# ZhengyiLuo/PULSE

Measured on NVIDIA H100. Metric: env-steps/sec at 16384 humanoid envs, 1/2/4/8 H100; obs-kernel HBM GB/s, higher is better.
Workload: dtype bf16 GEMM operands, fp32 accumulate / master weights / observations

## Files before the change

include/pulse_b200.h:

```cpp
#ifndef PULSE_B200_H_
#define PULSE_B200_H_

#include <stdint.h>

#ifdef __cplusplus
extern "C" {
#endif

#define PULSE_ABI_VERSION 3

enum pulse_status {
  PULSE_OK = 0,
  PULSE_ERR_ARG = -1,
  PULSE_ERR_CUDA = -2,
  PULSE_ERR_UNSUPPORTED = -3
};

#define PULSE_NUM_BODIES 24
#define PULSE_NUM_DOF 69
#define PULSE_BODY_STATE_W 13
#define PULSE_SELF_OBS 358
#define PULSE_TASK_OBS_V6 576
#define PULSE_IM_OBS (PULSE_SELF_OBS + PULSE_TASK_OBS_V6)
#define PULSE_AMP_OBS 196
#define PULSE_FRAME_REC 312
#define PULSE_AUX_REC 240

int pulse_abi_version(void);
const char* pulse_last_error(void);
int64_t pulse_launch_count(void);

typedef struct pulse_motionlib pulse_motionlib_t;

typedef struct {
  const float* gts;
  const float* grs;
  const float* lrs;
  const float* gvs;
  const float* gavs;
  const float* dvs;
  const float* motion_aa;
  const float* lengths;
  const float* dt;
  const int64_t* num_frames;
  const int64_t* length_starts;
  int64_t total_frames;
  int64_t num_motions;
  float* frame_rec;
  float* aux_rec;
} pulse_motionlib_desc_t;

int pulse_motionlib_create(const pulse_motionlib_desc_t* desc, void* stream, pulse_motionlib_t** out);
int pulse_motionlib_destroy(pulse_motionlib_t* lib);

typedef struct {
  const int64_t* motion_ids;
  const float* motion_times;
  const float* offset;
  float* root_pos;
  float* root_rot;
  float* dof_pos;
  float* root_vel;
  float* root_ang_vel;
  float* dof_vel;
  float* motion_aa;
  float* rg_pos;
  float* rb_rot;
  float* body_vel;
  float* body_ang_vel;
  int64_t* frame_idx0;
  int64_t* frame_idx1;
  float* blend;
} pulse_motion_query_t;
int pulse_motion_state(const pulse_motionlib_t* lib, const pulse_motion_query_t* q, int64_t n, void* stream);

#define PULSE_STEP_REWARD 1u
#define PULSE_STEP_RESET 2u
#define PULSE_STEP_OBS 4u
#define PULSE_STEP_ALL 7u
#define PULSE_STEP_ADVANCE 8u

typedef struct {
  const float* body_state;
  int64_t body_env_stride;
  const float* dof_vel;
  int64_t dof_env_stride;
  int64_t dof_elem_stride;
  const float* dof_force;
  int64_t dof_force_stride;
  const int64_t* env_ids;
  const int64_t* progress_buf;
  const int64_t* motion_ids;
  const float* motion_start_times;
  const float* motion_start_offset;
  const float* global_offset;
  const int32_t* cycle_counter;
  const int64_t* reset_buf_in;
  const float* termination_distances;
  uint32_t reset_body_mask;
  uint32_t flags;
  float dt;
  float k_pos, k_rot, k_vel, k_ang_vel, w_pos, w_rot, w_vel, w_ang_vel;
  float power_coefficient;
  int32_t cycle_motion;
  int64_t max_episode_length;
  int32_t enable_early_termination;
  int32_t use_mean_reset;
  float* obs_buf;
  int64_t obs_stride;
  float* self_obs_buf;
  float* rew_buf;
  float* reward_raw;
  int64_t raw_stride;
  int64_t* reset_buf;
  int64_t* terminate_buf;
  uint8_t* pass_time;
  float* ref_body_pos;
  float* ref_body_vel;
  float* ref_body_rot;
  float* ref_dof_pos;
  const int32_t* env_count;
  const int32_t* recovery_counter;
  int64_t* progress_rw;
  float* fdones_out;
} pulse_im_step_args_t;
int pulse_im_step(const pulse_motionlib_t* lib, const pulse_im_step_args_t* args, int64_t num_envs, void* stream);

typedef struct {
  const float* body_state; int64_t body_env_stride;
  const float* dof_pos; const float* dof_vel; int64_t dof_env_stride; int64_t dof_elem_stride;
  float* amp_obs_buf;
  int32_t num_steps;
  int32_t shift_history;
} pulse_amp_obs_args_t;
int pulse_amp_obs(const pulse_amp_obs_args_t* args, int64_t num_envs, void* stream);

typedef struct {
  const float* mu; int64_t ld_mu;
  const float* logstd;
  const float* eps; int64_t ld_eps;
  uint64_t seed; const uint64_t* rng_offset; uint64_t rng_step;
  int32_t num_actions; int32_t reserved;
  float* actions; int64_t ld_actions;
  float* neglogp; int64_t ld_neglogp;
  float* mus_out; int64_t ld_mus;
  const float* value; int64_t ld_value;
  const double* value_mean; const double* value_var; float value_eps; int32_t reserved2;
  float* values_out; int64_t ld_values;
  const float* pd_offset; const float* pd_scale; float* pd_targets; int64_t ld_pd;
} pulse_policy_post_args_t;
int pulse_policy_post(const pulse_policy_post_args_t* args, int64_t rows, void* stream);
int pulse_value_post(const float* value, int64_t ld_value, const double* mean, const double* var, float eps, const int64_t* terminate,
                     float* out, int64_t ld_out, int64_t rows, void* stream);
typedef struct {
  const float* body_state; int64_t body_env_stride;
  const float* dof_pos; const float* dof_vel; int64_t dof_env_stride; int64_t dof_elem_stride;
  const float* prev; int64_t ld_prev;
  float* out; int64_t ld_out;
  int32_t num_steps; int32_t reserved;
  int32_t* fresh;
  const float* fresh_rows;
} pulse_amp_row_args_t;
int pulse_amp_obs_row(const pulse_amp_row_args_t* args, int64_t num_envs, void* stream);
int pulse_bump_counter(uint64_t* counter, uint64_t by, void* stream);
int pulse_event_create(void** event);
int pulse_event_destroy(void* event);
int pulse_event_record(void* event, void* stream);
int pulse_event_elapsed_ms(void* start, void* stop, float* ms);

typedef struct {
  int64_t* reset_buf;
  const int64_t* env_ids_in;
  int64_t num_ids;
  const float* phase;
  uint64_t seed, offset;
  const int64_t* motion_ids;
  float* motion_start_times;
  float* motion_start_offset;
  float* global_offset;
  int32_t* cycle_counter;
  int64_t* progress_buf;
  int64_t* terminate_buf;
  float* root_states; int64_t root_env_stride;
  float* dof_pos; float* dof_vel; int64_t dof_env_stride; int64_t dof_elem_stride;
  float* rigid_body_state; int64_t body_env_stride;
  float* contact_forces; int64_t contact_env_stride; int32_t contact_bodies;
  int32_t num_amp_steps;
  float* amp_obs_buf;
  float dt;
  int32_t reserved;
  const int32_t* actor_ids;
  int64_t* env_list;
  int32_t* actor_list;
  int32_t* count;
  int32_t* amp_fresh;
  const uint64_t* offset_dev;
} pulse_reset_args_t;
int pulse_reset_ref_state(const pulse_motionlib_t* lib, const pulse_reset_args_t* args, int64_t num_envs, void* stream);

typedef struct {
  const float* rewards;
  const float* values;
  const float* next_values;
  const float* fdones;
  float gamma, tau;
  float* advantages;
  float* returns;
  double* adv_sum;
} pulse_gae_args_t;
int pulse_gae(const pulse_gae_args_t* args, int32_t horizon, int64_t num_envs, void* stream);
int pulse_normalize_advantages(float* advantages, const double* adv_sum, int64_t count, void* stream);

typedef uint16_t pulse_bf16_t;
#define PULSE_ACT_NONE 0
#define PULSE_ACT_RELU 1
#define PULSE_ACT_SILU 2

typedef struct {
  const float* bias;
  int32_t act;
  int32_t gate_mode;
  const pulse_bf16_t* gate;
  int64_t ldg;
  float alpha;
  pulse_bf16_t* out;
  int64_t ldo;
  pulse_bf16_t* out_t;
  int64_t ldot;
  float* out_f32;
  int64_t ldf;
  int64_t split_stride;
  pulse_bf16_t* preact;
  int64_t ldp;
  float* colsum;
  int32_t accumulate;
  int32_t reserved;
  double* sumsq;
  uint32_t* relu_mask; int64_t ld_rmask;
  const uint32_t* gate_mask; int64_t ld_gmask;
} pulse_gemm_epilogue_t;

#define PULSE_GEMM_A_MN 1u
#define PULSE_GEMM_B_MN 2u

int pulse_gemm_bf16_nt(const void* a, int64_t lda, const void* b, int64_t ldb, int64_t m, int64_t n, int64_t k,
                       const pulse_gemm_epilogue_t* ep, int32_t split_k, void* stream);
int pulse_gemm_bf16(const void* a, int64_t lda, const void* b, int64_t ldb, int64_t m, int64_t n, int64_t k,
                    const pulse_gemm_epilogue_t* ep, int32_t split_k, uint32_t flags, void* stream);
int pulse_gemm_num_splits(int64_t k, int32_t split_k);

typedef struct {
  const void* a; int64_t lda;
  const void* b; int64_t ldb;
  int64_t m, n, k;
  pulse_gemm_epilogue_t ep;
  int32_t split_k, reserved;
} pulse_gemm_problem_t;
int pulse_gemm_bf16_grouped(const pulse_gemm_problem_t* problems, int32_t count, uint32_t flags, void* stream);

int pulse_normalize_to_bf16(const float* x, int64_t ldx, int64_t rows, int64_t cols, const float* mean, const float* rstd,
                            pulse_bf16_t* out, int64_t ld_out, pulse_bf16_t* out_t, int64_t ld_t, float pad_one, void* stream);

int pulse_column_moments(const float* x, int64_t ldx, int64_t rows, int64_t cols, double* sums, void* stream);

int pulse_normalize_moments(const float* x, int64_t ldx, int64_t rows, int64_t cols, const float* mean, const float* rstd,
                            pulse_bf16_t* out, int64_t ld_out, double* sums, float pad_one, void* stream);

int pulse_rms_merge(double* sums, int64_t n, int32_t size, double* mean, double* var, double* count, float eps,
                    float* mean_f32, float* rstd_f32, void* stream);

int pulse_head1_forward(const pulse_bf16_t* h, int64_t ldh, int64_t rows, int32_t k, const pulse_bf16_t* w, const float* bias, float* out,
                        int64_t ldo, void* stream);

#define PULSE_HEAD1_MAX_CTAS 264
int pulse_head1_backward(const pulse_bf16_t* h, int64_t ldh, int64_t rows, int32_t k, const pulse_bf16_t* dv, int64_t ld_dv,
                         const pulse_bf16_t* w, pulse_bf16_t* dh, int64_t ld_dh, float* dw, float* db, float* dbias_prev, float* partials,
                         void* stream);

int pulse_ordered_sum_add(const float* x, int64_t n, int64_t stride_n, int64_t rows, int64_t cols, int64_t ld, float* out, int64_t ldo,
                          void* stream);

int pulse_gaussian_sample(const float* mu, int64_t ld_mu, const float* eps, const float* logstd, int64_t rows, int32_t num_actions,
                          float* actions, float* neglogp, void* stream);

typedef struct {
  const float* mu; int64_t ld_mu;
  const float* value; int64_t ld_value;
  const float* actions;
  const float* old_neglogp;
  const float* advantages;
  const float* returns;
  const float* old_mu;
  const float* logstd;
  int32_t num_actions;
  float e_clip, critic_coef, bounds_coef;
  pulse_bf16_t* dmu; int64_t ld_dmu; pulse_bf16_t* dmu_t; int64_t ld_dmu_t;
  pulse_bf16_t* dvalue; int64_t ld_dv; pulse_bf16_t* dvalue_t; int64_t ld_dv_t;
  double* stats;
} pulse_ppo_loss_args_t;
int pulse_ppo_loss(const pulse_ppo_loss_args_t* args, int64_t rows, void* stream);

int pulse_disc_loss(const float* logits, int64_t ld, int64_t n_agent, int64_t n_demo, float scale, pulse_bf16_t* dlogit, int64_t ld_d,
                    double* stats, void* stream);
int pulse_relu_mask_scale(const pulse_bf16_t* h, int64_t ldh, int64_t rows, int64_t cols, const float* w, pulse_bf16_t* out, int64_t ldo,
                          void* stream);
int pulse_axpy(float a, const float* x, float* y, int64_t count, void* stream);
typedef struct {
  const float* w; float* g; int64_t rows, cols, ld; float coef; int32_t reserved; double* sumsq; double* sumsq2;
} pulse_weight_block_t;
typedef struct { pulse_weight_block_t block[4]; int32_t count; int32_t reserved; } pulse_weight_reg_t;
int pulse_weight_reg(const pulse_weight_reg_t* desc, void* stream);

int pulse_column_sum_bf16(const pulse_bf16_t* x, int64_t ldx, int64_t rows, int64_t cols, float* out, void* stream);
int pulse_reduce_slabs(const float* slabs, int64_t slab_stride, int32_t num_slabs, int64_t count, float* dst, void* stream);
int pulse_sum_squares(const float* x, int64_t count, double* sumsq, void* stream);
#define PULSE_ADAM_ZERO_GRADS 1u
#define PULSE_ADAM_SELF_CONTAINED 2u
int pulse_adam_step(float* params, float* grads, float* exp_avg, float* exp_avg_sq, int64_t count, double* grad_sumsq,
                    float max_norm, float lr, float beta1, float beta2, float eps, int32_t* step, pulse_bf16_t* params_bf16, uint32_t flags,
                    uint32_t* block_counter, void* stream);
#define PULSE_PEER_MAX 8
#define PULSE_PEER_MAX_GRID 256
#define PULSE_PEER_SIGNAL_BYTES (3 * PULSE_PEER_MAX * 4 + PULSE_PEER_MAX * 8)
typedef struct {
  int32_t rank, world;
  float* grads[PULSE_PEER_MAX];
  float* params[PULSE_PEER_MAX];
  pulse_bf16_t* params_bf16[PULSE_PEER_MAX];
  uint32_t* signals[PULSE_PEER_MAX];
  const float* mc_grads; float* mc_params; pulse_bf16_t* mc_params_bf16;
  float* exp_avg; float* exp_avg_sq;
  int64_t count;
  float max_norm, lr, beta1, beta2, eps;
  int32_t grid;
  uint32_t timeout_ms;
  uint32_t reserved;
  int32_t* step;
  uint32_t* epoch;
  double* cta_partials;
  unsigned long long* grid_bar;
} pulse_peer_adam_args_t;
int pulse_peer_reduce_adam(const pulse_peer_adam_args_t* args, void* stream);

int pulse_refresh_weight_bf16(const float* w, int64_t n, int64_t k, pulse_bf16_t* w_bf16, int64_t ld_k, pulse_bf16_t* wt_bf16,
                              int64_t ld_n, void* stream);

int pulse_normalize_cols(const float* x, int64_t ldx, int64_t rows, int64_t cols, const float* mean, const float* rstd, float clamp,
                         pulse_bf16_t* out, int64_t ld_out, int64_t zero_to, void* stream);
int pulse_copy_cols_bf16(const pulse_bf16_t* src, int64_t ld_src, int64_t rows, int64_t cols, pulse_bf16_t* dst1, int64_t ld1,
                         pulse_bf16_t* dst2, int64_t ld2, void* stream);

#define PULSE_Z_SAMPLE 0
#define PULSE_Z_MEAN 1
#define PULSE_Z_RESIDUAL 2
int pulse_vae_reparam(const float* head, int64_t ld_head, const float* noise, int64_t ld_noise, int64_t rows, int32_t latent,
                      int32_t mode, int32_t clamp, float clamp_lo, float clamp_hi, pulse_bf16_t* z_bf16, int64_t ld_z, float* z_f32,
                      int64_t ld_zf, void* stream);

int pulse_vae_action_loss(const float* pred, int64_t ld_pred, const float* gt, int64_t ld_gt, int64_t rows, int32_t num_actions,
                          pulse_bf16_t* dpred, int64_t ld_d, int64_t zero_to, double* stats, void* stream);

typedef struct {
  const float* enc_head; int64_t ld_enc;
  const float* prior_head; int64_t ld_prior;
  const float* noise; int64_t ld_noise;
  const float* dz; int64_t ld_dz;
  const int64_t* progress;
  int32_t latent, horizon, clamp, reserved;
  float clamp_lo, clamp_hi, kld_coef, ar1_coef, regu_coef, phi;
  pulse_bf16_t* d_enc_head; int64_t ld_de;
  pulse_bf16_t* d_prior_head; int64_t ld_dp;
  double* stats;
} pulse_vae_latent_args_t;
int pulse_vae_latent_loss(const pulse_vae_latent_args_t* args, int64_t rows, void* stream);

int pulse_pnn_compose(const float* acts, int64_t prim_stride, int64_t ld_a, const float* w, int64_t ld_w, int32_t act, int64_t rows,
                      int32_t num_actions, int32_t num_prim, float* out, int64_t ld_out, void* stream);

int pulse_pd_targets(const float* action, int64_t ld_a, const float* offset, const float* scale, const uint8_t* freeze, int64_t rows,
                     int32_t dofs, float* out, int64_t ld_out, void* stream);

int pulse_reach_update_task(const int64_t* progress, int64_t* tar_change_steps, float* tar_pos, const float* rand01, const int64_t* steps,
                            float dist_max, float h_min, float h_max, int64_t num_envs, void* stream);

typedef struct {
  const float* body_state; int64_t body_env_stride;
  const float* contact_forces; int64_t contact_env_stride;
  const float* termination_heights;
  const float* tar_pos;
  const int64_t* progress_buf;
  uint32_t contact_body_mask;
  int32_t reach_body_id;
  int32_t enable_early_termination, reserved;
  int64_t max_episode_length;
  float* obs_buf; int64_t obs_stride;
  float* rew_buf;
  int64_t* reset_buf; int64_t* terminate_buf;
} pulse_reach_step_args_t;
#define PULSE_REACH_OBS 361
int pulse_reach_step(const pulse_reach_step_args_t* args, int64_t num_envs, void* stream);

#define PULSE_ZTASK_SPEED 1
#define PULSE_ZTASK_STRIKE 2
#define PULSE_SPEED_OBS 361
#define PULSE_STRIKE_OBS 373
typedef struct {
  int32_t kind, enable_early_termination;
  const float* body_state; int64_t body_env_stride;
  const float* contact_forces; int64_t contact_env_stride;
  const float* termination_heights;
  uint32_t contact_body_mask;
  uint32_t strike_body_mask;
  const int64_t* progress_buf; int64_t max_episode_length;
  const float* prev_root_pos; float dt; float power_coefficient;
  const float* tar_speed;
  const float* target_states; int64_t target_env_stride;
  const float* tar_contact_forces; int64_t tar_contact_env_stride;
  const float* dof_force; int64_t dof_force_stride;
  const float* dof_vel; int64_t dof_env_stride, dof_elem_stride;
  float* obs_buf; int64_t obs_stride; float* rew_buf; float* reward_raw; int64_t raw_stride;
  int64_t* reset_buf; int64_t* terminate_buf;
} pulse_ztask_step_args_t;
int pulse_ztask_step(const pulse_ztask_step_args_t* args, int64_t num_envs, void* stream);

#define PULSE_TRAJ_VERTS 101
#define PULSE_TRAJ_DRAWS (4 * (PULSE_TRAJ_VERTS - 1) + 2)
#define PULSE_TERRAIN_OBS 1402
typedef struct {
  uint32_t flags;
  int32_t upright;
  const float* body_state; int64_t body_env_stride;
  const float* root_states; int64_t root_env_stride;
  const int64_t* progress_buf; int64_t max_episode_length;
  const float* contact_forces; int64_t contact_env_stride;
  uint32_t contact_body_mask;
  int32_t enable_early_termination, no_collision_check, fuzzy_target, power_reward;
  int32_t num_traj_samples, num_height_points, num_center_points, head_body_id, use_center_height;
  float dt, traj_dur, traj_sample_timestep, fail_dist, power_coefficient;
  const float* traj_verts;
  const int16_t* heightfield; int64_t hf_rows, hf_cols;
  float horizontal_scale, vertical_scale;
  const float* height_points;
  const float* center_points;
  const float* dof_force; int64_t dof_force_stride;
  const float* dof_vel; int64_t dof_env_stride, dof_elem_stride;
  const int64_t* env_ids; const int32_t* env_count;
  float* obs_buf; int64_t obs_stride;
  float* rew_buf; float* reward_raw; int64_t raw_stride;
  int64_t* reset_buf; int64_t* terminate_buf;
} pulse_terrain_step_args_t;
int pulse_terrain_step(const pulse_terrain_step_args_t* args, int64_t num_envs, void* stream);

typedef struct {
  const int64_t* env_ids; int64_t num_ids;
  const float* init_pos; int64_t init_stride;
  const float* rand;
  uint64_t seed, offset; const uint64_t* offset_dev;
  float dtheta_scale, dspeed_scale, seg_dt, speed_min, speed_max, sharp_turn_prob;
  float* verts;
} pulse_traj_reset_args_t;
int pulse_traj_reset(const pulse_traj_reset_args_t* args, void* stream);

#define PULSE_HEIGHTS_CENTER 1
#define PULSE_HEIGHTS_GRID 2
typedef struct {
  int32_t mode, upright;
  const float* root_states; int64_t root_stride; int64_t num_rows;
  const float* points; int64_t num_points;
  const int16_t* heightfield; int64_t hf_rows, hf_cols;
  float horizontal_scale, vertical_scale;
  float* heights; int64_t heights_stride;
} pulse_terrain_heights_args_t;
int pulse_terrain_heights(const pulse_terrain_heights_args_t* args, void* stream);

typedef struct {
  const float* body_state; int64_t body_env_stride;
  const int32_t* track_ids;
  int32_t num_track, time_steps, version, upright;
  const float* ref_pos; const float* ref_rot; const float* ref_vel; const float* ref_ang_vel;
  const float* dof_pos; int64_t dof_env_stride, dof_elem_stride;
  const float* ref_dof_pos;
  float* obs; int64_t obs_stride;
  int64_t num_envs;
} pulse_task_obs_args_t;
int pulse_task_obs_size(int32_t version, int32_t num_track, int32_t time_steps);
int pulse_im_task_obs(const pulse_task_obs_args_t* args, void* stream);

typedef struct {
  const float* body_pos; int64_t pos_env_stride, pos_body_stride;
  const float* body_pos_gt; int64_t gt_env_stride, gt_body_stride;
  const int64_t* terminate;
  const int32_t* num_steps;
  int32_t num_envs, bound, max_steps_all, reserved;
  int32_t* ctrl; int32_t* terminate_state; float* hist; double* sums; int32_t* counts; float* mpjpe_out;
} pulse_eval_args_t;
int pulse_eval_step(const pulse_eval_args_t* args, void* stream);

typedef struct {
  const double* pose_quat_global;
  const double* root_trans;
  const int32_t* frame_clip;
  const int64_t* clip_start;
  const float* fps;
  const double* headings;
  const int32_t* parents;
  const float* local_translation;
  int64_t total_frames, num_clips;
  float* gts; float* grs; float* lrs; float* gvs; float* gavs; float* dvs;
  float* tmp_vel; float* tmp_ang;
} pulse_loader_args_t;
int pulse_motionlib_load_clips(const pulse_loader_args_t* args, void* stream);

#ifdef __cplusplus
}
#endif
#endif
```

pulse_b200/_lib.py:

```python
import ctypes as C
import os

_PKG = os.path.dirname(os.path.abspath(__file__))
LIB_PATH = os.path.join(_PKG, "libpulse_b200.so")


class PulseError(RuntimeError):
    pass


c_float_p = C.POINTER(C.c_float)
c_i64_p = C.POINTER(C.c_int64)
c_i32_p = C.POINTER(C.c_int32)
c_u8_p = C.POINTER(C.c_uint8)
c_f64_p = C.POINTER(C.c_double)


class MotionLibDesc(C.Structure):
    _fields_ = [
        ("gts", C.c_void_p), ("grs", C.c_void_p), ("lrs", C.c_void_p), ("gvs", C.c_void_p), ("gavs", C.c_void_p),
        ("dvs", C.c_void_p), ("motion_aa", C.c_void_p), ("lengths", C.c_void_p), ("dt", C.c_void_p),
        ("num_frames", C.c_void_p), ("length_starts", C.c_void_p), ("total_frames", C.c_int64),
        ("num_motions", C.c_int64), ("frame_rec", C.c_void_p), ("aux_rec", C.c_void_p),
    ]


class MotionQuery(C.Structure):
    _fields_ = [(n, C.c_void_p) for n in (
        "motion_ids", "motion_times", "offset", "root_pos", "root_rot", "dof_pos", "root_vel", "root_ang_vel", "dof_vel",
        "motion_aa", "rg_pos", "rb_rot", "body_vel", "body_ang_vel", "frame_idx0", "frame_idx1", "blend")]


class ImStepArgs(C.Structure):
    _fields_ = [
        ("body_state", C.c_void_p), ("body_env_stride", C.c_int64),
        ("dof_vel", C.c_void_p), ("dof_env_stride", C.c_int64), ("dof_elem_stride", C.c_int64),
        ("dof_force", C.c_void_p), ("dof_force_stride", C.c_int64), ("env_ids", C.c_void_p),
        ("progress_buf", C.c_void_p), ("motion_ids", C.c_void_p), ("motion_start_times", C.c_void_p),
        ("motion_start_offset", C.c_void_p), ("global_offset", C.c_void_p), ("cycle_counter", C.c_void_p),
        ("reset_buf_in", C.c_void_p), ("termination_distances", C.c_void_p),
        ("reset_body_mask", C.c_uint32), ("flags", C.c_uint32), ("dt", C.c_float),
        ("k_pos", C.c_float), ("k_rot", C.c_float), ("k_vel", C.c_float), ("k_ang_vel", C.c_float),
        ("w_pos", C.c_float), ("w_rot", C.c_float), ("w_vel", C.c_float), ("w_ang_vel", C.c_float),
        ("power_coefficient", C.c_float), ("cycle_motion", C.c_int32), ("max_episode_length", C.c_int64),
        ("enable_early_termination", C.c_int32), ("use_mean_reset", C.c_int32),
        ("obs_buf", C.c_void_p), ("obs_stride", C.c_int64), ("self_obs_buf", C.c_void_p), ("rew_buf", C.c_void_p),
        ("reward_raw", C.c_void_p), ("raw_stride", C.c_int64), ("reset_buf", C.c_void_p), ("terminate_buf", C.c_void_p),
        ("pass_time", C.c_void_p), ("ref_body_pos", C.c_void_p), ("ref_body_vel", C.c_void_p),
        ("ref_body_rot", C.c_void_p), ("ref_dof_pos", C.c_void_p),
        ("env_count", C.c_void_p), ("recovery_counter", C.c_void_p), ("progress_rw", C.c_void_p), ("fdones_out", C.c_void_p),
    ]


class ResetArgs(C.Structure):
    _fields_ = [
        ("reset_buf", C.c_void_p), ("env_ids_in", C.c_void_p), ("num_ids", C.c_int64), ("phase", C.c_void_p),
        ("seed", C.c_uint64), ("offset", C.c_uint64), ("motion_ids", C.c_void_p), ("motion_start_times", C.c_void_p),
        ("motion_start_offset", C.c_void_p), ("global_offset", C.c_void_p), ("cycle_counter", C.c_void_p), ("progress_buf", C.c_void_p),
        ("terminate_buf", C.c_void_p), ("root_states", C.c_void_p), ("root_env_stride", C.c_int64),
        ("dof_pos", C.c_void_p), ("dof_vel", C.c_void_p), ("dof_env_stride", C.c_int64), ("dof_elem_stride", C.c_int64),
        ("rigid_body_state", C.c_void_p), ("body_env_stride", C.c_int64),
        ("contact_forces", C.c_void_p), ("contact_env_stride", C.c_int64), ("contact_bodies", C.c_int32),
        ("num_amp_steps", C.c_int32), ("amp_obs_buf", C.c_void_p), ("dt", C.c_float), ("reserved", C.c_int32),
        ("actor_ids", C.c_void_p), ("env_list", C.c_void_p), ("actor_list", C.c_void_p), ("count", C.c_void_p), ("amp_fresh", C.c_void_p),
        ("offset_dev", C.c_void_p),
    ]


class WeightBlock(C.Structure):
    _fields_ = [("w", C.c_void_p), ("g", C.c_void_p), ("rows", C.c_int64), ("cols", C.c_int64), ("ld", C.c_int64), ("coef", C.c_float),
                ("reserved", C.c_int32), ("sumsq", C.c_void_p), ("sumsq2", C.c_void_p)]


class WeightReg(C.Structure):
    _fields_ = [("block", WeightBlock * 4), ("count", C.c_int32), ("reserved", C.c_int32)]


class PolicyPostArgs(C.Structure):
    _fields_ = [
        ("mu", C.c_void_p), ("ld_mu", C.c_int64), ("logstd", C.c_void_p), ("eps", C.c_void_p), ("ld_eps", C.c_int64),
        ("seed", C.c_uint64), ("rng_offset", C.c_void_p), ("rng_step", C.c_uint64), ("num_actions", C.c_int32), ("reserved", C.c_int32),
        ("actions", C.c_void_p), ("ld_actions", C.c_int64), ("neglogp", C.c_void_p), ("ld_neglogp", C.c_int64),
        ("mus_out", C.c_void_p), ("ld_mus", C.c_int64), ("value", C.c_void_p), ("ld_value", C.c_int64),
        ("value_mean", C.c_void_p), ("value_var", C.c_void_p), ("value_eps", C.c_float), ("reserved2", C.c_int32),
        ("values_out", C.c_void_p), ("ld_values", C.c_int64),
        ("pd_offset", C.c_void_p), ("pd_scale", C.c_void_p), ("pd_targets", C.c_void_p), ("ld_pd", C.c_int64),
    ]


class AmpRowArgs(C.Structure):
    _fields_ = [
        ("body_state", C.c_void_p), ("body_env_stride", C.c_int64), ("dof_pos", C.c_void_p), ("dof_vel", C.c_void_p),
        ("dof_env_stride", C.c_int64), ("dof_elem_stride", C.c_int64), ("prev", C.c_void_p), ("ld_prev", C.c_int64),
        ("out", C.c_void_p), ("ld_out", C.c_int64), ("num_steps", C.c_int32), ("reserved", C.c_int32),
        ("fresh", C.c_void_p), ("fresh_rows", C.c_void_p),
    ]


class AmpObsArgs(C.Structure):
    _fields_ = [
        ("body_state", C.c_void_p), ("body_env_stride", C.c_int64), ("dof_pos", C.c_void_p), ("dof_vel", C.c_void_p),
        ("dof_env_stride", C.c_int64), ("dof_elem_stride", C.c_int64), ("amp_obs_buf", C.c_void_p),
        ("num_steps", C.c_int32), ("shift_history", C.c_int32),
    ]


class GaeArgs(C.Structure):
    _fields_ = [
        ("rewards", C.c_void_p), ("values", C.c_void_p), ("next_values", C.c_void_p), ("fdones", C.c_void_p),
        ("gamma", C.c_float), ("tau", C.c_float), ("advantages", C.c_void_p), ("returns", C.c_void_p), ("adv_sum", C.c_void_p),
    ]


class GemmEpilogue(C.Structure):
    _fields_ = [
        ("bias", C.c_void_p), ("act", C.c_int32), ("gate_mode", C.c_int32), ("gate", C.c_void_p), ("ldg", C.c_int64),
        ("alpha", C.c_float), ("out", C.c_void_p), ("ldo", C.c_int64), ("out_t", C.c_void_p), ("ldot", C.c_int64),
        ("out_f32", C.c_void_p), ("ldf", C.c_int64), ("split_stride", C.c_int64), ("preact", C.c_void_p), ("ldp", C.c_int64),
        ("colsum", C.c_void_p), ("accumulate", C.c_int32), ("reserved", C.c_int32), ("sumsq", C.c_void_p),
        ("relu_mask", C.c_void_p), ("ld_rmask", C.c_int64), ("gate_mask", C.c_void_p), ("ld_gmask", C.c_int64),
    ]


GEMM_A_MN, GEMM_B_MN = 1, 2


class GemmProblem(C.Structure):
    _fields_ = [("a", C.c_void_p), ("lda", C.c_int64), ("b", C.c_void_p), ("ldb", C.c_int64), ("m", C.c_int64), ("n", C.c_int64),
                ("k", C.c_int64), ("ep", GemmEpilogue), ("split_k", C.c_int32), ("reserved", C.c_int32)]


class PpoLossArgs(C.Structure):
    _fields_ = [
        ("mu", C.c_void_p), ("ld_mu", C.c_int64), ("value", C.c_void_p), ("ld_value", C.c_int64), ("actions", C.c_void_p),
        ("old_neglogp", C.c_void_p), ("advantages", C.c_void_p), ("returns", C.c_void_p), ("old_mu", C.c_void_p),
        ("logstd", C.c_void_p), ("num_actions", C.c_int32), ("e_clip", C.c_float), ("critic_coef", C.c_float),
        ("bounds_coef", C.c_float), ("dmu", C.c_void_p), ("ld_dmu", C.c_int64), ("dmu_t", C.c_void_p), ("ld_dmu_t", C.c_int64),
        ("dvalue", C.c_void_p), ("ld_dv", C.c_int64), ("dvalue_t", C.c_void_p), ("ld_dv_t", C.c_int64), ("stats", C.c_void_p),
    ]


class VaeLatentArgs(C.Structure):
    _fields_ = [
        ("enc_head", C.c_void_p), ("ld_enc", C.c_int64), ("prior_head", C.c_void_p), ("ld_prior", C.c_int64),
        ("noise", C.c_void_p), ("ld_noise", C.c_int64), ("dz", C.c_void_p), ("ld_dz", C.c_int64), ("progress", C.c_void_p),
        ("latent", C.c_int32), ("horizon", C.c_int32), ("clamp", C.c_int32), ("reserved", C.c_int32),
        ("clamp_lo", C.c_float), ("clamp_hi", C.c_float), ("kld_coef", C.c_float), ("ar1_coef", C.c_float),
        ("regu_coef", C.c_float), ("phi", C.c_float),
        ("d_enc_head", C.c_void_p), ("ld_de", C.c_int64), ("d_prior_head", C.c_void_p), ("ld_dp", C.c_int64), ("stats", C.c_void_p),
    ]


class ReachStepArgs(C.Structure):
    _fields_ = [
        ("body_state", C.c_void_p), ("body_env_stride", C.c_int64), ("contact_forces", C.c_void_p), ("contact_env_stride", C.c_int64),
        ("termination_heights", C.c_void_p), ("tar_pos", C.c_void_p), ("progress_buf", C.c_void_p),
        ("contact_body_mask", C.c_uint32), ("reach_body_id", C.c_int32), ("enable_early_termination", C.c_int32), ("reserved", C.c_int32),
        ("max_episode_length", C.c_int64), ("obs_buf", C.c_void_p), ("obs_stride", C.c_int64), ("rew_buf", C.c_void_p),
        ("reset_buf", C.c_void_p), ("terminate_buf", C.c_void_p),
    ]


class LoaderArgs(C.Structure):
    _fields_ = [
        ("pose_quat_global", C.c_void_p), ("root_trans", C.c_void_p), ("frame_clip", C.c_void_p), ("clip_start", C.c_void_p),
        ("fps", C.c_void_p), ("headings", C.c_void_p), ("parents", C.c_void_p), ("local_translation", C.c_void_p),
        ("total_frames", C.c_int64), ("num_clips", C.c_int64),
        ("gts", C.c_void_p), ("grs", C.c_void_p), ("lrs", C.c_void_p), ("gvs", C.c_void_p), ("gavs", C.c_void_p), ("dvs", C.c_void_p),
        ("tmp_vel", C.c_void_p), ("tmp_ang", C.c_void_p),
    ]


class ZTaskStepArgs(C.Structure):
    _fields_ = [
        ("kind", C.c_int32), ("enable_early_termination", C.c_int32), ("body_state", C.c_void_p), ("body_env_stride", C.c_int64),
        ("contact_forces", C.c_void_p), ("contact_env_stride", C.c_int64), ("termination_heights", C.c_void_p),
        ("contact_body_mask", C.c_uint32), ("strike_body_mask", C.c_uint32), ("progress_buf", C.c_void_p), ("max_episode_length", C.c_int64),
        ("prev_root_pos", C.c_void_p), ("dt", C.c_float), ("power_coefficient", C.c_float), ("tar_speed", C.c_void_p),
        ("target_states", C.c_void_p), ("target_env_stride", C.c_int64), ("tar_contact_forces", C.c_void_p), ("tar_contact_env_stride", C.c_int64),
        ("dof_force", C.c_void_p), ("dof_force_stride", C.c_int64), ("dof_vel", C.c_void_p), ("dof_env_stride", C.c_int64), ("dof_elem_stride", C.c_int64),
        ("obs_buf", C.c_void_p), ("obs_stride", C.c_int64), ("rew_buf", C.c_void_p), ("reward_raw", C.c_void_p), ("raw_stride", C.c_int64),
        ("reset_buf", C.c_void_p), ("terminate_buf", C.c_void_p),
    ]


ZTASK_SPEED, ZTASK_STRIKE = 1, 2


class TerrainStepArgs(C.Structure):
    _fields_ = [
        ("flags", C.c_uint32), ("upright", C.c_int32), ("body_state", C.c_void_p), ("body_env_stride", C.c_int64),
        ("root_states", C.c_void_p), ("root_env_stride", C.c_int64), ("progress_buf", C.c_void_p), ("max_episode_length", C.c_int64),
        ("contact_forces", C.c_void_p), ("contact_env_stride", C.c_int64), ("contact_body_mask", C.c_uint32),
        ("enable_early_termination", C.c_int32), ("no_collision_check", C.c_int32), ("fuzzy_target", C.c_int32), ("power_reward", C.c_int32),
        ("num_traj_samples", C.c_int32), ("num_height_points", C.c_int32), ("num_center_points", C.c_int32), ("head_body_id", C.c_int32),
        ("use_center_height", C.c_int32), ("dt", C.c_float), ("traj_dur", C.c_float), ("traj_sample_timestep", C.c_float),
        ("fail_dist", C.c_float), ("power_coefficient", C.c_float), ("traj_verts", C.c_void_p),
        ("heightfield", C.c_void_p), ("hf_rows", C.c_int64), ("hf_cols", C.c_int64), ("horizontal_scale", C.c_float), ("vertical_scale", C.c_float),
        ("height_points", C.c_void_p), ("center_points", C.c_void_p), ("dof_force", C.c_void_p), ("dof_force_stride", C.c_int64),
        ("dof_vel", C.c_void_p), ("dof_env_stride", C.c_int64), ("dof_elem_stride", C.c_int64), ("env_ids", C.c_void_p), ("env_count", C.c_void_p),
        ("obs_buf", C.c_void_p), ("obs_stride", C.c_int64), ("rew_buf", C.c_void_p), ("reward_raw", C.c_void_p), ("raw_stride", C.c_int64),
        ("reset_buf", C.c_void_p), ("terminate_buf", C.c_void_p),
    ]


class TrajResetArgs(C.Structure):
    _fields_ = [
        ("env_ids", C.c_void_p), ("num_ids", C.c_int64), ("init_pos", C.c_void_p), ("init_stride", C.c_int64), ("rand", C.c_void_p),
        ("seed", C.c_uint64), ("offset", C.c_uint64), ("offset_dev", C.c_void_p), ("dtheta_scale", C.c_float), ("dspeed_scale", C.c_float),
        ("seg_dt", C.c_float), ("speed_min", C.c_float), ("speed_max", C.c_float), ("sharp_turn_prob", C.c_float), ("verts", C.c_void_p),
    ]


class TerrainHeightsArgs(C.Structure):
    _fields_ = [
        ("mode", C.c_int32), ("upright", C.c_int32), ("root_states", C.c_void_p), ("root_stride", C.c_int64), ("num_rows", C.c_int64),
        ("points", C.c_void_p), ("num_points", C.c_int64), ("heightfield", C.c_void_p), ("hf_rows", C.c_int64), ("hf_cols", C.c_int64),
        ("horizontal_scale", C.c_float), ("vertical_scale", C.c_float), ("heights", C.c_void_p), ("heights_stride", C.c_int64),
    ]


TRAJ_VERTS = 101
TRAJ_DRAWS = 4 * (TRAJ_VERTS - 1) + 2
HEIGHTS_CENTER, HEIGHTS_GRID = 1, 2


class TaskObsArgs(C.Structure):
    _fields_ = [
        ("body_state", C.c_void_p), ("body_env_stride", C.c_int64), ("track_ids", C.c_void_p),
        ("num_track", C.c_int32), ("time_steps", C.c_int32), ("version", C.c_int32), ("upright", C.c_int32),
        ("ref_pos", C.c_void_p), ("ref_rot", C.c_void_p), ("ref_vel", C.c_void_p), ("ref_ang_vel", C.c_void_p),
        ("dof_pos", C.c_void_p), ("dof_env_stride", C.c_int64), ("dof_elem_stride", C.c_int64), ("ref_dof_pos", C.c_void_p),
        ("obs", C.c_void_p), ("obs_stride", C.c_int64), ("num_envs", C.c_int64),
    ]


class EvalArgs(C.Structure):
    _fields_ = [
        ("body_pos", C.c_void_p), ("pos_env_stride", C.c_int64), ("pos_body_stride", C.c_int64),
        ("body_pos_gt", C.c_void_p), ("gt_env_stride", C.c_int64), ("gt_body_stride", C.c_int64),
        ("terminate", C.c_void_p), ("num_steps", C.c_void_p),
        ("num_envs", C.c_int32), ("bound", C.c_int32), ("max_steps_all", C.c_int32), ("reserved", C.c_int32),
        ("ctrl", C.c_void_p), ("terminate_state", C.c_void_p), ("hist", C.c_void_p), ("sums", C.c_void_p), ("counts", C.c_void_p),
        ("mpjpe_out", C.c_void_p),
    ]


PEER_MAX, PEER_MAX_GRID, PEER_SIGNAL_BYTES = 8, 256, 3 * 8 * 4 + 8 * 8


class PeerAdamArgs(C.Structure):
    _fields_ = [
        ("rank", C.c_int32), ("world", C.c_int32),
        ("grads", C.c_void_p * PEER_MAX), ("params", C.c_void_p * PEER_MAX), ("params_bf16", C.c_void_p * PEER_MAX),
        ("signals", C.c_void_p * PEER_MAX),
        ("mc_grads", C.c_void_p), ("mc_params", C.c_void_p), ("mc_params_bf16", C.c_void_p),
        ("exp_avg", C.c_void_p), ("exp_avg_sq", C.c_void_p), ("count", C.c_int64),
        ("max_norm", C.c_float), ("lr", C.c_float), ("beta1", C.c_float), ("beta2", C.c_float), ("eps", C.c_float), ("grid", C.c_int32),
        ("timeout_ms", C.c_uint32), ("reserved", C.c_uint32), ("step", C.c_void_p), ("epoch", C.c_void_p), ("cta_partials", C.c_void_p), ("grid_bar", C.c_void_p),
    ]


ABI_VERSION = 3
HEAD1_MAX_CTAS = 264
ACT_NONE, ACT_RELU, ACT_SILU = 0, 1, 2
Z_SAMPLE, Z_MEAN, Z_RESIDUAL = 0, 1, 2
STEP_REWARD, STEP_RESET, STEP_OBS, STEP_ALL, STEP_ADVANCE = 1, 2, 4, 7, 8

SIGNATURES = {
    "pulse_abi_version": (C.c_int, []),
    "pulse_last_error": (C.c_char_p, []),
    "pulse_launch_count": (C.c_int64, []),
    "pulse_motionlib_create": (C.c_int, [C.POINTER(MotionLibDesc), C.c_void_p, C.POINTER(C.c_void_p)]),
    "pulse_motionlib_destroy": (C.c_int, [C.c_void_p]),
    "pulse_motion_state": (C.c_int, [C.c_void_p, C.POINTER(MotionQuery), C.c_int64, C.c_void_p]),
    "pulse_im_step": (C.c_int, [C.c_void_p, C.POINTER(ImStepArgs), C.c_int64, C.c_void_p]),
    "pulse_reset_ref_state": (C.c_int, [C.c_void_p, C.POINTER(ResetArgs), C.c_int64, C.c_void_p]),
    "pulse_policy_post": (C.c_int, [C.POINTER(PolicyPostArgs), C.c_int64, C.c_void_p]),
    "pulse_value_post": (C.c_int, [C.c_void_p, C.c_int64, C.c_void_p, C.c_void_p, C.c_float, C.c_void_p, C.c_void_p, C.c_int64, C.c_int64, C.c_void_p]),
    "pulse_amp_obs_row": (C.c_int, [C.POINTER(AmpRowArgs), C.c_int64, C.c_void_p]),
    "pulse_bump_counter": (C.c_int, [C.c_void_p, C.c_uint64, C.c_void_p]),
    "pulse_event_create": (C.c_int, [C.POINTER(C.c_void_p)]),
    "pulse_event_destroy": (C.c_int, [C.c_void_p]),
    "pulse_event_record": (C.c_int, [C.c_void_p, C.c_void_p]),
    "pulse_event_elapsed_ms": (C.c_int, [C.c_void_p, C.c_void_p, C.POINTER(C.c_float)]),
    "pulse_amp_obs": (C.c_int, [C.POINTER(AmpObsArgs), C.c_int64, C.c_void_p]),
    "pulse_gae": (C.c_int, [C.POINTER(GaeArgs), C.c_int32, C.c_int64, C.c_void_p]),
    "pulse_normalize_advantages": (C.c_int, [C.c_void_p, C.c_void_p, C.c_int64, C.c_void_p]),
    "pulse_gemm_bf16_nt": (C.c_int, [C.c_void_p, C.c_int64, C.c_void_p, C.c_int64, C.c_int64, C.c_int64, C.c_int64,
                                     C.POINTER(GemmEpilogue), C.c_int32, C.c_void_p]),
    "pulse_gemm_bf16": (C.c_int, [C.c_void_p, C.c_int64, C.c_void_p, C.c_int64, C.c_int64, C.c_int64, C.c_int64,
                                  C.POINTER(GemmEpilogue), C.c_int32, C.c_uint32, C.c_void_p]),
    "pulse_gemm_num_splits": (C.c_int, [C.c_int64, C.c_int32]),
    "pulse_gemm_bf16_grouped": (C.c_int, [C.POINTER(GemmProblem), C.c_int32, C.c_uint32, C.c_void_p]),
    "pulse_normalize_to_bf16": (C.c_int, [C.c_void_p, C.c_int64, C.c_int64, C.c_int64, C.c_void_p, C.c_void_p, C.c_void_p, C.c_int64,
                                          C.c_void_p, C.c_int64, C.c_float, C.c_void_p]),
    "pulse_normalize_moments": (C.c_int, [C.c_void_p, C.c_int64, C.c_int64, C.c_int64, C.c_void_p, C.c_void_p, C.c_void_p, C.c_int64,
                                          C.c_void_p, C.c_float, C.c_void_p]),
    "pulse_head1_forward": (C.c_int, [C.c_void_p, C.c_int64, C.c_int64, C.c_int32, C.c_void_p, C.c_void_p, C.c_void_p, C.c_int64, C.c_void_p]),
    "pulse_head1_backward": (C.c_int, [C.c_void_p, C.c_int64, C.c_int64, C.c_int32, C.c_void_p, C.c_int64, C.c_void_p, C.c_void_p, C.c_int64,
                                       C.c_void_p, C.c_void_p, C.c_void_p, C.c_void_p, C.c_void_p]),
    "pulse_ordered_sum_add": (C.c_int, [C.c_void_p, C.c_int64, C.c_int64, C.c_int64, C.c_int64, C.c_int64, C.c_void_p, C.c_int64, C.c_void_p]),
    "pulse_column_moments": (C.c_int, [C.c_void_p, C.c_int64, C.c_int64, C.c_int64, C.c_void_p, C.c_void_p]),
    "pulse_rms_merge": (C.c_int, [C.c_void_p, C.c_int64, C.c_int32, C.c_void_p, C.c_void_p, C.c_void_p, C.c_float, C.c_void_p, C.c_void_p,
                                  C.c_void_p]),
    "pulse_gaussian_sample": (C.c_int, [C.c_void_p, C.c_int64, C.c_void_p, C.c_void_p, C.c_int64, C.c_int32, C.c_void_p, C.c_void_p,
                                        C.c_void_p]),
    "pulse_ppo_loss": (C.c_int, [C.POINTER(PpoLossArgs), C.c_int64, C.c_void_p]),
    "pulse_disc_loss": (C.c_int, [C.c_void_p, C.c_int64, C.c_int64, C.c_int64, C.c_float, C.c_void_p, C.c_int64, C.c_void_p, C.c_void_p]),
    "pulse_relu_mask_scale": (C.c_int, [C.c_void_p, C.c_int64, C.c_int64, C.c_int64, C.c_void_p, C.c_void_p, C.c_int64, C.c_void_p]),
    "pulse_weight_reg": (C.c_int, [C.POINTER(WeightReg), C.c_void_p]),
    "pulse_axpy": (C.c_int, [C.c_float, C.c_void_p, C.c_void_p, C.c_int64, C.c_void_p]),
    "pulse_column_sum_bf16": (C.c_int, [C.c_void_p, C.c_int64, C.c_int64, C.c_int64, C.c_void_p, C.c_void_p]),
    "pulse_reduce_slabs": (C.c_int, [C.c_void_p, C.c_int64, C.c_int32, C.c_int64, C.c_void_p, C.c_void_p]),
    "pulse_sum_squares": (C.c_int, [C.c_void_p, C.c_int64, C.c_void_p, C.c_void_p]),
    "pulse_adam_step": (C.c_int, [C.c_void_p, C.c_void_p, C.c_void_p, C.c_void_p, C.c_int64, C.c_void_p, C.c_float, C.c_float,
                                  C.c_float, C.c_float, C.c_float, C.c_void_p, C.c_void_p, C.c_uint32, C.c_void_p, C.c_void_p]),
    "pulse_peer_reduce_adam": (C.c_int, [C.POINTER(PeerAdamArgs), C.c_void_p]),
    "pulse_refresh_weight_bf16": (C.c_int, [C.c_void_p, C.c_int64, C.c_int64, C.c_void_p, C.c_int64, C.c_void_p, C.c_int64, C.c_void_p]),
    "pulse_normalize_cols": (C.c_int, [C.c_void_p, C.c_int64, C.c_int64, C.c_int64, C.c_void_p, C.c_void_p, C.c_float, C.c_void_p, C.c_int64,
                                       C.c_int64, C.c_void_p]),
    "pulse_copy_cols_bf16": (C.c_int, [C.c_void_p, C.c_int64, C.c_int64, C.c_int64, C.c_void_p, C.c_int64, C.c_void_p, C.c_int64, C.c_void_p]),
    "pulse_vae_reparam": (C.c_int, [C.c_void_p, C.c_int64, C.c_void_p, C.c_int64, C.c_int64, C.c_int32, C.c_int32, C.c_int32, C.c_float,
                                    C.c_float, C.c_void_p, C.c_int64, C.c_void_p, C.c_int64, C.c_void_p]),
    "pulse_vae_action_loss": (C.c_int, [C.c_void_p, C.c_int64, C.c_void_p, C.c_int64, C.c_int64, C.c_int32, C.c_void_p, C.c_int64, C.c_int64,
                                        C.c_void_p, C.c_void_p]),
    "pulse_vae_latent_loss": (C.c_int, [C.POINTER(VaeLatentArgs), C.c_int64, C.c_void_p]),
    "pulse_pnn_compose": (C.c_int, [C.c_void_p, C.c_int64, C.c_int64, C.c_void_p, C.c_int64, C.c_int32, C.c_int64, C.c_int32, C.c_int32,
                                    C.c_void_p, C.c_int64, C.c_void_p]),
    "pulse_pd_targets": (C.c_int, [C.c_void_p, C.c_int64, C.c_void_p, C.c_void_p, C.c_void_p, C.c_int64, C.c_int32, C.c_void_p, C.c_int64,
                                   C.c_void_p]),
    "pulse_reach_update_task": (C.c_int, [C.c_void_p, C.c_void_p, C.c_void_p, C.c_void_p, C.c_void_p, C.c_float, C.c_float, C.c_float,
                                          C.c_int64, C.c_void_p]),
    "pulse_reach_step": (C.c_int, [C.POINTER(ReachStepArgs), C.c_int64, C.c_void_p]),
    "pulse_ztask_step": (C.c_int, [C.POINTER(ZTaskStepArgs), C.c_int64, C.c_void_p]),
    "pulse_terrain_step": (C.c_int, [C.POINTER(TerrainStepArgs), C.c_int64, C.c_void_p]),
    "pulse_traj_reset": (C.c_int, [C.POINTER(TrajResetArgs), C.c_void_p]),
    "pulse_terrain_heights": (C.c_int, [C.POINTER(TerrainHeightsArgs), C.c_void_p]),
    "pulse_task_obs_size": (C.c_int, [C.c_int32, C.c_int32, C.c_int32]),
    "pulse_im_task_obs": (C.c_int, [C.POINTER(TaskObsArgs), C.c_void_p]),
    "pulse_eval_step": (C.c_int, [C.POINTER(EvalArgs), C.c_void_p]),
    "pulse_motionlib_load_clips": (C.c_int, [C.POINTER(LoaderArgs), C.c_void_p]),
}

_lib = None


def load():
    global _lib
    if _lib is not None:
        return _lib
    if not os.path.exists(LIB_PATH):
        raise PulseError(f"{LIB_PATH} is missing: build it with `python -m pulse_b200.build` "
                         "(nvcc, sm_90a). pulse_b200 has no CPU fallback.")
    lib = C.CDLL(LIB_PATH)
    for name, (res, args) in SIGNATURES.items():
        fn = getattr(lib, name)
        fn.restype = res
        fn.argtypes = args
    if lib.pulse_abi_version() != ABI_VERSION:
        raise PulseError(f"ABI version mismatch: library {lib.pulse_abi_version()} != binding {ABI_VERSION}")
    _lib = lib
    return lib


def check(status, what):
    if status != 0:
        msg = load().pulse_last_error().decode("utf-8", "replace")
        raise PulseError(f"{what} failed with status {status}: {msg}")


def ptr(t):
    return None if t is None else C.c_void_p(t.data_ptr())


def current_stream(device=None):
    import torch
    return C.c_void_p(torch.cuda.current_stream(device).cuda_stream)


class GraphEvent:

    def __init__(self):
        self._h = C.c_void_p()
        check(load().pulse_event_create(C.byref(self._h)), "pulse_event_create")

    def record(self, device=None):
        check(load().pulse_event_record(self._h, current_stream(device)), "pulse_event_record")

    def elapsed_ms(self, stop: "GraphEvent") -> float:
        ms = C.c_float()
        check(load().pulse_event_elapsed_ms(self._h, stop._h, C.byref(ms)), "pulse_event_elapsed_ms")
        return float(ms.value)

    def __del__(self):
        try:
            if self._h:
                load().pulse_event_destroy(self._h)
        except Exception:
            pass
```

pulse_b200/amp.py:

```python
import ctypes as C
from typing import Dict, Optional, Sequence

import torch

from . import _lib
from .dense import column_sum_add, gemm
from .nets import MLP, FlatParams, pad_k, pick_split
from .ppo import RunningMeanStdB200


class AmpDiscriminator:
    def __init__(self, flat: FlatParams, amp_obs_size: int = 1960, units: Sequence[int] = (1024, 512), disc_coef: float = 5.0,
                 logit_reg: float = 0.01, grad_penalty: float = 5.0, weight_decay: float = 0.0001, reward_scale: float = 2.0):
        self.flat, self.device = flat, flat.device
        self.size = amp_obs_size
        self.mlp = MLP(flat, amp_obs_size, units, 1, "relu", aug=True)
        self.Kp = self.mlp.Kp0
        if len(units) != 2:
            raise _lib.PulseError("the analytic gradient penalty is written for the 2-hidden-layer discriminator of im.yaml")
        self.disc_coef, self.logit_reg, self.grad_penalty, self.weight_decay = disc_coef, logit_reg, grad_penalty, weight_decay
        self.reward_scale = reward_scale
        self.rms = RunningMeanStdB200(amp_obs_size, self.device)
        self.rms.pad_one = 1.0
        self.stats = torch.zeros(8, dtype=torch.float64, device=self.device)
        self._bufs: Dict[int, dict] = {}
        self.lib = _lib.load()

    def rewards(self, amp_obs: torch.Tensor, x_buf: Optional[torch.Tensor] = None) -> torch.Tensor:
        R = amp_obs.shape[0]
        x = x_buf if x_buf is not None else torch.empty(R, self.Kp, device=self.device, dtype=torch.bfloat16)
        self.rms.normalize_into(amp_obs, x)
        logits = self.mlp.forward(x)
        prob = 1.0 / (1.0 + torch.exp(-logits))
        return -torch.log(torch.clamp(1.0 - prob, min=1e-4)) * self.reward_scale

    def _buf(self, B: int):
        if B not in self._bufs:
            dev, bf = self.device, torch.bfloat16
            L1, L2, _ = self.mlp.layers
            self._bufs[B] = {
                "x": torch.zeros(2, 3 * B, self.Kp, device=dev, dtype=bf),
                "dlogit": torch.zeros(3 * B, 8, device=dev, dtype=bf),
                "g2": torch.zeros(B, L2.Np, device=dev, dtype=bf), "g1": torch.zeros(B, L1.Np, device=dev, dtype=bf),
                "Gb": torch.zeros(B, self.Kp, device=dev, dtype=bf),
                "du": torch.zeros(B, L1.Np, device=dev, dtype=bf), "scratch": torch.zeros(B, L2.Np, device=dev),
                "split1": pick_split(((L1.N + 127) // 128) * ((L1.Kp + 127) // 128), (B + 63) // 64),
                "split2": pick_split(((L2.N + 127) // 128) * ((L2.Kp + 127) // 128), (B + 63) // 64),
            }
        return self._bufs[B]

    def prepare_inputs(self, amp_agent: torch.Tensor, amp_replay: torch.Tensor, amp_demo: torch.Tensor, update_rms: bool = True, slot: int = 0) -> None:
        B = amp_agent.shape[0]
        if amp_replay.shape[0] != B or amp_demo.shape[0] != B:
            raise _lib.PulseError("agent / replay / demo AMP batches must have the same number of rows")
        x = self._buf(B)["x"][slot]
        for k, src in enumerate((amp_agent, amp_replay, amp_demo)):
            if update_rms:
                self.rms.normalize_update(src, x[k * B:(k + 1) * B])
            else:
                self.rms.normalize_into(src, x[k * B:(k + 1) * B])

    def loss_backward(self, amp_agent: torch.Tensor, amp_replay: torch.Tensor, amp_demo: torch.Tensor, update_rms: bool = True,
                      slot: int = 0, prepared: bool = False) -> torch.Tensor:
        B = amp_agent.shape[0]
        if not prepared:
            self.prepare_inputs(amp_agent, amp_replay, amp_demo, update_rms, slot)
        b = self._buf(B)
        lib, dev = self.lib, self.device
        L1, L2, L3 = self.mlp.layers
        x = b["x"][slot]
        logits = self.mlp.forward(x, train=True)
        self.stats.zero_()
        with torch.cuda.device(dev):
            st = _lib.current_stream(dev)
            _lib.check(lib.pulse_disc_loss(logits.data_ptr(), logits.stride(0), 2 * B, B, self.disc_coef, b["dlogit"].data_ptr(),
                                           b["dlogit"].stride(0), self.stats.data_ptr(), st), "pulse_disc_loss")
        self.mlp.backward(b["dlogit"], 3 * B)
        ws = self.mlp._ws[(3 * B, True)]
        h2 = ws["act"][1][2 * B:]
        m1, m2 = ws["mask"][0][:, 2 * B:], ws["mask"][1][:, 2 * B:]
        w3 = L3.weight.view(-1)
        with torch.cuda.device(dev):
            _lib.check(lib.pulse_relu_mask_scale(h2.data_ptr(), h2.stride(0), B, L2.N, w3.data_ptr(), b["g2"].data_ptr(), b["g2"].stride(0),
                                                 _lib.current_stream(dev)), "pulse_relu_mask_scale")
        W1, W2 = L1.w_bf16[:, :L1.K], L2.w_bf16[:, :L1.N]
        gemm(b["g2"][:, :L2.N], W2, b_mn=True, gate_mask=m1, out=b["g1"])
        c = 2.0 * self.disc_coef * self.grad_penalty / B
        gemm(b["g1"][:, :L1.N], W1, b_mn=True, alpha=c, out=b["Gb"], sumsq=self.stats[4:])
        gemm(b["g1"][:, :L1.N], b["Gb"], a_mn=True, b_mn=True, out_f32=L1.weight_grad, accumulate=True, split_k=b["split1"])
        gemm(b["Gb"], L1.w_bf16, gate_mask=m1, out=b["du"])
        gemm(b["g2"][:, :L2.N], b["du"][:, :L1.N], a_mn=True, b_mn=True, out_f32=L2.weight_grad, accumulate=True, split_k=b["split2"])
        gemm(b["du"][:, :L1.N], W2, gate_mask=m2, out_f32=b["scratch"])
        column_sum_add(b["scratch"][:, :L2.N], L3.weight_grad.view(-1))
        reg = _lib.WeightReg()
        reg.count = 3
        for k, l in enumerate((L1, L2, L3)):
            coef = 2.0 * self.disc_coef * (self.weight_decay + (self.logit_reg if l is L3 else 0.0))
            blk = reg.block[k]
            blk.w, blk.g, blk.rows, blk.cols, blk.ld, blk.coef = l.weight.data_ptr(), l.weight_grad.data_ptr(), l.N, l.K, l.Kp, coef
            blk.sumsq = self.stats[6:].data_ptr()
            if l is L3:
                blk.sumsq2 = self.stats[5:].data_ptr()
        with torch.cuda.device(dev):
            _lib.check(lib.pulse_weight_reg(C.byref(reg), _lib.current_stream(dev)), "pulse_weight_reg")
        return self.stats

    def loss_from_stats(self, stats: torch.Tensor, B: int) -> Dict[str, float]:
        s = stats.cpu()
        c = 2.0 * self.disc_coef * self.grad_penalty / B
        gp = float(s[4]) / (c * c) / B
        bce = 0.5 * (float(s[0]) / (2 * B) + float(s[1]) / B)
        loss = bce + self.logit_reg * float(s[5]) + self.grad_penalty * gp + self.weight_decay * float(s[6])
        return {"disc_loss": loss, "disc_grad_penalty": gp, "disc_logit_loss": float(s[5]), "disc_agent_acc": float(s[2]) / (2 * B),
                "disc_demo_acc": float(s[3]) / B}

    def loss_tensors(self, B: int) -> Dict[str, torch.Tensor]:
        s = self.stats
        c = 2.0 * self.disc_coef * self.grad_penalty / B
        gp = s[4] / (c * c) / B
        bce = 0.5 * (s[0] / (2 * B) + s[1] / B)
        logits = self.mlp._ws[(3 * B, True)]["out"]
        return {"disc_loss": bce + self.logit_reg * s[5] + self.grad_penalty * gp + self.weight_decay * s[6], "disc_grad_penalty": gp,
                "disc_logit_loss": s[5].clone(), "disc_agent_acc": s[2] / (2 * B), "disc_demo_acc": s[3] / B,
                "disc_agent_logit": logits[:2 * B].mean(), "disc_demo_logit": logits[2 * B:].mean()}

    def state_dict(self) -> Dict[str, torch.Tensor]:
        sd = {f"a2c_network.{k}": v for k, v in self.mlp.state_dict("_disc_mlp", "_disc_logits").items()}
        sd["amp_input_mean_std.running_mean"] = self.rms.running_mean.clone()
        sd["amp_input_mean_std.running_var"] = self.rms.running_var.clone()
        sd["amp_input_mean_std.count"] = self.rms.count.clone()
        return sd
```

pulse_b200/csrc/gemm_kernel.inc:

```
#if PULSE_GEMM_GROUPED
#define PULSE_GEMM_FIRST(member) grp.p[0].member
#define PULSE_GEMM_W wl
#define PULSE_GEMM_SELECT(w)                                                                                         \
  int pi = 0;                                                                                                        \
  while (pi + 1 < grp.count && (w) >= grp.p[pi].item_end) ++pi;                                                      \
  const GemmProblem& P = grp.p[pi];                                                                                  \
  const int wl = (w) - (pi == 0 ? 0 : grp.p[pi - 1].item_end);                                                       \
  const CUtensorMap& map_a = P.map_a;                                                                                \
  const CUtensorMap& map_b = P.map_b;                                                                                \
  const CUtensorMap& map_c = P.map_c;                                                                                \
  const int use_tma_red = P.use_tma_red;                                                                             \
  const pulse_gemm_epilogue_t& ep = P.ep;                                                                            \
  const int M = P.M, N = P.N, K = P.K, kb_per_split = P.kb_per_split;                                                \
  const int tiles_n = (N + BN - 1) / BN, tiles_m = (M + BM - 1) / BM;                                                \
  const int tiles = tiles_m * tiles_n;                                                                               \
  const int num_kb_total = (K + BK - 1) / BK;                                                                        \
  (void)map_a; (void)map_b; (void)map_c; (void)use_tma_red; (void)ep; (void)M; (void)N; (void)tiles_n; (void)kb_per_split; (void)num_kb_total;
#else
#define PULSE_GEMM_FIRST(member) member
#define PULSE_GEMM_W w
#define PULSE_GEMM_SELECT(w)
#endif

#if PULSE_GEMM_GROUPED
template <bool A_MN, bool B_MN, int MODE>
__global__ void __launch_bounds__(kThreads, 1) gemm_bf16_grouped_kernel(const __grid_constant__ GemmGroup grp) {
#else
template <bool A_MN, bool B_MN, int MODE>
__global__ void __launch_bounds__(kThreads, 1) gemm_bf16_kernel(const __grid_constant__ CUtensorMap map_a,
                                                                const __grid_constant__ CUtensorMap map_b,
                                                                const __grid_constant__ CUtensorMap map_c,
                                                                const pulse_gemm_epilogue_t ep, int M, int N, int K,
                                                                int kb_per_split, int splits, int use_tma_red) {
#endif
  constexpr bool kFwd = MODE == kModeGeneric || MODE == kModeFwd;
  constexpr bool kDgrad = MODE == kModeGeneric || MODE == kModeDgrad || MODE == kModeDgradVec;
  constexpr bool kGateVec = MODE == kModeGeneric || MODE == kModeDgradVec;
  constexpr bool kAccum = MODE == kModeGeneric || MODE == kModeWgrad;
  constexpr bool kBf16Out = MODE != kModeWgrad;
  extern __shared__ unsigned char gsm_raw[];
  GemmSmem& sm = *reinterpret_cast<GemmSmem*>((reinterpret_cast<uintptr_t>(gsm_raw) + 1023) & ~static_cast<uintptr_t>(1023));
  const int warp = threadIdx.x >> 5, lane = threadIdx.x & 31;
  const int work0 = static_cast<int>(blockIdx.x);
  const int work_stride = static_cast<int>(gridDim.x);
#if PULSE_GEMM_GROUPED
  const int total = grp.total_items;
#else
  const int tiles_n = (N + BN - 1) / BN, tiles_m = (M + BM - 1) / BM;
  const int tiles = tiles_m * tiles_n;
  const int total = tiles * splits;
  const int num_kb_total = (K + BK - 1) / BK;
#endif
  if (threadIdx.x == 0) PULSE_TRACE(0);

  if (threadIdx.x == 0) {
#pragma unroll
    for (int s = 0; s < kStages; ++s) {
      g_mbar_init(&sm.full[s], 1);
      g_mbar_init(&sm.empty[s], kConsumerWarps);
    }
    asm volatile("fence.mbarrier_init.release.cluster;\n" ::: "memory");
    asm volatile("prefetch.tensormap [%0];\n" ::"l"(&PULSE_GEMM_FIRST(map_a)) : "memory");
    asm volatile("prefetch.tensormap [%0];\n" ::"l"(&PULSE_GEMM_FIRST(map_b)) : "memory");
  }
  __syncthreads();
  if (threadIdx.x == 0) PULSE_TRACE(1);
  asm volatile("griddepcontrol.launch_dependents;\n" ::: "memory");

  if (warp < 4) {
    if (warp == 0 && lane == 0) {
      asm volatile("griddepcontrol.wait;\n" ::: "memory");
      PULSE_TRACE(2);
      int it = 0;
      for (int w = work0; w < total; w += work_stride) {
        PULSE_GEMM_SELECT(w)
        const int split = PULSE_GEMM_W / tiles, t = PULSE_GEMM_W - split * tiles;
        const int m0 = (t / tiles_n) * BM, n0 = (t % tiles_n) * BN;
        const int kb0 = split * kb_per_split;
        const int num_kb = min(kb_per_split, num_kb_total - kb0);
        for (int kb = 0; kb < num_kb; ++kb, ++it) {
          const int s = it % kStages;
          g_mbar_wait(&sm.empty[s], ((it / kStages) & 1) ^ 1);
          g_mbar_expect_tx(&sm.full[s], kStageBytesA + kStageBytesB);
          const int kk = (kb0 + kb) * BK;
          if (A_MN) {
            tma_load_2d(sm.a[s], &map_a, m0, kk, &sm.full[s]);
            tma_load_2d(sm.a[s] + 8192, &map_a, m0 + 64, kk, &sm.full[s]);
          } else {
            tma_load_2d(sm.a[s], &map_a, kk, m0, &sm.full[s]);
          }
          if (B_MN) {
            tma_load_2d(sm.b[s], &map_b, n0, kk, &sm.full[s]);
            tma_load_2d(sm.b[s] + 8192, &map_b, n0 + 64, kk, &sm.full[s]);
          } else {
            tma_load_2d(sm.b[s], &map_b, kk, n0, &sm.full[s]);
          }
        }
      }
    }
  } else {
    const int wg = (warp >> 2) - 1;
    const int ew = warp - 4;
    const int quarter = wg * 2 + (warp & 1);
    const int chalf = (warp >> 1) & 1;
    float* red_stage = sm.red[ew];
    float* acc_s = sm.acc[wg];
    asm volatile("griddepcontrol.wait;\n" ::: "memory");
    int it = 0, lw = 0;
    for (int w = work0; w < total; w += work_stride, ++lw) {
      PULSE_GEMM_SELECT(w)
      const int split = PULSE_GEMM_W / tiles, t = PULSE_GEMM_W - split * tiles;
      const int m0 = (t / tiles_n) * BM, n0 = (t % tiles_n) * BN;
      const int kb0 = split * kb_per_split;
      const int num_kb = min(kb_per_split, num_kb_total - kb0);
      const int row = m0 + quarter * 32 + lane;
      const bool row_ok = row < M;
      const bool gate_fast = (MODE == kModeGeneric || MODE == kModeDgrad) && ep.gate != nullptr && ep.gate_mask == nullptr && ep.gate_mode == PULSE_ACT_RELU && (ep.ldg & 7) == 0 && n0 + chalf * kCols + kCols <= N;
      unsigned gmask[kChunks] = {};
      const bool gate_bits = kDgrad && ep.gate_mask != nullptr;
      if (gate_bits && row_ok) {
#pragma unroll
        for (int cc = 0; cc < kChunks; ++cc) {
          const int col = n0 + (chalf * kChunks + cc) * 32;
          if (col < N) gmask[cc] = __ldg(ep.gate_mask + static_cast<long long>(col >> 5) * ep.ld_gmask + row);
        }
      }
      if (gate_fast && row_ok) {
        const uint4* g = reinterpret_cast<const uint4*>(reinterpret_cast<const __nv_bfloat16*>(ep.gate) + static_cast<long long>(row) * ep.ldg +
                                                        n0 + chalf * kCols);
        uint4 u[kChunks * 4];
#pragma unroll
        for (int i = 0; i < kChunks * 4; ++i) u[i] = __ldg(g + i);
#pragma unroll
        for (int i = 0; i < kChunks * 4; ++i) {
          const unsigned wds[4] = {u[i].x, u[i].y, u[i].z, u[i].w};
#pragma unroll
          for (int q = 0; q < 4; ++q) {
            const unsigned pos = (((wds[q] & 0x7fff7fffu) + 0x7fff7fffu) & ~wds[q]) & 0x80008000u;
            gmask[i >> 2] |= (pos >> 15) << ((i & 3) * 4 + q);
          }
        }
      }
      const bool gate_vec = kGateVec && ep.gate != nullptr && !gate_fast && !gate_bits && (ep.ldg & 7) == 0;
      uint4 gq[4] = {};
      auto gate_fetch = [&](int cc) {
        const int c0 = n0 + cc * 32;
        if (gate_vec && row_ok && c0 + 32 <= N) {
          const uint4* g = reinterpret_cast<const uint4*>(reinterpret_cast<const __nv_bfloat16*>(ep.gate) + static_cast<long long>(row) * ep.ldg + c0);
#pragma unroll
          for (int q = 0; q < 4; ++q) gq[q] = __ldg(g + q);
        }
      };
      gate_fetch(chalf * kChunks);
      float bias_l[kChunks] = {};
      const bool fwd_fast = MODE == kModeFwd && ep.out != nullptr && (ep.ldo & 7) == 0 && ep.out_f32 == nullptr && ep.out_t == nullptr &&
                            (ep.preact == nullptr || (ep.ldp & 7) == 0) && n0 + chalf * kCols + kCols <= N;
      float* bias_s = sm.bias[ew];
      if (fwd_fast && ep.bias != nullptr) {
        __syncwarp();
#pragma unroll
        for (int cc = 0; cc < kChunks; ++cc) bias_s[cc * 32 + lane] = __ldg(ep.bias + n0 + (chalf * kChunks + cc) * 32 + lane);
        __syncwarp();
      } else if (kFwd && ep.bias != nullptr) {
#pragma unroll
        for (int cc = 0; cc < kChunks; ++cc) {
          const int col = n0 + (chalf * kChunks + cc) * 32 + lane;
          if (col < N) bias_l[cc] = __ldg(ep.bias + col);
        }
      }

      float d[64];
#pragma unroll
      for (int i = 0; i < 64; ++i) d[i] = 0.0f;
      acc_fence(d);
      int prev_s = -1;
      for (int kb = 0; kb < num_kb; ++kb, ++it) {
        const int s = it % kStages;
        g_mbar_wait(&sm.full[s], (it / kStages) & 1);
        if (it == 0 && ew == 0 && lane == 0) PULSE_TRACE(3);
        wgmma_fence();
        const unsigned a_addr = s_u32(sm.a[s]) + static_cast<unsigned>(wg) * 8192u, b_addr = s_u32(sm.b[s]);
#pragma unroll
        for (int k = 0; k < BK / MMA_K; ++k) {
          const unsigned long long da = A_MN ? gmma_desc(a_addr + k * 2048, 8192) : gmma_desc(a_addr + k * 32, 16);
          const unsigned long long db = B_MN ? gmma_desc(b_addr + k * 2048, 8192) : gmma_desc(b_addr + k * 32, 16);
          wgmma_m64n128<A_MN ? 1 : 0, B_MN ? 1 : 0>(d, da, db, (kb | k) != 0 ? 1u : 0u);
        }
        wgmma_commit();
        wgmma_wait<1>();
        if (prev_s >= 0 && lane == 0) g_mbar_arrive(&sm.empty[prev_s]);
        prev_s = s;
      }
      wgmma_wait<0>();
      acc_fence(d);
      if (lane == 0) g_mbar_arrive(&sm.empty[prev_s]);
      if (ew == 0 && lane == 0 && lw < 3) PULSE_TRACE(4 + lw);

      wg_sync(wg);
      {
        const int r0 = (warp & 3) * 16 + (lane >> 2);
#pragma unroll
        for (int j = 0; j < BN / 8; ++j) {
          const int col = 8 * j + 2 * (lane & 3);
#pragma unroll
          for (int h = 0; h < 2; ++h) {
            const int r = r0 + 8 * h;
            const int rb = r & 31;
            float* blk = acc_s + ((r >> 5) * 4 + (col >> 5)) * 1024;
            const int unit = ((col & 31) >> 2) ^ (rb & 7);
            *reinterpret_cast<float2*>(blk + rb * 32 + unit * 4 + (col & 3)) = make_float2(d[4 * j + 2 * h], d[4 * j + 2 * h + 1]);
          }
        }
      }
      if (MODE == kModeWgrad && use_tma_red) asm volatile("fence.proxy.async.shared::cta;\n" ::: "memory");
      wg_sync(wg);
      if (ew == 0 && lane == 0 && lw < 3) PULSE_TRACE(16 + 2 * lw);

      float* outf = ep.out_f32 != nullptr ? ep.out_f32 + static_cast<long long>(ep.accumulate ? 0 : split) * ep.split_stride : nullptr;
      float sq = 0.0f;
#pragma unroll 1
      for (int c = chalf * kChunks; c < chalf * kChunks + kChunks; ++c) {
        const int col0 = n0 + c * 32;
        const bool full = col0 + 32 <= N;
        float* blk = acc_s + ((quarter & 1) * 4 + c) * 1024;
        if (MODE == kModeWgrad && use_tma_red) {
          if (lane == 0) {
            asm volatile("cp.reduce.async.bulk.tensor.2d.global.shared::cta.add.tile.bulk_group [%0, {%2, %3}], [%1];\n" ::"l"(&map_c),
                         "r"(s_u32(blk)), "r"(col0), "r"(m0 + quarter * 32)
                         : "memory");
            asm volatile("cp.async.bulk.commit_group;\n" ::: "memory");
          }
          continue;
        }
        float v[32];
        {
          const float4* b4 = reinterpret_cast<const float4*>(blk) + lane * 8;
#pragma unroll
          for (int u = 0; u < 8; ++u) {
            const float4 x = b4[u ^ (lane & 7)];
            v[4 * u] = x.x; v[4 * u + 1] = x.y; v[4 * u + 2] = x.z; v[4 * u + 3] = x.w;
          }
        }
        if (MODE != kModeWgrad && ep.alpha != 1.0f) {
#pragma unroll
          for (int i = 0; i < 32; ++i) v[i] *= ep.alpha;
        }
        if (fwd_fast) {
          if (ep.bias != nullptr) {
            const float4* b4 = reinterpret_cast<const float4*>(bias_s + (c % kChunks) * 32);
#pragma unroll
            for (int i = 0; i < 32; i += 4) {
              const float4 b = b4[i >> 2];
              v[i] += b.x; v[i + 1] += b.y; v[i + 2] += b.z; v[i + 3] += b.w;
            }
          }
          if (ep.relu_mask != nullptr) {
            unsigned word = 0u;
#pragma unroll
            for (int i = 0; i < 32; ++i) word |= (v[i] > 0.0f ? 1u : 0u) << i;
            if (row_ok) ep.relu_mask[static_cast<long long>(col0 >> 5) * ep.ld_rmask + row] = word;
          }
          uint4* st = reinterpret_cast<uint4*>(red_stage);
          const int sw = (lane >> 1) & 3;
#pragma unroll
          for (int q = 0; q < 4; ++q) {
            const int i = 8 * q;
            __nv_bfloat162 h0 = __floats2bfloat162_rn(v[i], v[i + 1]), h1 = __floats2bfloat162_rn(v[i + 2], v[i + 3]);
            __nv_bfloat162 h2 = __floats2bfloat162_rn(v[i + 4], v[i + 5]), h3 = __floats2bfloat162_rn(v[i + 6], v[i + 7]);
            uint4 u;
            u.x = *reinterpret_cast<unsigned*>(&h0);
            u.y = *reinterpret_cast<unsigned*>(&h1);
            u.z = *reinterpret_cast<unsigned*>(&h2);
            u.w = *reinterpret_cast<unsigned*>(&h3);
            st[lane * 4 + (q ^ sw)] = u;
          }
          __syncwarp();
          const long long coff = col0 + (lane & 3) * 8;
          const __nv_bfloat162 zero2 = __float2bfloat162_rn(0.0f);
#pragma unroll
          for (int it2 = 0; it2 < 4; ++it2) {
            const int rr = it2 * 8 + (lane >> 2);
            uint4 u = st[rr * 4 + ((lane & 3) ^ ((rr >> 1) & 3))];
            __nv_bfloat162* h = reinterpret_cast<__nv_bfloat162*>(&u);
            const long long grow = m0 + quarter * 32 + rr;
            if (grow < M) {
              if (ep.preact != nullptr) *reinterpret_cast<uint4*>(reinterpret_cast<__nv_bfloat16*>(ep.preact) + grow * ep.ldp + coff) = u;
              if (ep.act == PULSE_ACT_RELU) {
#pragma unroll
                for (int q = 0; q < 4; ++q) h[q] = __hmax2(h[q], zero2);
              } else if (ep.act == PULSE_ACT_SILU) {
#pragma unroll
                for (int q = 0; q < 4; ++q) h[q] = silu_bf16x2(h[q]);
              }
              *reinterpret_cast<uint4*>(reinterpret_cast<__nv_bfloat16*>(ep.out) + grow * ep.ldo + coff) = u;
            }
          }
          __syncwarp();
          continue;
        }
        if (kFwd && ep.bias != nullptr) {
          float bl = bias_l[0];
#pragma unroll
          for (int cc = 1; cc < kChunks; ++cc) bl = (c % kChunks) == cc ? bias_l[cc] : bl;
#pragma unroll
          for (int i = 0; i < 32; ++i) v[i] += __shfl_sync(0xffffffffu, bl, i);
        }
        if (kFwd && ep.preact != nullptr) {
          if (full && (ep.ldp & 7) == 0) {
            store_block_bf16(reinterpret_cast<uint4*>(red_stage), v,
                             reinterpret_cast<__nv_bfloat16*>(ep.preact) + static_cast<long long>(m0 + quarter * 32) * ep.ldp + col0, ep.ldp,
                             M - (m0 + quarter * 32), lane);
          } else if (row_ok) {
            __nv_bfloat16* p = reinterpret_cast<__nv_bfloat16*>(ep.preact) + static_cast<long long>(row) * ep.ldp + col0;
#pragma unroll
            for (int i = 0; i < 32; ++i)
              if (col0 + i < N) p[i] = __float2bfloat16(v[i]);
          }
        }
        if (kFwd && ep.relu_mask != nullptr && row_ok) {
          unsigned word = 0u;
#pragma unroll
          for (int i = 0; i < 32; ++i) word |= ((col0 + i < N && v[i] > 0.0f) ? 1u : 0u) << i;
          if (col0 < N) ep.relu_mask[static_cast<long long>(col0 >> 5) * ep.ld_rmask + row] = word;
        }
        if (kFwd && ep.act != PULSE_ACT_NONE) {
#pragma unroll
          for (int i = 0; i < 32; ++i) v[i] = act_apply(v[i], ep.act);
        }
        if (gate_bits) {
          unsigned mk = gmask[0];
#pragma unroll
          for (int cc = 1; cc < kChunks; ++cc) mk = (c % kChunks) == cc ? gmask[cc] : mk;
#pragma unroll
          for (int i = 0; i < 32; ++i) v[i] = ((mk >> i) & 1u) ? v[i] : 0.0f;
        } else if (gate_fast) {
          unsigned mk = gmask[0];
#pragma unroll
          for (int cc = 1; cc < kChunks; ++cc) mk = (c % kChunks) == cc ? gmask[cc] : mk;
#pragma unroll
          for (int i = 0; i < 32; ++i) v[i] = ((mk >> ((i >> 1) + 16 * (i & 1))) & 1u) ? v[i] : 0.0f;
        } else if (kDgrad && ep.gate != nullptr && row_ok) {
          const __nv_bfloat16* g = reinterpret_cast<const __nv_bfloat16*>(ep.gate) + static_cast<long long>(row) * ep.ldg + col0;
          if (full && (gate_vec || (ep.ldg & 7) == 0)) {
#pragma unroll
            for (int i = 0; i < 32; i += 8) {
              const uint4 u = gate_vec ? gq[i >> 3] : __ldg(reinterpret_cast<const uint4*>(g + i));
              const __nv_bfloat162* h = reinterpret_cast<const __nv_bfloat162*>(&u);
#pragma unroll
              for (int q = 0; q < 4; ++q) {
                const float2 f = __bfloat1622float2(h[q]);
                v[i + 2 * q] *= act_grad(f.x, ep.gate_mode);
                v[i + 2 * q + 1] *= act_grad(f.y, ep.gate_mode);
              }
            }
          } else {
#pragma unroll
            for (int i = 0; i < 32; ++i)
              if (col0 + i < N) v[i] *= act_grad(__bfloat162float(g[i]), ep.gate_mode);
          }
        }
        if (gate_vec && c != chalf * kChunks + kChunks - 1) gate_fetch(c + 1);
        if (kDgrad && ep.sumsq != nullptr && row_ok) {
#pragma unroll
          for (int i = 0; i < 32; ++i)
            if (full || col0 + i < N) sq = fmaf(v[i], v[i], sq);
        }
        if (kDgrad && ep.colsum != nullptr) {
          float wv[32];
#pragma unroll
          for (int i = 0; i < 32; ++i) wv[i] = row_ok ? v[i] : 0.0f;
#pragma unroll
          for (int half = 16; half >= 1; half >>= 1) {
            const bool upper = (lane & half) != 0;
#pragma unroll
            for (int i = 0; i < half; ++i) {
              const float mine = upper ? wv[i + half] : wv[i];
              const float send = upper ? wv[i] : wv[i + half];
              wv[i] = mine + __shfl_xor_sync(0xffffffffu, send, half);
            }
          }
          if (col0 + lane < N) atomicAdd(ep.colsum + col0 + lane, wv[0]);
        }
        if (kAccum && outf != nullptr && ep.accumulate) {
#pragma unroll
          for (int hr = 0; hr < 2; ++hr) {
            if ((lane >> 4) == hr) {
#pragma unroll
              for (int i = 0; i < 32; ++i) red_stage[(lane & 15) * 33 + i] = v[i];
            }
            __syncwarp();
            const int rbase = m0 + quarter * 32 + hr * 16;
            const int rows_here = min(16, M - rbase);
            if (col0 + lane < N) {
              float* p = outf + static_cast<long long>(rbase) * ep.ldf + col0 + lane;
              for (int rr = 0; rr < rows_here; ++rr) atomicAdd(p + static_cast<long long>(rr) * ep.ldf, red_stage[rr * 33 + lane]);
            }
            __syncwarp();
          }
        } else if (outf != nullptr && row_ok) {
          float* p = outf + static_cast<long long>(row) * ep.ldf + col0;
          if (full && (ep.ldf & 3) == 0 && (reinterpret_cast<uintptr_t>(outf) & 15u) == 0) {
#pragma unroll
            for (int i = 0; i < 32; i += 4) *reinterpret_cast<float4*>(p + i) = make_float4(v[i], v[i + 1], v[i + 2], v[i + 3]);
          } else {
#pragma unroll
            for (int i = 0; i < 32; ++i)
              if (col0 + i < N) p[i] = v[i];
          }
        }
        if (kBf16Out && ep.out != nullptr) {
          if (full && (ep.ldo & 7) == 0) {
            store_block_bf16(reinterpret_cast<uint4*>(red_stage), v,
                             reinterpret_cast<__nv_bfloat16*>(ep.out) + static_cast<long long>(m0 + quarter * 32) * ep.ldo + col0, ep.ldo,
                             M - (m0 + quarter * 32), lane);
          } else if (row_ok) {
            __nv_bfloat16* p = reinterpret_cast<__nv_bfloat16*>(ep.out) + static_cast<long long>(row) * ep.ldo + col0;
#pragma unroll
            for (int i = 0; i < 32; ++i)
              if (col0 + i < N) p[i] = __float2bfloat16(v[i]);
          }
        }
        if (kFwd && ep.out_t != nullptr && row_ok) {
#pragma unroll
          for (int i = 0; i < 32; ++i)
            if (col0 + i < N)
              reinterpret_cast<__nv_bfloat16*>(ep.out_t)[static_cast<long long>(col0 + i) * ep.ldot + row] = __float2bfloat16(v[i]);
        }
      }
      if (MODE == kModeWgrad && use_tma_red) {
        if (lane == 0) asm volatile("cp.async.bulk.wait_group.read 0;\n" ::: "memory");
        __syncwarp();
      }
      if (kDgrad && ep.sumsq != nullptr) {
#pragma unroll
        for (int o = 16; o > 0; o >>= 1) sq += __shfl_xor_sync(0xffffffffu, sq, o);
        if (lane == 0) atomicAdd(ep.sumsq, static_cast<double>(sq));
      }
      if (ew == 0 && lane == 0 && lw < 3) PULSE_TRACE(17 + 2 * lw);
    }
  }
  if (MODE == kModeWgrad && warp >= 4 && lane == 0) asm volatile("cp.async.bulk.wait_group 0;\n" ::: "memory");
  if (threadIdx.x == 0) PULSE_TRACE(10);
}


#undef PULSE_GEMM_FIRST
#undef PULSE_GEMM_W
#undef PULSE_GEMM_SELECT
```

pulse_b200/csrc/gemm_wgmma.cu:

```cuda
#include <cuda.h>
#include <stdlib.h>
#include <string.h>
#include <cuda_bf16.h>

#include "pulse_common.cuh"

namespace pulse {
namespace {

#ifndef PULSE_GEMM_VARIANT
#define PULSE_GEMM_VARIANT 0
#endif
constexpr int BM = 128, BN = 128, BK = 64, MMA_K = 16;
constexpr int kConsumerWarps = 8;
constexpr int kThreads = 128 + 32 * kConsumerWarps;
constexpr int kCols = 64;
constexpr int kChunks = kCols / 32;
constexpr int kStages = 4;
constexpr unsigned kStageBytesA = BM * BK * 2;
constexpr unsigned kStageBytesB = BN * BK * 2;

struct __align__(1024) GemmSmem {
  unsigned char a[kStages][kStageBytesA];
  unsigned char b[kStages][kStageBytesB];
  float acc[2][64 * BN];
  float red[kConsumerWarps][16 * 33];
  float bias[kConsumerWarps][kCols];
  unsigned long long full[kStages];
  unsigned long long empty[kStages];
};

__device__ __forceinline__ unsigned s_u32(const void* p) { return static_cast<unsigned>(__cvta_generic_to_shared(p)); }
__device__ __forceinline__ void g_mbar_init(unsigned long long* bar, unsigned count) {
  asm volatile("mbarrier.init.shared::cta.b64 [%0], %1;\n" ::"r"(s_u32(bar)), "r"(count));
}
__device__ __forceinline__ void g_mbar_expect_tx(unsigned long long* bar, unsigned bytes) {
  asm volatile("mbarrier.arrive.expect_tx.shared::cta.b64 _, [%0], %1;\n" ::"r"(s_u32(bar)), "r"(bytes) : "memory");
}
__device__ __forceinline__ void g_mbar_arrive(unsigned long long* bar) {
  asm volatile("mbarrier.arrive.shared::cta.b64 _, [%0];\n" ::"r"(s_u32(bar)) : "memory");
}
__device__ __forceinline__ bool g_mbar_try(unsigned long long* bar, unsigned parity) {
  unsigned ok;
  asm volatile(
      "{\n\t.reg .pred p;\n\t"
      "mbarrier.try_wait.parity.shared::cta.b64 p, [%1], %2;\n\t"
      "selp.u32 %0, 1, 0, p;\n\t}\n"
      : "=r"(ok)
      : "r"(s_u32(bar)), "r"(parity)
      : "memory");
  return ok != 0;
}
__device__ __forceinline__ void g_mbar_wait(unsigned long long* bar, unsigned parity) {
  for (int spin = 0; spin < (1 << 26); ++spin)
    if (g_mbar_try(bar, parity)) return;
  __trap();
}
__device__ __forceinline__ void tma_load_2d(void* smem_dst, const CUtensorMap* map, int c0, int c1, unsigned long long* bar) {
  asm volatile("cp.async.bulk.tensor.2d.shared::cluster.global.mbarrier::complete_tx::bytes [%0], [%1, {%3, %4}], [%2];\n" ::"r"(
                   s_u32(smem_dst)),
               "l"(map), "r"(s_u32(bar)), "r"(c0), "r"(c1)
               : "memory");
}
__device__ __forceinline__ void wg_sync(int wg) { asm volatile("bar.sync %0, 128;\n" ::"r"(1 + wg) : "memory"); }

__device__ __forceinline__ unsigned long long gmma_desc(unsigned smem_addr, unsigned lbo) {
  unsigned long long d = 0;
  d |= static_cast<unsigned long long>((smem_addr >> 4) & 0x3fffu);
  d |= static_cast<unsigned long long>((lbo >> 4) & 0x3fffu) << 16;
  d |= static_cast<unsigned long long>(1024u >> 4) << 32;
  d |= static_cast<unsigned long long>(1u) << 62;
  return d;
}
__device__ __forceinline__ void wgmma_fence() { asm volatile("wgmma.fence.sync.aligned;\n" ::: "memory"); }
__device__ __forceinline__ void wgmma_commit() { asm volatile("wgmma.commit_group.sync.aligned;\n" ::: "memory"); }
template <int N>
__device__ __forceinline__ void wgmma_wait() { asm volatile("wgmma.wait_group.sync.aligned %0;\n" ::"n"(N) : "memory"); }
__device__ __forceinline__ void acc_fence(float (&d)[64]) {
#pragma unroll
  for (int i = 0; i < 64; ++i) asm volatile("" : "+f"(d[i])::"memory");
}
template <int TA, int TB>
__device__ __forceinline__ void wgmma_m64n128(float (&d)[64], unsigned long long da, unsigned long long db, unsigned accumulate) {
  asm volatile(
      "{\n\t.reg .pred p;\n\t"
      "setp.ne.b32 p, %66, 0;\n\t"
      "wgmma.mma_async.sync.aligned.m64n128k16.f32.bf16.bf16 "
      "{%0, %1, %2, %3, %4, %5, %6, %7, %8, %9, %10, %11, %12, %13, %14, %15, %16, %17, %18, %19, %20, %21, %22, %23, %24, %25, %26, "
      "%27, %28, %29, %30, %31, %32, %33, %34, %35, %36, %37, %38, %39, %40, %41, %42, %43, %44, %45, %46, %47, %48, %49, %50, %51, "
      "%52, %53, %54, %55, %56, %57, %58, %59, %60, %61, %62, %63}, "
      "%64, %65, p, 1, 1, %67, %68;\n\t}\n"
      : "+f"(d[0]), "+f"(d[1]), "+f"(d[2]), "+f"(d[3]), "+f"(d[4]), "+f"(d[5]), "+f"(d[6]), "+f"(d[7]),
        "+f"(d[8]), "+f"(d[9]), "+f"(d[10]), "+f"(d[11]), "+f"(d[12]), "+f"(d[13]), "+f"(d[14]), "+f"(d[15]),
        "+f"(d[16]), "+f"(d[17]), "+f"(d[18]), "+f"(d[19]), "+f"(d[20]), "+f"(d[21]), "+f"(d[22]), "+f"(d[23]),
        "+f"(d[24]), "+f"(d[25]), "+f"(d[26]), "+f"(d[27]), "+f"(d[28]), "+f"(d[29]), "+f"(d[30]), "+f"(d[31]),
        "+f"(d[32]), "+f"(d[33]), "+f"(d[34]), "+f"(d[35]), "+f"(d[36]), "+f"(d[37]), "+f"(d[38]), "+f"(d[39]),
        "+f"(d[40]), "+f"(d[41]), "+f"(d[42]), "+f"(d[43]), "+f"(d[44]), "+f"(d[45]), "+f"(d[46]), "+f"(d[47]),
        "+f"(d[48]), "+f"(d[49]), "+f"(d[50]), "+f"(d[51]), "+f"(d[52]), "+f"(d[53]), "+f"(d[54]), "+f"(d[55]),
        "+f"(d[56]), "+f"(d[57]), "+f"(d[58]), "+f"(d[59]), "+f"(d[60]), "+f"(d[61]), "+f"(d[62]), "+f"(d[63])
      : "l"(da), "l"(db), "r"(accumulate), "n"(TA), "n"(TB)
      : "memory");
}

__device__ __forceinline__ float act_apply(float x, int act) {
  if (act == PULSE_ACT_RELU) return fmaxf(x, 0.0f);
  if (act == PULSE_ACT_SILU) return __fdividef(x, 1.0f + __expf(-x));
  return x;
}
__device__ __forceinline__ float act_grad(float g, int mode) {
  if (mode == PULSE_ACT_RELU) return g > 0.0f ? 1.0f : 0.0f;
  if (mode == PULSE_ACT_SILU) {
    const float s = __fdividef(1.0f, 1.0f + __expf(-g));
    return s * (1.0f + g * (1.0f - s));
  }
  return 1.0f;
}


__device__ __forceinline__ void store_block_bf16(uint4* st, const float (&v)[32], __nv_bfloat16* base, long long ld, int rows_valid, int lane) {
  const int sw = (lane >> 1) & 3;
#pragma unroll
  for (int q = 0; q < 4; ++q) {
    const int i = 8 * q;
    __nv_bfloat162 h0 = __floats2bfloat162_rn(v[i], v[i + 1]), h1 = __floats2bfloat162_rn(v[i + 2], v[i + 3]);
    __nv_bfloat162 h2 = __floats2bfloat162_rn(v[i + 4], v[i + 5]), h3 = __floats2bfloat162_rn(v[i + 6], v[i + 7]);
    uint4 u;
    u.x = *reinterpret_cast<unsigned*>(&h0);
    u.y = *reinterpret_cast<unsigned*>(&h1);
    u.z = *reinterpret_cast<unsigned*>(&h2);
    u.w = *reinterpret_cast<unsigned*>(&h3);
    st[lane * 4 + (q ^ sw)] = u;
  }
  __syncwarp();
  __nv_bfloat16* obase = base + (lane & 3) * 8;
#pragma unroll
  for (int it = 0; it < 4; ++it) {
    const int rr = it * 8 + (lane >> 2);
    const uint4 val = st[rr * 4 + ((lane & 3) ^ ((rr >> 1) & 3))];
    if (rr < rows_valid) *reinterpret_cast<uint4*>(obase + static_cast<long long>(rr) * ld) = val;
  }
  __syncwarp();
}

#if PULSE_GEMM_VARIANT == 3
__device__ long long g_gemm_trace[32];
#define PULSE_TRACE(slot)                                          \
  do {                                                             \
    if (blockIdx.x == 0) g_gemm_trace[slot] = clock64();           \
  } while (0)
#else
#define PULSE_TRACE(slot) \
  do {                    \
  } while (0)
#endif

__device__ __forceinline__ __nv_bfloat162 silu_bf16x2(__nv_bfloat162 z) {
  float2 f = __bfloat1622float2(z);
  f.x = __fdividef(f.x, 1.0f + __expf(-f.x));
  f.y = __fdividef(f.y, 1.0f + __expf(-f.y));
  return __floats2bfloat162_rn(f.x, f.y);
}

enum : int { kModeGeneric = 0, kModeFwd = 1, kModeDgrad = 2, kModeWgrad = 3, kModeDgradVec = 4 };

constexpr int kMaxGroup = 4;
struct GemmProblem {
  CUtensorMap map_a, map_b, map_c;
  pulse_gemm_epilogue_t ep;
  int M, N, K, kb_per_split;
  int item_end;
  int use_tma_red;
  int pad[2];
};
struct GemmGroup {
  GemmProblem p[kMaxGroup];
  int count, total_items;
};

#define PULSE_GEMM_GROUPED 0
#include "gemm_kernel.inc"
#undef PULSE_GEMM_GROUPED
#define PULSE_GEMM_GROUPED 1
#include "gemm_kernel.inc"
#undef PULSE_GEMM_GROUPED

typedef CUresult (*EncodeTiledFn)(CUtensorMap*, CUtensorMapDataType, cuuint32_t, void*, const cuuint64_t*, const cuuint64_t*,
                                  const cuuint32_t*, const cuuint32_t*, CUtensorMapInterleave, CUtensorMapSwizzle,
                                  CUtensorMapL2promotion, CUtensorMapFloatOOBfill);
EncodeTiledFn get_encode_fn() {
  static EncodeTiledFn fn = nullptr;
  if (fn == nullptr) {
    void* p = nullptr;
    cudaDriverEntryPointQueryResult q;
    if (cudaGetDriverEntryPoint("cuTensorMapEncodeTiled", &p, cudaEnableDefault, &q) == cudaSuccess && q == cudaDriverEntryPointSuccess)
      fn = reinterpret_cast<EncodeTiledFn>(p);
  }
  return fn;
}

bool make_map(CUtensorMap* map, const void* base, long long rows, long long cols, long long ld, unsigned box_rows) {
  EncodeTiledFn fn = get_encode_fn();
  if (fn == nullptr) return false;
  cuuint64_t dims[2] = {static_cast<cuuint64_t>(cols), static_cast<cuuint64_t>(rows)};
  cuuint64_t strides[1] = {static_cast<cuuint64_t>(ld) * 2};
  cuuint32_t box[2] = {BK, box_rows};
  cuuint32_t estr[2] = {1, 1};
  return fn(map, CU_TENSOR_MAP_DATA_TYPE_BFLOAT16, 2, const_cast<void*>(base), dims, strides, box, estr, CU_TENSOR_MAP_INTERLEAVE_NONE,
            CU_TENSOR_MAP_SWIZZLE_128B, CU_TENSOR_MAP_L2_PROMOTION_L2_256B, CU_TENSOR_MAP_FLOAT_OOB_FILL_NONE) == CUDA_SUCCESS;
}

bool make_map_c(CUtensorMap* map, const float* base, long long rows, long long cols, long long ld) {
  EncodeTiledFn fn = get_encode_fn();
  if (fn == nullptr) return false;
  cuuint64_t dims[2] = {static_cast<cuuint64_t>(cols), static_cast<cuuint64_t>(rows)};
  cuuint64_t strides[1] = {static_cast<cuuint64_t>(ld) * 4};
  cuuint32_t box[2] = {32, 32};
  cuuint32_t estr[2] = {1, 1};
  return fn(map, CU_TENSOR_MAP_DATA_TYPE_FLOAT32, 2, const_cast<float*>(base), dims, strides, box, estr, CU_TENSOR_MAP_INTERLEAVE_NONE,
            CU_TENSOR_MAP_SWIZZLE_128B, CU_TENSOR_MAP_L2_PROMOTION_NONE, CU_TENSOR_MAP_FLOAT_OOB_FILL_NONE) == CUDA_SUCCESS;
}
bool tma_reduce_ok(const pulse_gemm_epilogue_t& ep) {
  return ep.out_f32 != nullptr && ep.accumulate && (ep.ldf % 4) == 0 && (reinterpret_cast<uintptr_t>(ep.out_f32) % 16) == 0;
}

constexpr size_t kSmemBytes = sizeof(GemmSmem) + 1024;

int gemm_num_sms(bool honour_limit) {
  static int num_sms = 0, limited = 0;
  if (num_sms == 0) {
    int dev = 0;
    if (cudaGetDevice(&dev) != cudaSuccess || cudaDeviceGetAttribute(&num_sms, cudaDevAttrMultiProcessorCount, dev) != cudaSuccess) return 0;
    limited = num_sms;
    const char* e = getenv("PULSE_GEMM_SMS");
    if (e != nullptr && atoi(e) >= 1 && atoi(e) < num_sms) limited = atoi(e);
  }
  return honour_limit ? limited : num_sms;
}

template <bool A_MN, bool B_MN, int MODE>
int launch_gemm(const CUtensorMap& map_a, const CUtensorMap& map_b, const pulse_gemm_epilogue_t& ep, int m, int n, int k, int splits,
                int kb_per_split, cudaStream_t stream) {
  static bool attr_set = false;
  CUtensorMap map_c;
  memset(&map_c, 0, sizeof(map_c));
  int use_tma_red = 0;
  if (MODE == kModeWgrad && tma_reduce_ok(ep)) {
    if (!make_map_c(&map_c, ep.out_f32, m, n, ep.ldf)) {
      set_error("pulse_gemm_bf16: cuTensorMapEncodeTiled failed for the fp32 output");
      return PULSE_ERR_CUDA;
    }
    use_tma_red = 1;
  }
  if (!attr_set) {
    PULSE_CUDA_OK(cudaFuncSetAttribute(gemm_bf16_kernel<A_MN, B_MN, MODE>, cudaFuncAttributeMaxDynamicSharedMemorySize, (int)kSmemBytes));
    attr_set = true;
  }
  const int num_sms = gemm_num_sms(true);
  PULSE_REQUIRE(num_sms > 0, "pulse_gemm_bf16: cannot query the device's SM count");
  const long long total = static_cast<long long>((n + BN - 1) / BN) * ((m + BM - 1) / BM) * splits;
  const unsigned grid = static_cast<unsigned>(total < num_sms ? total : num_sms);
  static int use_pdl = -1;
  if (use_pdl < 0) {
    const char* e = getenv("PULSE_GEMM_PDL");
    use_pdl = (e != nullptr && e[0] == '0') ? 0 : 1;
  }
  cudaLaunchConfig_t cfg = {};
  cfg.gridDim = dim3(grid, 1, 1);
  cfg.blockDim = dim3(kThreads, 1, 1);
  cfg.dynamicSmemBytes = kSmemBytes;
  cfg.stream = stream;
  cudaLaunchAttribute attr[1];
  int na = 0;
  if (use_pdl) {
    attr[na].id = cudaLaunchAttributeProgrammaticStreamSerialization;
    attr[na].val.programmaticStreamSerializationAllowed = 1;
    ++na;
  }
  cfg.attrs = attr;
  cfg.numAttrs = na;
  PULSE_CUDA_OK(cudaLaunchKernelEx(&cfg, gemm_bf16_kernel<A_MN, B_MN, MODE>, map_a, map_b, map_c, ep, m, n, k, kb_per_split, splits, use_tma_red));
  PULSE_LAUNCH_OK("gemm_bf16_kernel");
  return PULSE_OK;
}

template <bool A_MN, bool B_MN, int MODE>
int launch_gemm_grouped(const GemmGroup& grp, cudaStream_t stream) {
  static bool attr_set = false;
  if (!attr_set) {
    PULSE_CUDA_OK(cudaFuncSetAttribute(gemm_bf16_grouped_kernel<A_MN, B_MN, MODE>, cudaFuncAttributeMaxDynamicSharedMemorySize, (int)kSmemBytes));
    attr_set = true;
  }
  const int num_sms = gemm_num_sms(false);
  PULSE_REQUIRE(num_sms > 0, "pulse_gemm_bf16_grouped: cannot query the device's SM count");
  const unsigned grid = static_cast<unsigned>(grp.total_items < num_sms ? grp.total_items : num_sms);
  cudaLaunchConfig_t cfg = {};
  cfg.gridDim = dim3(grid, 1, 1);
  cfg.blockDim = dim3(kThreads, 1, 1);
  cfg.dynamicSmemBytes = kSmemBytes;
  cfg.stream = stream;
  cudaLaunchAttribute attr[1];
  attr[0].id = cudaLaunchAttributeProgrammaticStreamSerialization;
  attr[0].val.programmaticStreamSerializationAllowed = 1;
  cfg.attrs = attr;
  cfg.numAttrs = 1;
  PULSE_CUDA_OK(cudaLaunchKernelEx(&cfg, gemm_bf16_grouped_kernel<A_MN, B_MN, MODE>, grp));
  PULSE_LAUNCH_OK("gemm_bf16_grouped_kernel");
  return PULSE_OK;
}

int epilogue_mode(const pulse_gemm_epilogue_t* ep) {
  const bool want_fwd = ep->bias || ep->act != PULSE_ACT_NONE || ep->preact || ep->out_t || ep->relu_mask;
  const bool want_dgrad = ep->gate || ep->colsum || ep->sumsq || ep->gate_mask;
  const bool want_accum = ep->accumulate != 0;
  if (!want_dgrad && !want_accum) return kModeFwd;
  if (!want_fwd && !want_accum) return (ep->gate && ep->gate_mode != PULSE_ACT_RELU) ? kModeDgradVec : kModeDgrad;
  if (!want_fwd && !want_dgrad && !ep->out) return kModeWgrad;
  return kModeGeneric;
}

}
}

#if PULSE_GEMM_VARIANT == 3
extern "C" int pulse_debug_gemm_trace(long long* out) {
  return cudaMemcpyFromSymbol(out, pulse::g_gemm_trace, sizeof(long long) * 32) == cudaSuccess ? 0 : -2;
}
#endif

extern "C" int pulse_gemm_num_splits(int64_t k, int32_t split_k) {
  const int num_kb = static_cast<int>((k + 63) / 64);
  int splits = split_k < 1 ? 1 : (split_k > num_kb ? num_kb : split_k);
  const int kb_per_split = (num_kb + splits - 1) / splits;
  return (num_kb + kb_per_split - 1) / kb_per_split;
}

extern "C" int pulse_gemm_bf16(const void* a, int64_t lda, const void* b, int64_t ldb, int64_t m, int64_t n, int64_t k,
                               const pulse_gemm_epilogue_t* ep, int32_t split_k, uint32_t flags, void* stream) {
  using namespace pulse;
  PULSE_REQUIRE(a && b && ep, "pulse_gemm_bf16: null argument");
  PULSE_REQUIRE(m > 0 && n > 0 && k > 0, "pulse_gemm_bf16: empty problem %lld x %lld x %lld", (long long)m, (long long)n, (long long)k);
  PULSE_REQUIRE(m < (1ll << 31) && n < (1ll << 31) && k < (1ll << 31), "pulse_gemm_bf16: dimension too large");
  PULSE_REQUIRE((flags & ~3u) == 0, "pulse_gemm_bf16: bad flags");
  const bool a_mn = flags & PULSE_GEMM_A_MN, b_mn = flags & PULSE_GEMM_B_MN;
  PULSE_REQUIRE(lda >= (a_mn ? m : k) && ldb >= (b_mn ? n : k) && (lda % 8) == 0 && (ldb % 8) == 0,
                "pulse_gemm_bf16: leading dimensions must cover the contiguous extent and be multiples of 8 (16-byte rows), got %lld %lld",
                (long long)lda, (long long)ldb);
  PULSE_REQUIRE(aligned16(a) && aligned16(b), "pulse_gemm_bf16: operands must be 16-byte aligned");
  PULSE_REQUIRE(ep->out || ep->out_t || ep->out_f32, "pulse_gemm_bf16: no output requested");
  PULSE_REQUIRE(split_k >= 1, "pulse_gemm_bf16: split_k must be >= 1");
  PULSE_REQUIRE(split_k == 1 || (ep->out_f32 && !ep->out && !ep->out_t && !ep->bias && ep->act == PULSE_ACT_NONE && !ep->gate && !ep->preact && !ep->colsum),
                "pulse_gemm_bf16: split-K only supports plain fp32 outputs (slabs or atomic accumulation)");
  PULSE_REQUIRE(ep->gate == nullptr || ep->gate_mode == PULSE_ACT_RELU || ep->gate_mode == PULSE_ACT_SILU, "pulse_gemm_bf16: bad gate_mode");
  PULSE_REQUIRE((ep->relu_mask == nullptr || ep->ld_rmask >= m) && (ep->gate_mask == nullptr || ep->ld_gmask >= m),
                "pulse_gemm_bf16: mask word rows must hold at least M entries");
  PULSE_REQUIRE(!(ep->gate_mask && ep->gate), "pulse_gemm_bf16: give the ReLU gate either as bf16 activations or as bit words, not both");
  CUtensorMap map_a, map_b;
  const bool ok_a = a_mn ? make_map(&map_a, a, k, m, lda, 64) : make_map(&map_a, a, m, k, lda, BM);
  const bool ok_b = b_mn ? make_map(&map_b, b, k, n, ldb, 64) : make_map(&map_b, b, n, k, ldb, BN);
  if (!ok_a || !ok_b) {
    set_error("pulse_gemm_bf16: cuTensorMapEncodeTiled failed (driver entry point missing or bad strides)");
    return PULSE_ERR_CUDA;
  }
  const int num_kb = static_cast<int>((k + BK - 1) / BK);
  const int splits = pulse_gemm_num_splits(k, split_k);
  const int kb_per_split = (num_kb + splits - 1) / splits;
  cudaStream_t st = static_cast<cudaStream_t>(stream);
  const int mode = epilogue_mode(ep);
  const int mi = (int)m, ni = (int)n, ki = (int)k;
#define PULSE_GEMM_DISPATCH(AM, BM_)                                                                                        \
  switch (mode) {                                                                                                           \
    case kModeFwd: return launch_gemm<AM, BM_, kModeFwd>(map_a, map_b, *ep, mi, ni, ki, splits, kb_per_split, st);             \
    case kModeDgrad: return launch_gemm<AM, BM_, kModeDgrad>(map_a, map_b, *ep, mi, ni, ki, splits, kb_per_split, st);         \
    case kModeWgrad: return launch_gemm<AM, BM_, kModeWgrad>(map_a, map_b, *ep, mi, ni, ki, splits, kb_per_split, st);         \
    case kModeDgradVec: return launch_gemm<AM, BM_, kModeDgradVec>(map_a, map_b, *ep, mi, ni, ki, splits, kb_per_split, st);   \
    default: return launch_gemm<AM, BM_, kModeGeneric>(map_a, map_b, *ep, mi, ni, ki, splits, kb_per_split, st);               \
  }
  if (a_mn && b_mn) { PULSE_GEMM_DISPATCH(true, true) }
  if (a_mn) { PULSE_GEMM_DISPATCH(true, false) }
  if (b_mn) { PULSE_GEMM_DISPATCH(false, true) }
  PULSE_GEMM_DISPATCH(false, false)
#undef PULSE_GEMM_DISPATCH
}

extern "C" int pulse_gemm_bf16_nt(const void* a, int64_t lda, const void* b, int64_t ldb, int64_t m, int64_t n, int64_t k,
                                  const pulse_gemm_epilogue_t* ep, int32_t split_k, void* stream) {
  return pulse_gemm_bf16(a, lda, b, ldb, m, n, k, ep, split_k, 0u, stream);
}

extern "C" int pulse_gemm_bf16_grouped(const pulse_gemm_problem_t* problems, int32_t count, uint32_t flags, void* stream) {
  using namespace pulse;
  PULSE_REQUIRE(problems != nullptr && count >= 1 && count <= kMaxGroup, "pulse_gemm_bf16_grouped: 1..%d problems", kMaxGroup);
  PULSE_REQUIRE((flags & ~3u) == 0, "pulse_gemm_bf16_grouped: bad flags");
  const bool a_mn = flags & PULSE_GEMM_A_MN, b_mn = flags & PULSE_GEMM_B_MN;
  int mode = -1;
  for (int i = 0; i < count; ++i) {
    const pulse_gemm_problem_t& q = problems[i];
    PULSE_REQUIRE(q.a && q.b, "pulse_gemm_bf16_grouped: null operand in problem %d", i);
    PULSE_REQUIRE(q.m > 0 && q.n > 0 && q.k > 0 && q.m < (1ll << 31) && q.n < (1ll << 31) && q.k < (1ll << 31), "pulse_gemm_bf16_grouped: bad shape in problem %d", i);
    PULSE_REQUIRE(q.lda >= (a_mn ? q.m : q.k) && q.ldb >= (b_mn ? q.n : q.k) && (q.lda % 8) == 0 && (q.ldb % 8) == 0,
                  "pulse_gemm_bf16_grouped: leading dimensions of problem %d must cover the contiguous extent and be multiples of 8", i);
    PULSE_REQUIRE(aligned16(q.a) && aligned16(q.b), "pulse_gemm_bf16_grouped: operands of problem %d must be 16-byte aligned", i);
    PULSE_REQUIRE(q.ep.out || q.ep.out_t || q.ep.out_f32, "pulse_gemm_bf16_grouped: problem %d has no output", i);
    PULSE_REQUIRE(q.split_k >= 1, "pulse_gemm_bf16_grouped: split_k must be >= 1");
    PULSE_REQUIRE(q.split_k == 1 || (q.ep.out_f32 && q.ep.accumulate && !q.ep.out && !q.ep.out_t && !q.ep.bias && q.ep.act == PULSE_ACT_NONE && !q.ep.gate &&
                                     !q.ep.preact && !q.ep.colsum),
                  "pulse_gemm_bf16_grouped: split-K only with fp32 atomic accumulation");
    const int mq = epilogue_mode(&q.ep);
    PULSE_REQUIRE(mode < 0 || mq == mode, "pulse_gemm_bf16_grouped: problem %d needs a different epilogue specialisation than problem 0", i);
    mode = mq;
  }
  PULSE_REQUIRE(mode == kModeFwd || mode == kModeDgrad || mode == kModeWgrad, "pulse_gemm_bf16_grouped: forward, ReLU-dgrad and wgrad groups only");
  PULSE_REQUIRE((mode == kModeFwd && !a_mn && !b_mn) || (mode == kModeDgrad && !a_mn && b_mn) || (mode == kModeWgrad && a_mn && b_mn),
                "pulse_gemm_bf16_grouped: operand majors do not match the group kind (fwd K/K, dgrad K/MN, wgrad MN/MN)");
  GemmGroup grp;
  memset(&grp, 0, sizeof(grp));
  grp.count = count;
  long long items = 0;
  for (int i = 0; i < count; ++i) {
    const pulse_gemm_problem_t& q = problems[i];
    GemmProblem& g = grp.p[i];
    const bool ok_a = a_mn ? make_map(&g.map_a, q.a, q.k, q.m, q.lda, 64) : make_map(&g.map_a, q.a, q.m, q.k, q.lda, BM);
    const bool ok_b = b_mn ? make_map(&g.map_b, q.b, q.k, q.n, q.ldb, 64) : make_map(&g.map_b, q.b, q.n, q.k, q.ldb, BN);
    if (!ok_a || !ok_b) {
      set_error("pulse_gemm_bf16_grouped: cuTensorMapEncodeTiled failed for problem %d", i);
      return PULSE_ERR_CUDA;
    }
    g.ep = q.ep;
    g.use_tma_red = 0;
    if (mode == kModeWgrad && tma_reduce_ok(q.ep)) {
      if (!make_map_c(&g.map_c, q.ep.out_f32, q.m, q.n, q.ep.ldf)) {
        set_error("pulse_gemm_bf16_grouped: cuTensorMapEncodeTiled failed for the fp32 output of problem %d", i);
        return PULSE_ERR_CUDA;
      }
      g.use_tma_red = 1;
    }
    g.M = static_cast<int>(q.m);
    g.N = static_cast<int>(q.n);
    g.K = static_cast<int>(q.k);
    const int num_kb = static_cast<int>((q.k + BK - 1) / BK);
    const int splits = pulse_gemm_num_splits(q.k, q.split_k);
    g.kb_per_split = (num_kb + splits - 1) / splits;
    items += static_cast<long long>((q.n + BN - 1) / BN) * ((q.m + BM - 1) / BM) * splits;
    PULSE_REQUIRE(items < (1ll << 30), "pulse_gemm_bf16_grouped: too many work items");
    g.item_end = static_cast<int>(items);
  }
  grp.total_items = static_cast<int>(items);
  cudaStream_t st = static_cast<cudaStream_t>(stream);
  if (mode == kModeFwd) return launch_gemm_grouped<false, false, kModeFwd>(grp, st);
  if (mode == kModeDgrad) return launch_gemm_grouped<false, true, kModeDgrad>(grp, st);
  return launch_gemm_grouped<true, true, kModeWgrad>(grp, st);
}
```

pulse_b200/dense.py:

```python
import ctypes as C
from typing import Optional

import torch

from . import _lib

ACT = {"none": _lib.ACT_NONE, None: _lib.ACT_NONE, "relu": _lib.ACT_RELU, "silu": _lib.ACT_SILU}


def _check_bf16(t, name):
    if t.dtype != torch.bfloat16 or t.dim() != 2 or t.stride(1) != 1:
        raise _lib.PulseError(f"{name} must be a 2-D bf16 tensor with contiguous rows, got {t.dtype} {tuple(t.shape)} {t.stride()}")


def num_splits(k: int, split_k: int) -> int:
    return int(_lib.load().pulse_gemm_num_splits(k, split_k))


def ordered_sum_add(x: torch.Tensor, out: torch.Tensor) -> None:
    if x.dtype != torch.float32 or out.dtype != torch.float32 or x.stride(-1) != 1 or out.stride(-1) != 1 or x.shape[1:] != out.shape:
        raise _lib.PulseError("ordered_sum_add: fp32 x [n, rows, cols] and out [rows, cols] with contiguous columns")
    with torch.cuda.device(x.device):
        _lib.check(_lib.load().pulse_ordered_sum_add(x.data_ptr(), x.shape[0], x.stride(0), x.shape[1], x.shape[2], x.stride(1), out.data_ptr(),
                                                     out.stride(0), _lib.current_stream(x.device)), "pulse_ordered_sum_add")


def column_sum_add(y: torch.Tensor, out: torch.Tensor, chunk: int = 64) -> None:
    rows, cols = y.shape
    n = -(-rows // chunk)
    part = torch.zeros(n, cols, device=y.device)
    full = rows // chunk
    if full:
        ordered_sum_add(y[:full * chunk].as_strided((chunk, full, cols), (y.stride(0), chunk * y.stride(0), 1)), part[:full])
    if rows > full * chunk:
        ordered_sum_add(y[full * chunk:].unsqueeze(1), part[full:])
    ordered_sum_add(part.unsqueeze(1), out.view(1, -1)[:, :cols])


def gemm_nt(a, b, **kw) -> None:
    gemm(a, b, **kw)


def gemm(a: torch.Tensor, b: torch.Tensor, *, a_mn: bool = False, b_mn: bool = False, bias: Optional[torch.Tensor] = None, act=None,
         gate: Optional[torch.Tensor] = None, gate_mode=None, alpha: float = 1.0, out: Optional[torch.Tensor] = None,
         out_t: Optional[torch.Tensor] = None, out_f32: Optional[torch.Tensor] = None, preact: Optional[torch.Tensor] = None,
         colsum: Optional[torch.Tensor] = None, accumulate: bool = False, split_k: int = 1, sumsq: Optional[torch.Tensor] = None,
         relu_mask: Optional[torch.Tensor] = None, gate_mask: Optional[torch.Tensor] = None) -> None:
    lib = _lib.load()
    _check_bf16(a, "a")
    _check_bf16(b, "b")
    (K, M) = a.shape if a_mn else (a.shape[1], a.shape[0])
    if accumulate and out_f32 is not None and out_f32.dim() == 2 and split_k > 1 and num_splits(K, split_k) > 1:
        if (bias, gate, gate_mode, out, out_t, preact, colsum, sumsq, relu_mask, gate_mask) != (None,) * 10 or act not in (None, "none") \
                or alpha != 1.0:
            raise _lib.PulseError("split-K accumulation takes a plain fp32 output only (no alpha, activation, gate or extra outputs)")
        N = b.shape[1] if b_mn else b.shape[0]
        slabs = torch.empty(num_splits(K, split_k), M, (N + 3) // 4 * 4, device=a.device)[:, :, :N]
        gemm(a, b, a_mn=a_mn, b_mn=b_mn, out_f32=slabs, split_k=split_k)
        if out_f32.stride(-1) != 1:
            raise _lib.PulseError("out_f32 must be fp32 with contiguous rows")
        ordered_sum_add(slabs, out_f32[:M, :N])
        return
    (Kb, N) = b.shape if b_mn else (b.shape[1], b.shape[0])
    if K != Kb:
        raise _lib.PulseError(f"K mismatch: a {tuple(a.shape)} (mn={a_mn}) vs b {tuple(b.shape)} (mn={b_mn})")
    ep = _lib.GemmEpilogue()
    ep.alpha = alpha
    ep.act = ACT[act] if not isinstance(act, int) else act
    if bias is not None:
        if bias.dtype != torch.float32 or bias.numel() != N or not bias.is_contiguous():
            raise _lib.PulseError("bias must be contiguous fp32 [N]")
        ep.bias = bias.data_ptr()
    if gate is not None:
        _check_bf16(gate, "gate")
        ep.gate, ep.ldg = gate.data_ptr(), gate.stride(0)
        ep.gate_mode = ACT[gate_mode] if not isinstance(gate_mode, int) else gate_mode
    if out is not None:
        _check_bf16(out, "out")
        if out.shape[0] < M or out.shape[1] < N:
            raise _lib.PulseError("out too small")
        ep.out, ep.ldo = out.data_ptr(), out.stride(0)
    if out_t is not None:
        _check_bf16(out_t, "out_t")
        if out_t.shape[0] < N or out_t.shape[1] < M:
            raise _lib.PulseError("out_t too small")
        ep.out_t, ep.ldot = out_t.data_ptr(), out_t.stride(0)
    if preact is not None:
        _check_bf16(preact, "preact")
        ep.preact, ep.ldp = preact.data_ptr(), preact.stride(0)
    if out_f32 is not None:
        if out_f32.dtype != torch.float32 or out_f32.stride(-1) != 1:
            raise _lib.PulseError("out_f32 must be fp32 with contiguous rows")
        if out_f32.dim() == 3:
            if out_f32.shape[0] < num_splits(K, split_k):
                raise _lib.PulseError("out_f32 has fewer slabs than split-K needs")
            ep.split_stride, ep.ldf = out_f32.stride(0), out_f32.stride(1)
        else:
            if split_k != 1 and not accumulate:
                raise _lib.PulseError("split_k > 1 needs a [splits, M, N] out_f32 or accumulate=True")
            ep.ldf = out_f32.stride(0)
        ep.out_f32 = out_f32.data_ptr()
        ep.accumulate = int(accumulate)
    if colsum is not None:
        if colsum.dtype != torch.float32 or colsum.numel() < N:
            raise _lib.PulseError("colsum must be fp32 [N]")
        ep.colsum = colsum.data_ptr()
    if sumsq is not None:
        if sumsq.dtype != torch.float64 or sumsq.numel() < 1:
            raise _lib.PulseError("sumsq must be an fp64 accumulator")
        ep.sumsq = sumsq.data_ptr()
    for name, t in (("relu_mask", relu_mask), ("gate_mask", gate_mask)):
        if t is not None:
            if t.dtype != torch.int32 or t.dim() != 2 or t.stride(1) != 1 or t.shape[0] * 32 < N or t.shape[1] < M:
                raise _lib.PulseError(f"{name} must be int32 [ceil(N/32), >= M] with contiguous rows, got {t.dtype} {tuple(t.shape)}")
            if name == "relu_mask":
                ep.relu_mask, ep.ld_rmask = t.data_ptr(), t.stride(0)
            else:
                ep.gate_mask, ep.ld_gmask = t.data_ptr(), t.stride(0)
    flags = (_lib.GEMM_A_MN if a_mn else 0) | (_lib.GEMM_B_MN if b_mn else 0)
    with torch.cuda.device(a.device):
        _lib.check(lib.pulse_gemm_bf16(a.data_ptr(), a.stride(0), b.data_ptr(), b.stride(0), M, N, K, C.byref(ep), split_k, flags,
                                       _lib.current_stream(a.device)), "pulse_gemm_bf16")


def _prepare(a: torch.Tensor, b: torch.Tensor, *, a_mn: bool = False, b_mn: bool = False, bias: Optional[torch.Tensor] = None, act=None,
         gate: Optional[torch.Tensor] = None, gate_mode=None, alpha: float = 1.0, out: Optional[torch.Tensor] = None,
         out_t: Optional[torch.Tensor] = None, out_f32: Optional[torch.Tensor] = None, preact: Optional[torch.Tensor] = None,
         colsum: Optional[torch.Tensor] = None, accumulate: bool = False, split_k: int = 1, sumsq: Optional[torch.Tensor] = None,
         relu_mask: Optional[torch.Tensor] = None, gate_mask: Optional[torch.Tensor] = None) -> tuple:
    _check_bf16(a, "a")
    _check_bf16(b, "b")
    (K, M) = a.shape if a_mn else (a.shape[1], a.shape[0])
    (Kb, N) = b.shape if b_mn else (b.shape[1], b.shape[0])
    if K != Kb:
        raise _lib.PulseError(f"K mismatch: a {tuple(a.shape)} (mn={a_mn}) vs b {tuple(b.shape)} (mn={b_mn})")
    ep = _lib.GemmEpilogue()
    ep.alpha = alpha
    ep.act = ACT[act] if not isinstance(act, int) else act
    if bias is not None:
        if bias.dtype != torch.float32 or bias.numel() != N or not bias.is_contiguous():
            raise _lib.PulseError("bias must be contiguous fp32 [N]")
        ep.bias = bias.data_ptr()
    if gate is not None:
        _check_bf16(gate, "gate")
        ep.gate, ep.ldg = gate.data_ptr(), gate.stride(0)
        ep.gate_mode = ACT[gate_mode] if not isinstance(gate_mode, int) else gate_mode
    if out is not None:
        _check_bf16(out, "out")
        if out.shape[0] < M or out.shape[1] < N:
            raise _lib.PulseError("out too small")
        ep.out, ep.ldo = out.data_ptr(), out.stride(0)
    if out_t is not None:
        _check_bf16(out_t, "out_t")
        if out_t.shape[0] < N or out_t.shape[1] < M:
            raise _lib.PulseError("out_t too small")
        ep.out_t, ep.ldot = out_t.data_ptr(), out_t.stride(0)
    if preact is not None:
        _check_bf16(preact, "preact")
        ep.preact, ep.ldp = preact.data_ptr(), preact.stride(0)
    if out_f32 is not None:
        if out_f32.dtype != torch.float32 or out_f32.stride(-1) != 1:
            raise _lib.PulseError("out_f32 must be fp32 with contiguous rows")
        if out_f32.dim() == 3:
            if out_f32.shape[0] < num_splits(K, split_k):
                raise _lib.PulseError("out_f32 has fewer slabs than split-K needs")
            ep.split_stride, ep.ldf = out_f32.stride(0), out_f32.stride(1)
        else:
            if split_k != 1 and not accumulate:
                raise _lib.PulseError("split_k > 1 needs a [splits, M, N] out_f32 or accumulate=True")
            ep.ldf = out_f32.stride(0)
        ep.out_f32 = out_f32.data_ptr()
        ep.accumulate = int(accumulate)
    if colsum is not None:
        if colsum.dtype != torch.float32 or colsum.numel() < N:
            raise _lib.PulseError("colsum must be fp32 [N]")
        ep.colsum = colsum.data_ptr()
    if sumsq is not None:
        if sumsq.dtype != torch.float64 or sumsq.numel() < 1:
            raise _lib.PulseError("sumsq must be an fp64 accumulator")
        ep.sumsq = sumsq.data_ptr()
    for name, t in (("relu_mask", relu_mask), ("gate_mask", gate_mask)):
        if t is not None:
            if t.dtype != torch.int32 or t.dim() != 2 or t.stride(1) != 1 or t.shape[0] * 32 < N or t.shape[1] < M:
                raise _lib.PulseError(f"{name} must be int32 [ceil(N/32), >= M] with contiguous rows, got {t.dtype} {tuple(t.shape)}")
            if name == "relu_mask":
                ep.relu_mask, ep.ld_rmask = t.data_ptr(), t.stride(0)
            else:
                ep.gate_mask, ep.ld_gmask = t.data_ptr(), t.stride(0)
    flags = (_lib.GEMM_A_MN if a_mn else 0) | (_lib.GEMM_B_MN if b_mn else 0)
    return ep, M, N, K, flags, split_k


def grouped_enabled() -> bool:
    import os
    return os.environ.get("PULSE_GROUPED", "0") == "1"


def gemm_grouped(problems) -> None:
    lib = _lib.load()
    if not 1 <= len(problems) <= 4:
        raise _lib.PulseError("gemm_grouped takes 1..4 problems")
    arr = (_lib.GemmProblem * len(problems))()
    flags0 = None
    for i, (a, b, kw) in enumerate(problems):
        ep, M, N, K, flags, split_k = _prepare(a, b, **kw)
        if flags0 is None:
            flags0 = flags
        elif flags != flags0:
            raise _lib.PulseError("gemm_grouped: all problems must share the operand majors")
        arr[i].a, arr[i].lda, arr[i].b, arr[i].ldb = a.data_ptr(), a.stride(0), b.data_ptr(), b.stride(0)
        arr[i].m, arr[i].n, arr[i].k, arr[i].ep, arr[i].split_k = M, N, K, ep, split_k
    dev = problems[0][0].device
    with torch.cuda.device(dev):
        _lib.check(lib.pulse_gemm_bf16_grouped(arr, len(problems), flags0, _lib.current_stream(dev)), "pulse_gemm_bf16_grouped")
```

pulse_b200/nets.py:

```python
import ctypes as C
import math
import os
import warnings
from typing import Dict, List, Optional, Sequence

import torch

from . import _lib
from .dense import gemm, gemm_nt


def pad8(n: int) -> int:
    return (n + 7) // 8 * 8


def pad_k(n: int) -> int:
    return pad8(n) if n <= 64 else (n + 63) // 64 * 64


def pick_split(tiles: int, num_kb: int, sms: int = 132, epilogue_kb: int = 24) -> int:
    best, best_cost = 1, None
    for s in range(1, min(64, num_kb) + 1):
        per = -(-num_kb // s)
        if -(-num_kb // per) != s:
            continue
        rounds = -(-(tiles * s) // sms)
        cost = rounds * (per + epilogue_kb)
        if best_cost is None or cost < best_cost:
            best, best_cost = s, cost
    return best


class FlatParams:

    def __init__(self, device):
        self.device = device
        self._shapes: List[tuple] = []
        self._numel = 0
        self.params = self.grads = self.exp_avg = self.exp_avg_sq = None
        self.step = None
        self.sumsq = None

    def reserve(self, *shape) -> int:
        off = self._numel
        n = 1
        for s in shape:
            n *= s
        self._numel += (n + 63) // 64 * 64
        self._shapes.append((off, tuple(shape)))
        return len(self._shapes) - 1

    def finalize(self, peer: Optional[bool] = None):
        z = lambda: torch.zeros(self._numel, device=self.device, dtype=torch.float32)
        self.peer = None
        if peer is None:
            peer = os.environ.get("PULSE_PEER_ADAM", "1") != "0"
        if peer and torch.device(self.device).type == "cuda":
            try:
                self._alloc_peer()
            except Exception as e:
                warnings.warn(f"pulse_b200: peer-memory optimizer unavailable ({type(e).__name__}: {e}); using the NCCL all-reduce path")
                self.peer = None
        if self.peer is None:
            self.params, self.grads = z(), z()
            self.params_bf16 = torch.zeros(self._numel, device=self.device, dtype=torch.bfloat16)
        self.exp_avg, self.exp_avg_sq = z(), z()
        self.sumsq = torch.zeros(1, device=self.device, dtype=torch.float64)
        self.step = torch.zeros(1, device=self.device, dtype=torch.int32)
        self._adam_sync = torch.zeros(1, device=self.device, dtype=torch.int32)
        self.clean = True

    def _alloc_peer(self):
        import torch.distributed as dist
        if not (dist.is_available() and dist.is_initialized()) or dist.get_world_size() <= 1 or dist.get_backend() != "nccl":
            return
        world, rank = dist.get_world_size(), dist.get_rank()
        if world > _lib.PEER_MAX:
            return
        import torch.distributed._symmetric_memory as symm
        group = dist.group.WORLD
        try:
            symm.enable_symm_mem_for_group(group.group_name)
        except Exception:
            pass

        def alloc(n, dtype):
            t = symm.empty(n, dtype=dtype, device=self.device)
            t.zero_()
            return t, symm.rendezvous(t, group)

        grads, hg = alloc(self._numel, torch.float32)
        params, hp = alloc(self._numel, torch.float32)
        pbf16, hb = alloc(self._numel, torch.bfloat16)
        sig, hs = alloc(256, torch.uint8)
        torch.cuda.synchronize(self.device)
        dist.barrier()
        a = _lib.PeerAdamArgs(rank=rank, world=world, count=self._numel)
        for p in range(world):
            a.grads[p], a.params[p], a.params_bf16[p], a.signals[p] = int(hg.buffer_ptrs[p]), int(hp.buffer_ptrs[p]), int(hb.buffer_ptrs[p]), int(hs.buffer_ptrs[p])
        if int(a.grads[rank]) != grads.data_ptr() or int(a.params[rank]) != params.data_ptr():
            raise RuntimeError("symmetric-memory handle does not describe the local tensors")
        mc_env = os.environ.get("PULSE_PEER_MC", "auto")
        use_mc = mc_env == "1" or (mc_env == "auto" and world >= 8)
        mc = [int(getattr(h, "multicast_ptr", 0) or 0) for h in (hg, hp, hb)]
        if use_mc and all(mc):
            a.mc_grads, a.mc_params, a.mc_params_bf16 = mc
        self.grads, self.params, self.params_bf16 = grads, params, pbf16
        dev = self.device
        scratch = dict(epoch=torch.zeros(1, dtype=torch.int32, device=dev), partials=torch.zeros(_lib.PEER_MAX_GRID, dtype=torch.float64, device=dev),
                       bar=torch.zeros(1, dtype=torch.int64, device=dev))
        a.epoch, a.cta_partials, a.grid_bar = scratch["epoch"].data_ptr(), scratch["partials"].data_ptr(), scratch["bar"].data_ptr()
        a.grid = int(os.environ.get("PULSE_PEER_GRID", "0"))
        a.timeout_ms = int(os.environ.get("PULSE_PEER_TIMEOUT_MS", "0"))
        self.peer = dict(args=a, handles=(hg, hp, hb, hs), signals=sig, scratch=scratch, world=world, rank=rank, multicast=bool(a.mc_grads))

    def shard_span(self):
        if self.peer is None:
            return 0, self._numel
        w, r, n4 = self.peer["world"], self.peer["rank"], self._numel // 4
        per = (n4 + w - 1) // w
        s0 = min(per * r, n4)
        return 4 * s0, 4 * min(s0 + per, n4)

    def peer_adam_step(self, lr: float, max_norm: float = 0.0, betas=(0.9, 0.999), eps: float = 1e-8):
        a = self.peer["args"]
        a.exp_avg, a.exp_avg_sq, a.step = self.exp_avg.data_ptr(), self.exp_avg_sq.data_ptr(), self.step.data_ptr()
        a.max_norm, a.lr, a.beta1, a.beta2, a.eps = float(max_norm or 0.0), float(lr), float(betas[0]), float(betas[1]), float(eps)
        with torch.cuda.device(self.device):
            _lib.check(_lib.load().pulse_peer_reduce_adam(C.byref(a), _lib.current_stream(self.device)), "pulse_peer_reduce_adam")
        self.clean = True

    def gather_moments(self):
        if self.peer is None:
            return
        import torch.distributed as dist
        s0, s1 = self.shard_span()
        for buf in (self.exp_avg, self.exp_avg_sq):
            tmp = torch.zeros_like(buf)
            tmp[s0:s1] = buf[s0:s1]
            dist.all_reduce(tmp)
            buf.copy_(tmp)

    def sync_bf16(self):
        self.params_bf16.copy_(self.params)

    def view(self, idx: int, what: str = "params") -> torch.Tensor:
        off, shape = self._shapes[idx]
        n = 1
        for s in shape:
            n *= s
        return getattr(self, what)[off:off + n].view(*shape)

    def view_padded(self, idx: int, what: str, n: int) -> torch.Tensor:
        off, _ = self._shapes[idx]
        return getattr(self, what)[off:off + n]

    @property
    def numel(self):
        return self._numel

    def slot_span(self, first_idx: int, last_idx: int):
        start = self._shapes[first_idx][0]
        end = self._shapes[last_idx + 1][0] if last_idx + 1 < len(self._shapes) else self._numel
        return start, end

    def zero_grad(self):
        self.grads.zero_()
        self.clean = True

    def begin_backward(self):
        if not self.clean:
            self.grads.zero_()
        self.clean = False

    def adam_step(self, lr: float, max_norm: float = 0.0, betas=(0.9, 0.999), eps: float = 1e-8, zero_grads: bool = True):
        lib = _lib.load()
        with torch.cuda.device(self.device):
            st = _lib.current_stream(self.device)
            sumsq_ptr = None
            if max_norm and max_norm > 0:
                _lib.check(lib.pulse_sum_squares(self.grads.data_ptr(), self._numel, self.sumsq.data_ptr(), st), "pulse_sum_squares")
                sumsq_ptr = self.sumsq.data_ptr()
            _lib.check(lib.pulse_adam_step(self.params.data_ptr(), self.grads.data_ptr(), self.exp_avg.data_ptr(), self.exp_avg_sq.data_ptr(),
                                           self._numel, sumsq_ptr, float(max_norm or 0.0), lr, betas[0], betas[1], eps, self.step.data_ptr(),
                                           self.params_bf16.data_ptr(), 3 if zero_grads else 2, self._adam_sync.data_ptr(), st),
                       "pulse_adam_step")
        self.clean = bool(zero_grads)


class Dense:

    def __init__(self, flat: FlatParams, in_features: int, out_features: int, act: Optional[str], aug: bool = False):
        self.K, self.N, self.act, self.aug = in_features, out_features, act, aug
        self.Kp = pad_k(in_features + 1) if aug else pad_k(in_features)
        self.Np = pad_k(out_features + 1) if aug else pad_k(out_features)
        self.flat = flat
        self.w_idx = flat.reserve(out_features, self.Kp)
        self.b_idx = None if aug else flat.reserve(out_features)

    @property
    def weight(self):
        return self.flat.view(self.w_idx)

    @property
    def bias(self):
        return self.weight[:, self.K] if self.aug else self.flat.view(self.b_idx)

    @property
    def w_bf16(self):
        return self.flat.view(self.w_idx, "params_bf16")

    @property
    def weight_grad(self):
        return self.flat.view(self.w_idx, "grads")

    @property
    def bias_grad(self):
        return self.weight_grad[:, self.K] if self.aug else self.flat.view(self.b_idx, "grads")

    @property
    def pad_start(self):
        return self.K + (1 if self.aug else 0)

    def init_default(self, gen: Optional[torch.Generator] = None):
        bound = 1.0 / math.sqrt(self.K)
        w = (torch.rand(self.N, self.K, device=self.flat.device, generator=gen) * 2 - 1) * bound
        b = (torch.rand(self.N, device=self.flat.device, generator=gen) * 2 - 1) * bound
        self.set_weights(w, b)

    def set_weights(self, w: torch.Tensor, b: torch.Tensor):
        self.weight.zero_()
        self.weight[:, :self.K].copy_(w)
        self.bias.copy_(b)
        self.refresh()

    def refresh(self):
        self.w_bf16.copy_(self.weight)


class MLP:

    def __init__(self, flat: FlatParams, in_features: int, units: Sequence[int], head: Optional[int], act: str = "relu",
                 hidden_acts: Optional[Sequence[Optional[str]]] = None, input_grad_cols: int = 0, in_perm: Optional[torch.Tensor] = None,
                 aug: bool = False):
        self.flat = flat
        self.act = act
        self.aug = aug
        sizes = [in_features] + list(units)
        acts = list(hidden_acts) if hidden_acts is not None else [act] * len(units)
        if len(acts) != len(units):
            raise _lib.PulseError("hidden_acts must have one entry per hidden layer")
        self.layers: List[Dense] = [Dense(flat, sizes[i], sizes[i + 1], acts[i], aug) for i in range(len(units))]
        if head is not None:
            self.layers.append(Dense(flat, sizes[-1], head, None, aug))
        self.in_features, self.Kp0 = in_features, self.layers[0].Kp
        self.input_grad_cols = input_grad_cols
        self.in_perm = in_perm
        self._ws: Dict[int, dict] = {}
        self._scratch = None
        self._zero = None

    def param_span(self):
        idx = [i for l in self.layers for i in (l.w_idx, l.b_idx) if i is not None]
        return self.flat.slot_span(min(idx), max(idx))

    def _zero_bias(self) -> torch.Tensor:
        if self._zero is None:
            self._zero = torch.zeros(8, device=self.flat.device)
        return self._zero

    def init_default(self, gen=None):
        for l in self.layers:
            l.init_default(gen)

    def refresh(self):
        for l in self.layers:
            l.refresh()

    def _workspace(self, M: int, train: bool, slot: int = 0):
        key = (M, train) if slot == 0 else (M, train, slot)
        if key not in self._ws:
            dev = self.flat.device
            bf = lambda r, c: torch.zeros(r, c, device=dev, dtype=torch.bfloat16)
            ws = {"act": [], "pre": [], "dact": [], "split": [], "mask": []}
            for i, l in enumerate(self.layers):
                last = i == len(self.layers) - 1
                a = None if last else bf(M, l.Np)
                if a is not None and self.aug:
                    a[:, l.N] = 1.0
                ws["act"].append(a)
                if train:
                    ws["pre"].append(bf(M, l.Np) if (l.act == "silu") else None)
                    ws["dact"].append(None if last else bf(M, l.Np))
                    ws["mask"].append(torch.zeros((l.N + 31) // 32, M, device=dev, dtype=torch.int32) if (l.act == "relu" and not last) else None)
                    tiles = ((l.N + 127) // 128) * ((l.Kp + 127) // 128)
                    ws["split"].append(pick_split(tiles, (M + 63) // 64))
            hn = self.layers[-1].N
            ws["out"] = torch.zeros(M, (hn + 3) // 4 * 4, device=dev)[:, :hn]
            if train and self.input_grad_cols:
                ws["dx"] = torch.zeros(M, self.input_grad_cols, device=dev)
            self._ws[key] = ws
        return self._ws[key]

    def _dummy(self, n: int) -> torch.Tensor:
        if self._scratch is None or self._scratch.numel() < n:
            self._scratch = torch.zeros(max(n, 8), device=self.flat.device)
        return self._scratch

    def _head1(self, i: int) -> bool:
        l = self.layers[i]
        return i == len(self.layers) - 1 and i > 0 and l.N == 1 and self.layers[i - 1].act == "relu" and l.Kp <= 2048

    def _fwd_problem(self, i: int, h: torch.Tensor, ws: dict, train: bool):
        l = self.layers[i]
        kw = dict(bias=None if self.aug else l.bias, act=l.act, out=ws["act"][i], preact=ws["pre"][i] if train else None)
        if train and ws["mask"][i] is not None:
            kw["relu_mask"] = ws["mask"][i]
        return h[:, :l.Kp], l.w_bf16, kw

    def _wgrad_problem(self, i: int, dy: torch.Tensor, x_in: torch.Tensor, ws: dict):
        l = self.layers[i]
        return dy[:, :l.N], x_in[:, :l.Kp], dict(a_mn=True, b_mn=True, out_f32=l.weight_grad, accumulate=True, split_k=ws["split"][i])

    def _dgrad_problem(self, i: int, dy: torch.Tensor, ws: dict):
        l, prev = self.layers[i], self.layers[i - 1]
        kw = dict(b_mn=True, out=ws["dact"][i - 1])
        if prev.act == "relu" and ws["mask"][i - 1] is not None:
            kw["gate_mask"] = ws["mask"][i - 1]
        elif prev.act is not None:
            kw.update(gate=ws["pre"][i - 1] if prev.act == "silu" else ws["act"][i - 1], gate_mode=prev.act)
        if not self.aug:
            kw["colsum"] = self.flat.view_padded(prev.b_idx, "grads", prev.Np)
        w = l.w_bf16[:, :prev.N] if self.aug else l.w_bf16
        return dy[:, :l.N], w, kw

    def forward(self, x: torch.Tensor, train: bool = False, out: Optional[torch.Tensor] = None, slot: int = 0) -> torch.Tensor:
        M = x.shape[0]
        ws = self._workspace(M, train, slot)
        if out is not None:
            ws = dict(ws, out=out)
        h = x
        for i, l in enumerate(self.layers):
            last = i == len(self.layers) - 1
            if last and self._head1(i):
                bias = self._zero_bias() if self.aug else l.bias
                with torch.cuda.device(self.flat.device):
                    _lib.check(_lib.load().pulse_head1_forward(h.data_ptr(), h.stride(0), M, l.Kp, l.w_bf16.data_ptr(), bias.data_ptr(),
                                                               ws["out"].data_ptr(), ws["out"].stride(0),
                                                               _lib.current_stream(self.flat.device)), "pulse_head1_forward")
            elif last:
                gemm_nt(h[:, :l.Kp], l.w_bf16, bias=None if self.aug else l.bias, act=None, out_f32=ws["out"])
            else:
                a, b, kw = self._fwd_problem(i, h, ws, train)
                gemm_nt(a, b, **kw)
                h = ws["act"][i]
        if train:
            self._ws[(M, True)]["x"] = x
        return ws["out"]

    def _backward_head(self, ws: dict, dout: torch.Tensor, M: int):
        lib = _lib.load()
        dev = self.flat.device
        head = self.layers[-1]
        top = len(self.layers) - 1
        if self._head1(top):
            prev, h, dh = self.layers[top - 1], ws["act"][top - 1], ws["dact"][top - 1]
            if self.aug:
                hb, pb = self._dummy(prev.Np + 8), self._dummy(prev.Np + 8)[8:]
            else:
                hb, pb = head.bias_grad, self.flat.view_padded(prev.b_idx, "grads", prev.Np)
            with torch.cuda.device(dev):
                if "head1_partials" not in ws:
                    ws["head1_partials"] = torch.empty(_lib.HEAD1_MAX_CTAS * (2 * head.Kp + 1), device=dev)
                _lib.check(lib.pulse_head1_backward(h.data_ptr(), h.stride(0), M, head.Kp, dout.data_ptr(), dout.stride(0), head.w_bf16.data_ptr(),
                                                    dh.data_ptr(), dh.stride(0), head.weight_grad.data_ptr(), hb.data_ptr(), pb.data_ptr(),
                                                    ws["head1_partials"].data_ptr(), _lib.current_stream(dev)), "pulse_head1_backward")
            return dh, top - 1
        if not self.aug:
            with torch.cuda.device(dev):
                _lib.check(lib.pulse_column_sum_bf16(dout.data_ptr(), dout.stride(0), M, head.N, head.bias_grad.data_ptr(), _lib.current_stream(dev)),
                           "pulse_column_sum_bf16")
        return dout, top

    def backward(self, dout: torch.Tensor, M: int) -> None:
        ws = self._ws[(M, True)]
        dy, top = self._backward_head(ws, dout, M)
        for i in reversed(range(top + 1)):
            l = self.layers[i]
            x_in = ws["x"] if i == 0 else ws["act"][i - 1]
            a, b, kw = self._wgrad_problem(i, dy, x_in, ws)
            gemm(a, b, **kw)
            if i > 0:
                a, b, kw = self._dgrad_problem(i, dy, ws)
                gemm(a, b, **kw)
                dy = ws["dact"][i - 1]
            elif self.input_grad_cols:
                gemm(dy[:, :l.N], l.w_bf16[:, :self.input_grad_cols], b_mn=True, out_f32=ws["dx"])

    def state_dict(self, prefix: str, head_name: Optional[str] = None) -> Dict[str, torch.Tensor]:
        out = {}
        hidden = self.layers[:-1] if head_name is not None else self.layers
        for i, l in enumerate(hidden):
            w = l.weight[:, :l.K].clone()
            if i == 0 and self.in_perm is not None:
                w_ref = torch.empty_like(w)
                w_ref[:, self.in_perm.to(w.device)] = w
                w = w_ref
            out[f"{prefix}.{2 * i}.weight"] = w
            out[f"{prefix}.{2 * i}.bias"] = l.bias.clone()
        if head_name is not None:
            l = self.layers[-1]
            out[f"{head_name}.weight"] = l.weight[:, :l.K].clone()
            out[f"{head_name}.bias"] = l.bias.clone()
        return out

    def load_state_dict(self, sd: Dict[str, torch.Tensor], prefix: str, head_name: Optional[str] = None):
        hidden = self.layers[:-1] if head_name is not None else self.layers
        for i, l in enumerate(hidden):
            w = sd[f"{prefix}.{2 * i}.weight"].to(self.flat.device)
            if i == 0 and self.in_perm is not None:
                w = w[:, self.in_perm.to(w.device)]
            l.set_weights(w, sd[f"{prefix}.{2 * i}.bias"].to(self.flat.device))
        if head_name is not None:
            l = self.layers[-1]
            l.set_weights(sd[f"{head_name}.weight"].to(self.flat.device), sd[f"{head_name}.bias"].to(self.flat.device))


def normalize_to_bf16(x: torch.Tensor, mean: Optional[torch.Tensor], rstd: Optional[torch.Tensor], out: torch.Tensor,
                      out_t: Optional[torch.Tensor] = None, pad_one: float = 0.0) -> None:
    lib = _lib.load()
    rows, cols = x.shape
    if x.dtype != torch.float32 or x.stride(1) != 1:
        raise _lib.PulseError("normalize_to_bf16: x must be fp32 with contiguous rows")
    with torch.cuda.device(x.device):
        _lib.check(lib.pulse_normalize_to_bf16(x.data_ptr(), x.stride(0), rows, cols, _lib.ptr(mean), _lib.ptr(rstd), out.data_ptr(), out.stride(0),
                                               _lib.ptr(out_t), out_t.stride(0) if out_t is not None else 0, float(pad_one),
                                               _lib.current_stream(x.device)),
                   "pulse_normalize_to_bf16")


def forward_lockstep(mlps: Sequence["MLP"], xs: Sequence[torch.Tensor], train: bool = False) -> List[torch.Tensor]:
    from .dense import gemm_grouped
    depth = len(mlps[0].layers)
    if any(len(m.layers) != depth for m in mlps) or any(x.shape[0] != xs[0].shape[0] for x in xs):
        raise _lib.PulseError("forward_lockstep needs nets of the same depth on batches of the same size")
    M = xs[0].shape[0]
    wss = [m._workspace(M, train) for m in mlps]
    hs = list(xs)
    for i in range(depth - 1):
        gemm_grouped([m._fwd_problem(i, h, ws, train) for m, ws, h in zip(mlps, wss, hs)])
        hs = [ws["act"][i] for ws in wss]
    outs = []
    for m, ws, h, x in zip(mlps, wss, hs, xs):
        i = depth - 1
        l = m.layers[i]
        if m._head1(i):
            bias = m._zero_bias() if m.aug else l.bias
            with torch.cuda.device(m.flat.device):
                _lib.check(_lib.load().pulse_head1_forward(h.data_ptr(), h.stride(0), M, l.Kp, l.w_bf16.data_ptr(), bias.data_ptr(),
                                                           ws["out"].data_ptr(), ws["out"].stride(0), _lib.current_stream(m.flat.device)),
                           "pulse_head1_forward")
        else:
            gemm_nt(h[:, :l.Kp], l.w_bf16, bias=None if m.aug else l.bias, act=None, out_f32=ws["out"])
        if train:
            m._ws[(M, True)]["x"] = x
        outs.append(ws["out"])
    return outs


def backward_lockstep(mlps: Sequence["MLP"], douts: Sequence[torch.Tensor], M: int) -> None:
    from .dense import gemm_grouped
    depth = len(mlps[0].layers)
    wss = [m._ws[(M, True)] for m in mlps]
    dys, tops = [], []
    for m, ws, dy in zip(mlps, wss, douts):
        dy, top = m._backward_head(ws, dy, M)
        dys.append(dy)
        tops.append(top)
    for i in reversed(range(depth)):
        live = [j for j in range(len(mlps)) if tops[j] >= i]
        if not live:
            continue
        wg, dg = [], []
        for j in live:
            m, ws, dy = mlps[j], wss[j], dys[j]
            x_in = ws["x"] if i == 0 else ws["act"][i - 1]
            wg.append(m._wgrad_problem(i, dy, x_in, ws))
            if i > 0:
                if m.layers[i - 1].act != "relu":
                    raise _lib.PulseError("backward_lockstep groups ReLU nets only (the grouped dgrad kernel is the ReLU-gate specialisation)")
                dg.append(m._dgrad_problem(i, dy, ws))
        gemm_grouped(wg)
        if dg:
            gemm_grouped(dg)
            for j in live:
                dys[j] = wss[j]["dact"][i - 1]
```

Baseline: 1.440 million.

## Add 256-wide N tile to bf16 GEMM with tile-aware split-K selection

Templates the Hopper wgmma GEMM kernel on tile width BN and adds a 256-column variant. It uses setmaxnreg to move registers from producer to consumer warps and runs the epilogue in multiple passes through shared memory. A new host-side heuristic picks the tile width and split-K count together from M, N, K and the SM count, replacing the Python pick_split. The goal is better operand reuse and fewer waves on large GEMMs. The cost is higher register pressure, fewer pipeline stages at BN=256, and more template instantiations.

```diff
diff --git a/include/pulse_b200.h b/include/pulse_b200.h
--- a/include/pulse_b200.h
+++ b/include/pulse_b200.h
@@ -248,6 +248,8 @@
 int pulse_gemm_bf16(const void* a, int64_t lda, const void* b, int64_t ldb, int64_t m, int64_t n, int64_t k,
                     const pulse_gemm_epilogue_t* ep, int32_t split_k, uint32_t flags, void* stream);
 int pulse_gemm_num_splits(int64_t k, int32_t split_k);
+int pulse_gemm_split_k(int64_t m, int64_t n, int64_t k);
+int pulse_gemm_tile_n(int64_t m, int64_t n, int64_t k, int32_t split_k);
 
 typedef struct {
   const void* a; int64_t lda;
diff --git a/pulse_b200/_lib.py b/pulse_b200/_lib.py
--- a/pulse_b200/_lib.py
+++ b/pulse_b200/_lib.py
@@ -292,6 +292,8 @@
     "pulse_gemm_bf16": (C.c_int, [C.c_void_p, C.c_int64, C.c_void_p, C.c_int64, C.c_int64, C.c_int64, C.c_int64,
                                   C.POINTER(GemmEpilogue), C.c_int32, C.c_uint32, C.c_void_p]),
     "pulse_gemm_num_splits": (C.c_int, [C.c_int64, C.c_int32]),
+    "pulse_gemm_split_k": (C.c_int, [C.c_int64, C.c_int64, C.c_int64]),
+    "pulse_gemm_tile_n": (C.c_int, [C.c_int64, C.c_int64, C.c_int64, C.c_int32]),
     "pulse_gemm_bf16_grouped": (C.c_int, [C.POINTER(GemmProblem), C.c_int32, C.c_uint32, C.c_void_p]),
     "pulse_normalize_to_bf16": (C.c_int, [C.c_void_p, C.c_int64, C.c_int64, C.c_int64, C.c_void_p, C.c_void_p, C.c_void_p, C.c_int64,
                                           C.c_void_p, C.c_int64, C.c_float, C.c_void_p]),
diff --git a/pulse_b200/amp.py b/pulse_b200/amp.py
--- a/pulse_b200/amp.py
+++ b/pulse_b200/amp.py
@@ -5,7 +5,8 @@
 
 from . import _lib
 from .dense import column_sum_add, gemm
-from .nets import MLP, FlatParams, pad_k, pick_split
+from .dense import split_k
+from .nets import MLP, FlatParams, pad_k
 from .ppo import RunningMeanStdB200
 
 
@@ -38,14 +39,15 @@
         if B not in self._bufs:
             dev, bf = self.device, torch.bfloat16
             L1, L2, _ = self.mlp.layers
+            with torch.cuda.device(dev):
+                split1, split2 = split_k(L1.N, L1.Kp, B), split_k(L2.N, L2.Kp, B)
             self._bufs[B] = {
                 "x": torch.zeros(2, 3 * B, self.Kp, device=dev, dtype=bf),
                 "dlogit": torch.zeros(3 * B, 8, device=dev, dtype=bf),
                 "g2": torch.zeros(B, L2.Np, device=dev, dtype=bf), "g1": torch.zeros(B, L1.Np, device=dev, dtype=bf),
                 "Gb": torch.zeros(B, self.Kp, device=dev, dtype=bf),
                 "du": torch.zeros(B, L1.Np, device=dev, dtype=bf), "scratch": torch.zeros(B, L2.Np, device=dev),
-                "split1": pick_split(((L1.N + 127) // 128) * ((L1.Kp + 127) // 128), (B + 63) // 64),
-                "split2": pick_split(((L2.N + 127) // 128) * ((L2.Kp + 127) // 128), (B + 63) // 64),
+                "split1": split1, "split2": split2,
             }
         return self._bufs[B]
 
diff --git a/pulse_b200/csrc/gemm_kernel.inc b/pulse_b200/csrc/gemm_kernel.inc
--- a/pulse_b200/csrc/gemm_kernel.inc
+++ b/pulse_b200/csrc/gemm_kernel.inc
@@ -23,10 +23,10 @@
 #endif
 
 #if PULSE_GEMM_GROUPED
-template <bool A_MN, bool B_MN, int MODE>
+template <bool A_MN, bool B_MN, int MODE, int BN>
 __global__ void __launch_bounds__(kThreads, 1) gemm_bf16_grouped_kernel(const __grid_constant__ GemmGroup grp) {
 #else
-template <bool A_MN, bool B_MN, int MODE>
+template <bool A_MN, bool B_MN, int MODE, int BN>
 __global__ void __launch_bounds__(kThreads, 1) gemm_bf16_kernel(const __grid_constant__ CUtensorMap map_a,
                                                                 const __grid_constant__ CUtensorMap map_b,
                                                                 const __grid_constant__ CUtensorMap map_c,
@@ -38,8 +38,13 @@
   constexpr bool kGateVec = MODE == kModeGeneric || MODE == kModeDgradVec;
   constexpr bool kAccum = MODE == kModeGeneric || MODE == kModeWgrad;
   constexpr bool kBf16Out = MODE != kModeWgrad;
+  constexpr int kStg = kStages<BN>, kSW = kStageCols<BN>;
+  constexpr int kPass = BN / kSW;
+  constexpr int kCh = kSW / 64;
+  constexpr int kWC = BN / 64;
+  constexpr unsigned kStageBytesB = BN * BK * 2;
   extern __shared__ unsigned char gsm_raw[];
-  GemmSmem& sm = *reinterpret_cast<GemmSmem*>((reinterpret_cast<uintptr_t>(gsm_raw) + 1023) & ~static_cast<uintptr_t>(1023));
+  GemmSmem<BN>& sm = *reinterpret_cast<GemmSmem<BN>*>((reinterpret_cast<uintptr_t>(gsm_raw) + 1023) & ~static_cast<uintptr_t>(1023));
   const int warp = threadIdx.x >> 5, lane = threadIdx.x & 31;
   const int work0 = static_cast<int>(blockIdx.x);
   const int work_stride = static_cast<int>(gridDim.x);
@@ -55,7 +60,7 @@
 
   if (threadIdx.x == 0) {
 #pragma unroll
-    for (int s = 0; s < kStages; ++s) {
+    for (int s = 0; s < kStg; ++s) {
       g_mbar_init(&sm.full[s], 1);
       g_mbar_init(&sm.empty[s], kConsumerWarps);
     }
@@ -68,6 +73,7 @@
   asm volatile("griddepcontrol.launch_dependents;\n" ::: "memory");
 
   if (warp < 4) {
+    if constexpr (BN == 256) asm volatile("setmaxnreg.dec.sync.aligned.u32 24;\n" ::: "memory");
     if (warp == 0 && lane == 0) {
       asm volatile("griddepcontrol.wait;\n" ::: "memory");
       PULSE_TRACE(2);
@@ -79,8 +85,8 @@
         const int kb0 = split * kb_per_split;
         const int num_kb = min(kb_per_split, num_kb_total - kb0);
         for (int kb = 0; kb < num_kb; ++kb, ++it) {
-          const int s = it % kStages;
-          g_mbar_wait(&sm.empty[s], ((it / kStages) & 1) ^ 1);
+          const int s = it % kStg;
+          g_mbar_wait(&sm.empty[s], ((it / kStg) & 1) ^ 1);
           g_mbar_expect_tx(&sm.full[s], kStageBytesA + kStageBytesB);
           const int kk = (kb0 + kb) * BK;
           if (A_MN) {
@@ -90,8 +96,8 @@
             tma_load_2d(sm.a[s], &map_a, kk, m0, &sm.full[s]);
           }
           if (B_MN) {
-            tma_load_2d(sm.b[s], &map_b, n0, kk, &sm.full[s]);
-            tma_load_2d(sm.b[s] + 8192, &map_b, n0 + 64, kk, &sm.full[s]);
+#pragma unroll
+            for (int j = 0; j < BN / 64; ++j) tma_load_2d(sm.b[s] + 8192 * j, &map_b, n0 + 64 * j, kk, &sm.full[s]);
           } else {
             tma_load_2d(sm.b[s], &map_b, kk, n0, &sm.full[s]);
           }
@@ -99,6 +105,7 @@
       }
     }
   } else {
+    if constexpr (BN == 256) asm volatile("setmaxnreg.inc.sync.aligned.u32 240;\n" ::: "memory");
     const int wg = (warp >> 2) - 1;
     const int ew = warp - 4;
     const int quarter = wg * 2 + (warp & 1);
@@ -115,24 +122,26 @@
       const int num_kb = min(kb_per_split, num_kb_total - kb0);
       const int row = m0 + quarter * 32 + lane;
       const bool row_ok = row < M;
-      const bool gate_fast = (MODE == kModeGeneric || MODE == kModeDgrad) && ep.gate != nullptr && ep.gate_mask == nullptr && ep.gate_mode == PULSE_ACT_RELU && (ep.ldg & 7) == 0 && n0 + chalf * kCols + kCols <= N;
-      unsigned gmask[kChunks] = {};
+      auto chunk_of = [&](int wc) { return (wc / kCh) * (kSW / 32) + chalf * kCh + wc % kCh; };
+      auto group_full = [&](int wc) { return n0 + ((chunk_of(wc) * 32) & ~63) + 64 <= N; };
+      const bool gate_fast = (MODE == kModeGeneric || MODE == kModeDgrad) && ep.gate != nullptr && ep.gate_mask == nullptr && ep.gate_mode == PULSE_ACT_RELU && (ep.ldg & 7) == 0;
+      unsigned gmask[kWC] = {};
       const bool gate_bits = kDgrad && ep.gate_mask != nullptr;
       if (gate_bits && row_ok) {
 #pragma unroll
-        for (int cc = 0; cc < kChunks; ++cc) {
-          const int col = n0 + (chalf * kChunks + cc) * 32;
-          if (col < N) gmask[cc] = __ldg(ep.gate_mask + static_cast<long long>(col >> 5) * ep.ld_gmask + row);
+        for (int wc = 0; wc < kWC; ++wc) {
+          const int col = n0 + chunk_of(wc) * 32;
+          if (col < N) gmask[wc] = __ldg(ep.gate_mask + static_cast<long long>(col >> 5) * ep.ld_gmask + row);
         }
       }
       if (gate_fast && row_ok) {
-        const uint4* g = reinterpret_cast<const uint4*>(reinterpret_cast<const __nv_bfloat16*>(ep.gate) + static_cast<long long>(row) * ep.ldg +
-                                                        n0 + chalf * kCols);
-        uint4 u[kChunks * 4];
-#pragma unroll
-        for (int i = 0; i < kChunks * 4; ++i) u[i] = __ldg(g + i);
-#pragma unroll
-        for (int i = 0; i < kChunks * 4; ++i) {
+        const uint4* g = reinterpret_cast<const uint4*>(reinterpret_cast<const __nv_bfloat16*>(ep.gate) + static_cast<long long>(row) * ep.ldg + n0);
+        uint4 u[kWC * 4] = {};
+#pragma unroll
+        for (int i = 0; i < kWC * 4; ++i)
+          if (group_full(i >> 2)) u[i] = __ldg(g + chunk_of(i >> 2) * 4 + (i & 3));
+#pragma unroll
+        for (int i = 0; i < kWC * 4; ++i) {
           const unsigned wds[4] = {u[i].x, u[i].y, u[i].z, u[i].w};
 #pragma unroll
           for (int q = 0; q < 4; ++q) {
@@ -151,32 +160,28 @@
           for (int q = 0; q < 4; ++q) gq[q] = __ldg(g + q);
         }
       };
-      gate_fetch(chalf * kChunks);
-      float bias_l[kChunks] = {};
+      gate_fetch(chunk_of(0));
       const bool fwd_fast = MODE == kModeFwd && ep.out != nullptr && (ep.ldo & 7) == 0 && ep.out_f32 == nullptr && ep.out_t == nullptr &&
-                            (ep.preact == nullptr || (ep.ldp & 7) == 0) && n0 + chalf * kCols + kCols <= N;
+                            (ep.preact == nullptr || (ep.ldp & 7) == 0);
       float* bias_s = sm.bias[ew];
-      if (fwd_fast && ep.bias != nullptr) {
+      if (kFwd && ep.bias != nullptr) {
         __syncwarp();
 #pragma unroll
-        for (int cc = 0; cc < kChunks; ++cc) bias_s[cc * 32 + lane] = __ldg(ep.bias + n0 + (chalf * kChunks + cc) * 32 + lane);
+        for (int wc = 0; wc < kWC; ++wc) {
+          const int col = n0 + chunk_of(wc) * 32 + lane;
+          bias_s[wc * 32 + lane] = col < N ? __ldg(ep.bias + col) : 0.0f;
+        }
         __syncwarp();
-      } else if (kFwd && ep.bias != nullptr) {
-#pragma unroll
-        for (int cc = 0; cc < kChunks; ++cc) {
-          const int col = n0 + (chalf * kChunks + cc) * 32 + lane;
-          if (col < N) bias_l[cc] = __ldg(ep.bias + col);
-        }
-      }
-
-      float d[64];
-#pragma unroll
-      for (int i = 0; i < 64; ++i) d[i] = 0.0f;
+      }
+
+      float d[BN / 2];
+#pragma unroll
+      for (int i = 0; i < BN / 2; ++i) d[i] = 0.0f;
       acc_fence(d);
       int prev_s = -1;
       for (int kb = 0; kb < num_kb; ++kb, ++it) {
-        const int s = it % kStages;
-        g_mbar_wait(&sm.full[s], (it / kStages) & 1);
+        const int s = it % kStg;
+        g_mbar_wait(&sm.full[s], (it / kStg) & 1);
         if (it == 0 && ew == 0 && lane == 0) PULSE_TRACE(3);
         wgmma_fence();
         const unsigned a_addr = s_u32(sm.a[s]) + static_cast<unsigned>(wg) * 8192u, b_addr = s_u32(sm.b[s]);
@@ -184,7 +189,7 @@
         for (int k = 0; k < BK / MMA_K; ++k) {
           const unsigned long long da = A_MN ? gmma_desc(a_addr + k * 2048, 8192) : gmma_desc(a_addr + k * 32, 16);
           const unsigned long long db = B_MN ? gmma_desc(b_addr + k * 2048, 8192) : gmma_desc(b_addr + k * 32, 16);
-          wgmma_m64n128<A_MN ? 1 : 0, B_MN ? 1 : 0>(d, da, db, (kb | k) != 0 ? 1u : 0u);
+          wgmma_step<BN, A_MN ? 1 : 0, B_MN ? 1 : 0>(d, da, db, (kb | k) != 0 ? 1u : 0u);
         }
         wgmma_commit();
         wgmma_wait<1>();
@@ -196,235 +201,246 @@
       if (lane == 0) g_mbar_arrive(&sm.empty[prev_s]);
       if (ew == 0 && lane == 0 && lw < 3) PULSE_TRACE(4 + lw);
 
-      wg_sync(wg);
-      {
-        const int r0 = (warp & 3) * 16 + (lane >> 2);
-#pragma unroll
-        for (int j = 0; j < BN / 8; ++j) {
-          const int col = 8 * j + 2 * (lane & 3);
-#pragma unroll
-          for (int h = 0; h < 2; ++h) {
-            const int r = r0 + 8 * h;
-            const int rb = r & 31;
-            float* blk = acc_s + ((r >> 5) * 4 + (col >> 5)) * 1024;
-            const int unit = ((col & 31) >> 2) ^ (rb & 7);
-            *reinterpret_cast<float2*>(blk + rb * 32 + unit * 4 + (col & 3)) = make_float2(d[4 * j + 2 * h], d[4 * j + 2 * h + 1]);
-          }
-        }
-      }
-      if (MODE == kModeWgrad && use_tma_red) asm volatile("fence.proxy.async.shared::cta;\n" ::: "memory");
-      wg_sync(wg);
-      if (ew == 0 && lane == 0 && lw < 3) PULSE_TRACE(16 + 2 * lw);
-
       float* outf = ep.out_f32 != nullptr ? ep.out_f32 + static_cast<long long>(ep.accumulate ? 0 : split) * ep.split_stride : nullptr;
       float sq = 0.0f;
+#pragma unroll
+      for (int p = 0; p < kPass; ++p) {
+        if (MODE == kModeWgrad && use_tma_red && p > 0) {
+          if (lane == 0) asm volatile("cp.async.bulk.wait_group.read 0;\n" ::: "memory");
+          __syncwarp();
+        }
+        wg_sync(wg);
+        {
+          const int r0 = (warp & 3) * 16 + (lane >> 2);
+#pragma unroll
+          for (int j = 0; j < kSW / 8; ++j) {
+            const int col = 8 * j + 2 * (lane & 3);
+            const int jj = p * (kSW / 8) + j;
+#pragma unroll
+            for (int h = 0; h < 2; ++h) {
+              const int r = r0 + 8 * h;
+              const int rb = r & 31;
+              float* blk = acc_s + ((r >> 5) * (kSW / 32) + (col >> 5)) * 1024;
+              const int unit = ((col & 31) >> 2) ^ (rb & 7);
+              *reinterpret_cast<float2*>(blk + rb * 32 + unit * 4 + (col & 3)) = make_float2(d[4 * jj + 2 * h], d[4 * jj + 2 * h + 1]);
+            }
+          }
+        }
+        if (MODE == kModeWgrad && use_tma_red) asm volatile("fence.proxy.async.shared::cta;\n" ::: "memory");
+        wg_sync(wg);
+        if (ew == 0 && lane == 0 && lw < 3 && p == 0) PULSE_TRACE(16 + 2 * lw);
+
 #pragma unroll 1
-      for (int c = chalf * kChunks; c < chalf * kChunks + kChunks; ++c) {
-        const int col0 = n0 + c * 32;
-        const bool full = col0 + 32 <= N;
-        float* blk = acc_s + ((quarter & 1) * 4 + c) * 1024;
-        if (MODE == kModeWgrad && use_tma_red) {
-          if (lane == 0) {
-            asm volatile("cp.reduce.async.bulk.tensor.2d.global.shared::cta.add.tile.bulk_group [%0, {%2, %3}], [%1];\n" ::"l"(&map_c),
-                         "r"(s_u32(blk)), "r"(col0), "r"(m0 + quarter * 32)
-                         : "memory");
-            asm volatile("cp.async.bulk.commit_group;\n" ::: "memory");
-          }
-          continue;
-        }
-        float v[32];
-        {
-          const float4* b4 = reinterpret_cast<const float4*>(blk) + lane * 8;
-#pragma unroll
-          for (int u = 0; u < 8; ++u) {
-            const float4 x = b4[u ^ (lane & 7)];
-            v[4 * u] = x.x; v[4 * u + 1] = x.y; v[4 * u + 2] = x.z; v[4 * u + 3] = x.w;
-          }
-        }
-        if (MODE != kModeWgrad && ep.alpha != 1.0f) {
-#pragma unroll
-          for (int i = 0; i < 32; ++i) v[i] *= ep.alpha;
-        }
-        if (fwd_fast) {
-          if (ep.bias != nullptr) {
-            const float4* b4 = reinterpret_cast<const float4*>(bias_s + (c % kChunks) * 32);
+        for (int cc = 0; cc < kCh; ++cc) {
+          const int wc = p * kCh + cc;
+          const int c = chunk_of(wc);
+          const int col0 = n0 + c * 32;
+          const bool full = col0 + 32 <= N;
+          float* blk = acc_s + ((quarter & 1) * (kSW / 32) + c - p * (kSW / 32)) * 1024;
+          if (MODE == kModeWgrad && use_tma_red) {
+            if (lane == 0) {
+              asm volatile("cp.reduce.async.bulk.tensor.2d.global.shared::cta.add.tile.bulk_group [%0, {%2, %3}], [%1];\n" ::"l"(&map_c),
+                           "r"(s_u32(blk)), "r"(col0), "r"(m0 + quarter * 32)
+                           : "memory");
+              asm volatile("cp.async.bulk.commit_group;\n" ::: "memory");
+            }
+            continue;
+          }
+          float v[32];
+          {
+            const float4* b4 = reinterpret_cast<const float4*>(blk) + lane * 8;
+#pragma unroll
+            for (int u = 0; u < 8; ++u) {
+              const float4 x = b4[u ^ (lane & 7)];
+              v[4 * u] = x.x; v[4 * u + 1] = x.y; v[4 * u + 2] = x.z; v[4 * u + 3] = x.w;
+            }
+          }
+          if (MODE != kModeWgrad && ep.alpha != 1.0f) {
+#pragma unroll
+            for (int i = 0; i < 32; ++i) v[i] *= ep.alpha;
+          }
+          if (fwd_fast && group_full(wc)) {
+            if (ep.bias != nullptr) {
+              const float4* b4 = reinterpret_cast<const float4*>(bias_s + wc * 32);
+#pragma unroll
+              for (int i = 0; i < 32; i += 4) {
+                const float4 b = b4[i >> 2];
+                v[i] += b.x; v[i + 1] += b.y; v[i + 2] += b.z; v[i + 3] += b.w;
+              }
+            }
+            if (ep.relu_mask != nullptr) {
+              unsigned word = 0u;
+#pragma unroll
+              for (int i = 0; i < 32; ++i) word |= (v[i] > 0.0f ? 1u : 0u) << i;
+              if (row_ok) ep.relu_mask[static_cast<long long>(col0 >> 5) * ep.ld_rmask + row] = word;
+            }
+            uint4* st = reinterpret_cast<uint4*>(red_stage);
+            const int sw = (lane >> 1) & 3;
+#pragma unroll
+            for (int q = 0; q < 4; ++q) {
+              const int i = 8 * q;
+              __nv_bfloat162 h0 = __floats2bfloat162_rn(v[i], v[i + 1]), h1 = __floats2bfloat162_rn(v[i + 2], v[i + 3]);
+              __nv_bfloat162 h2 = __floats2bfloat162_rn(v[i + 4], v[i + 5]), h3 = __floats2bfloat162_rn(v[i + 6], v[i + 7]);
+              uint4 u;
+              u.x = *reinterpret_cast<unsigned*>(&h0);
+              u.y = *reinterpret_cast<unsigned*>(&h1);
+              u.z = *reinterpret_cast<unsigned*>(&h2);
+              u.w = *reinterpret_cast<unsigned*>(&h3);
+              st[lane * 4 + (q ^ sw)] = u;
+            }
+            __syncwarp();
+            const long long coff = col0 + (lane & 3) * 8;
+            const __nv_bfloat162 zero2 = __float2bfloat162_rn(0.0f);
+#pragma unroll
+            for (int it2 = 0; it2 < 4; ++it2) {
+              const int rr = it2 * 8 + (lane >> 2);
+              uint4 u = st[rr * 4 + ((lane & 3) ^ ((rr >> 1) & 3))];
+              __nv_bfloat162* h = reinterpret_cast<__nv_bfloat162*>(&u);
+              const long long grow = m0 + quarter * 32 + rr;
+              if (grow < M) {
+                if (ep.preact != nullptr) *reinterpret_cast<uint4*>(reinterpret_cast<__nv_bfloat16*>(ep.preact) + grow * ep.ldp + coff) = u;
+                if (ep.act == PULSE_ACT_RELU) {
+#pragma unroll
+                  for (int q = 0; q < 4; ++q) h[q] = __hmax2(h[q], zero2);
+                } else if (ep.act == PULSE_ACT_SILU) {
+#pragma unroll
+                  for (int q = 0; q < 4; ++q) h[q] = silu_bf16x2(h[q]);
+                }
+                *reinterpret_cast<uint4*>(reinterpret_cast<__nv_bfloat16*>(ep.out) + grow * ep.ldo + coff) = u;
+              }
+            }
+            __syncwarp();
+            continue;
+          }
+          if (kFwd && ep.bias != nullptr) {
+            const float4* b4 = reinterpret_cast<const float4*>(bias_s + wc * 32);
 #pragma unroll
             for (int i = 0; i < 32; i += 4) {
               const float4 b = b4[i >> 2];
               v[i] += b.x; v[i + 1] += b.y; v[i + 2] += b.z; v[i + 3] += b.w;
             }
           }
-          if (ep.relu_mask != nullptr) {
+          if (kFwd && ep.preact != nullptr) {
+            if (full && (ep.ldp & 7) == 0) {
+              store_block_bf16(reinterpret_cast<uint4*>(red_stage), v,
+                               reinterpret_cast<__nv_bfloat16*>(ep.preact) + static_cast<long long>(m0 + quarter * 32) * ep.ldp + col0, ep.ldp,
+                               M - (m0 + quarter * 32), lane);
+            } else if (row_ok) {
+              __nv_bfloat16* p = reinterpret_cast<__nv_bfloat16*>(ep.preact) + static_cast<long long>(row) * ep.ldp + col0;
+#pragma unroll
+              for (int i = 0; i < 32; ++i)
+                if (col0 + i < N) p[i] = __float2bfloat16(v[i]);
+            }
+          }
+          if (kFwd && ep.relu_mask != nullptr && row_ok) {
             unsigned word = 0u;
 #pragma unroll
-            for (int i = 0; i < 32; ++i) word |= (v[i] > 0.0f ? 1u : 0u) << i;
-            if (row_ok) ep.relu_mask[static_cast<long long>(col0 >> 5) * ep.ld_rmask + row] = word;
-          }
-          uint4* st = reinterpret_cast<uint4*>(red_stage);
-          const int sw = (lane >> 1) & 3;
-#pragma unroll
-          for (int q = 0; q < 4; ++q) {
-            const int i = 8 * q;
-            __nv_bfloat162 h0 = __floats2bfloat162_rn(v[i], v[i + 1]), h1 = __floats2bfloat162_rn(v[i + 2], v[i + 3]);
-            __nv_bfloat162 h2 = __floats2bfloat162_rn(v[i + 4], v[i + 5]), h3 = __floats2bfloat162_rn(v[i + 6], v[i + 7]);
-            uint4 u;
-            u.x = *reinterpret_cast<unsigned*>(&h0);
-            u.y = *reinterpret_cast<unsigned*>(&h1);
-            u.z = *reinterpret_cast<unsigned*>(&h2);
-            u.w = *reinterpret_cast<unsigned*>(&h3);
-            st[lane * 4 + (q ^ sw)] = u;
-          }
-          __syncwarp();
-          const long long coff = col0 + (lane & 3) * 8;
-          const __nv_bfloat162 zero2 = __float2bfloat162_rn(0.0f);
-#pragma unroll
-          for (int it2 = 0; it2 < 4; ++it2) {
-            const int rr = it2 * 8 + (lane >> 2);
-            uint4 u = st[rr * 4 + ((lane & 3) ^ ((rr >> 1) & 3))];
-            __nv_bfloat162* h = reinterpret_cast<__nv_bfloat162*>(&u);
-            const long long grow = m0 + quarter * 32 + rr;
-            if (grow < M) {
-              if (ep.preact != nullptr) *reinterpret_cast<uint4*>(reinterpret_cast<__nv_bfloat16*>(ep.preact) + grow * ep.ldp + coff) = u;
-              if (ep.act == PULSE_ACT_RELU) {
-#pragma unroll
-                for (int q = 0; q < 4; ++q) h[q] = __hmax2(h[q], zero2);
-              } else if (ep.act == PULSE_ACT_SILU) {
-#pragma unroll
-                for (int q = 0; q < 4; ++q) h[q] = silu_bf16x2(h[q]);
-              }
-              *reinterpret_cast<uint4*>(reinterpret_cast<__nv_bfloat16*>(ep.out) + grow * ep.ldo + coff) = u;
-            }
-          }
-          __syncwarp();
-          continue;
-        }
-        if (kFwd && ep.bias != nullptr) {
-          float bl = bias_l[0];
-#pragma unroll
-          for (int cc = 1; cc < kChunks; ++cc) bl = (c % kChunks) == cc ? bias_l[cc] : bl;
-#pragma unroll
-          for (int i = 0; i < 32; ++i) v[i] += __shfl_sync(0xffffffffu, bl, i);
-        }
-        if (kFwd && ep.preact != nullptr) {
-          if (full && (ep.ldp & 7) == 0) {
-            store_block_bf16(reinterpret_cast<uint4*>(red_stage), v,
-                             reinterpret_cast<__nv_bfloat16*>(ep.preact) + static_cast<long long>(m0 + quarter * 32) * ep.ldp + col0, ep.ldp,
-                             M - (m0 + quarter * 32), lane);
-          } else if (row_ok) {
-            __nv_bfloat16* p = reinterpret_cast<__nv_bfloat16*>(ep.preact) + static_cast<long long>(row) * ep.ldp + col0;
+            for (int i = 0; i < 32; ++i) word |= ((col0 + i < N && v[i] > 0.0f) ? 1u : 0u) << i;
+            if (col0 < N) ep.relu_mask[static_cast<long long>(col0 >> 5) * ep.ld_rmask + row] = word;
+          }
+          if (kFwd && ep.act != PULSE_ACT_NONE) {
+#pragma unroll
+            for (int i = 0; i < 32; ++i) v[i] = act_apply(v[i], ep.act);
+          }
+          if (gate_bits) {
+            unsigned mk = gmask[0];
+#pragma unroll
+            for (int k = 1; k < kWC; ++k) mk = wc == k ? gmask[k] : mk;
+#pragma unroll
+            for (int i = 0; i < 32; ++i) v[i] = ((mk >> i) & 1u) ? v[i] : 0.0f;
+          } else if (gate_fast && group_full(wc)) {
+            unsigned mk = gmask[0];
+#pragma unroll
+            for (int k = 1; k < kWC; ++k) mk = wc == k ? gmask[k] : mk;
+#pragma unroll
+            for (int i = 0; i < 32; ++i) v[i] = ((mk >> ((i >> 1) + 16 * (i & 1))) & 1u) ? v[i] : 0.0f;
+          } else if (kDgrad && ep.gate != nullptr && row_ok) {
+            const __nv_bfloat16* g = reinterpret_cast<const __nv_bfloat16*>(ep.gate) + static_cast<long long>(row) * ep.ldg + col0;
+            if (full && (gate_vec || (ep.ldg & 7) == 0)) {
+#pragma unroll
+              for (int i = 0; i < 32; i += 8) {
+                const uint4 u = gate_vec ? gq[i >> 3] : __ldg(reinterpret_cast<const uint4*>(g + i));
+                const __nv_bfloat162* h = reinterpret_cast<const __nv_bfloat162*>(&u);
+#pragma unroll
+                for (int q = 0; q < 4; ++q) {
+                  const float2 f = __bfloat1622float2(h[q]);
+                  v[i + 2 * q] *= act_grad(f.x, ep.gate_mode);
+                  v[i + 2 * q + 1] *= act_grad(f.y, ep.gate_mode);
+                }
+              }
+            } else {
+#pragma unroll
+              for (int i = 0; i < 32; ++i)
+                if (col0 + i < N) v[i] *= act_grad(__bfloat162float(g[i]), ep.gate_mode);
+            }
+          }
+          if (gate_vec && wc != kWC - 1) gate_fetch(chunk_of(wc + 1));
+          if (kDgrad && ep.sumsq != nullptr && row_ok) {
 #pragma unroll
             for (int i = 0; i < 32; ++i)
-              if (col0 + i < N) p[i] = __float2bfloat16(v[i]);
-          }
-        }
-        if (kFwd && ep.relu_mask != nullptr && row_ok) {
-          unsigned word = 0u;
-#pragma unroll
-          for (int i = 0; i < 32; ++i) word |= ((col0 + i < N && v[i] > 0.0f) ? 1u : 0u) << i;
-          if (col0 < N) ep.relu_mask[static_cast<long long>(col0 >> 5) * ep.ld_rmask + row] = word;
-        }
-        if (kFwd && ep.act != PULSE_ACT_NONE) {
-#pragma unroll
-          for (int i = 0; i < 32; ++i) v[i] = act_apply(v[i], ep.act);
-        }
-        if (gate_bits) {
-          unsigned mk = gmask[0];
-#pragma unroll
-          for (int cc = 1; cc < kChunks; ++cc) mk = (c % kChunks) == cc ? gmask[cc] : mk;
-#pragma unroll
-          for (int i = 0; i < 32; ++i) v[i] = ((mk >> i) & 1u) ? v[i] : 0.0f;
-        } else if (gate_fast) {
-          unsigned mk = gmask[0];
-#pragma unroll
-          for (int cc = 1; cc < kChunks; ++cc) mk = (c % kChunks) == cc ? gmask[cc] : mk;
-#pragma unroll
-          for (int i = 0; i < 32; ++i) v[i] = ((mk >> ((i >> 1) + 16 * (i & 1))) & 1u) ? v[i] : 0.0f;
-        } else if (kDgrad && ep.gate != nullptr && row_ok) {
-          const __nv_bfloat16* g = reinterpret_cast<const __nv_bfloat16*>(ep.gate) + static_cast<long long>(row) * ep.ldg + col0;
-          if (full && (gate_vec || (ep.ldg & 7) == 0)) {
-#pragma unroll
-            for (int i = 0; i < 32; i += 8) {
-              const uint4 u = gate_vec ? gq[i >> 3] : __ldg(reinterpret_cast<const uint4*>(g + i));
-              const __nv_bfloat162* h = reinterpret_cast<const __nv_bfloat162*>(&u);
-#pragma unroll
-              for (int q = 0; q < 4; ++q) {
-                const float2 f = __bfloat1622float2(h[q]);
-                v[i + 2 * q] *= act_grad(f.x, ep.gate_mode);
-                v[i + 2 * q + 1] *= act_grad(f.y, ep.gate_mode);
-              }
-            }
-          } else {
+              if (full || col0 + i < N) sq = fmaf(v[i], v[i], sq);
+          }
+          if (kDgrad && ep.colsum != nullptr) {
+            float wv[32];
+#pragma unroll
+            for (int i = 0; i < 32; ++i) wv[i] = row_ok ? v[i] : 0.0f;
+#pragma unroll
+            for (int half = 16; half >= 1; half >>= 1) {
+              const bool upper = (lane & half) != 0;
+#pragma unroll
+              for (int i = 0; i < half; ++i) {
+                const float mine = upper ? wv[i + half] : wv[i];
+                const float send = upper ? wv[i] : wv[i + half];
+                wv[i] = mine + __shfl_xor_sync(0xffffffffu, send, half);
+              }
+            }
+            if (col0 + lane < N) atomicAdd(ep.colsum + col0 + lane, wv[0]);
+          }
+          if (kAccum && outf != nullptr && ep.accumulate) {
+#pragma unroll
+            for (int hr = 0; hr < 2; ++hr) {
+              if ((lane >> 4) == hr) {
+#pragma unroll
+                for (int i = 0; i < 32; ++i) red_stage[(lane & 15) * 33 + i] = v[i];
+              }
+              __syncwarp();
+              const int rbase = m0 + quarter * 32 + hr * 16;
+              const int rows_here = min(16, M - rbase);
+              if (col0 + lane < N) {
+                float* p = outf + static_cast<long long>(rbase) * ep.ldf + col0 + lane;
+                for (int rr = 0; rr < rows_here; ++rr) atomicAdd(p + static_cast<long long>(rr) * ep.ldf, red_stage[rr * 33 + lane]);
+              }
+              __syncwarp();
+            }
+          } else if (outf != nullptr && row_ok) {
+            float* p = outf + static_cast<long long>(row) * ep.ldf + col0;
+            if (full && (ep.ldf & 3) == 0 && (reinterpret_cast<uintptr_t>(outf) & 15u) == 0) {
+#pragma unroll
+              for (int i = 0; i < 32; i += 4) *reinterpret_cast<float4*>(p + i) = make_float4(v[i], v[i + 1], v[i + 2], v[i + 3]);
+            } else {
+#pragma unroll
+              for (int i = 0; i < 32; ++i)
+                if (col0 + i < N) p[i] = v[i];
+            }
+          }
+          if (kBf16Out && ep.out != nullptr) {
+            if (full && (ep.ldo & 7) == 0) {
+              store_block_bf16(reinterpret_cast<uint4*>(red_stage), v,
+                               reinterpret_cast<__nv_bfloat16*>(ep.out) + static_cast<long long>(m0 + quarter * 32) * ep.ldo + col0, ep.ldo,
+                               M - (m0 + quarter * 32), lane);
+            } else if (row_ok) {
+              __nv_bfloat16* p = reinterpret_cast<__nv_bfloat16*>(ep.out) + static_cast<long long>(row) * ep.ldo + col0;
+#pragma unroll
+              for (int i = 0; i < 32; ++i)
+                if (col0 + i < N) p[i] = __float2bfloat16(v[i]);
+            }
+          }
+          if (kFwd && ep.out_t != nullptr && row_ok) {
 #pragma unroll
             for (int i = 0; i < 32; ++i)
-              if (col0 + i < N) v[i] *= act_grad(__bfloat162float(g[i]), ep.gate_mode);
-          }
-        }
-        if (gate_vec && c != chalf * kChunks + kChunks - 1) gate_fetch(c + 1);
-        if (kDgrad && ep.sumsq != nullptr && row_ok) {
-#pragma unroll
-          for (int i = 0; i < 32; ++i)
-            if (full || col0 + i < N) sq = fmaf(v[i], v[i], sq);
-        }
-        if (kDgrad && ep.colsum != nullptr) {
-          float wv[32];
-#pragma unroll
-          for (int i = 0; i < 32; ++i) wv[i] = row_ok ? v[i] : 0.0f;
-#pragma unroll
-          for (int half = 16; half >= 1; half >>= 1) {
-            const bool upper = (lane & half) != 0;
-#pragma unroll
-            for (int i = 0; i < half; ++i) {
-              const float mine = upper ? wv[i + half] : wv[i];
-              const float send = upper ? wv[i] : wv[i + half];
-              wv[i] = mine + __shfl_xor_sync(0xffffffffu, send, half);
-            }
-          }
-          if (col0 + lane < N) atomicAdd(ep.colsum + col0 + lane, wv[0]);
-        }
-        if (kAccum && outf != nullptr && ep.accumulate) {
-#pragma unroll
-          for (int hr = 0; hr < 2; ++hr) {
-            if ((lane >> 4) == hr) {
-#pragma unroll
-              for (int i = 0; i < 32; ++i) red_stage[(lane & 15) * 33 + i] = v[i];
-            }
-            __syncwarp();
-            const int rbase = m0 + quarter * 32 + hr * 16;
-            const int rows_here = min(16, M - rbase);
-            if (col0 + lane < N) {
-              float* p = outf + static_cast<long long>(rbase) * ep.ldf + col0 + lane;
-              for (int rr = 0; rr < rows_here; ++rr) atomicAdd(p + static_cast<long long>(rr) * ep.ldf, red_stage[rr * 33 + lane]);
-            }
-            __syncwarp();
-          }
-        } else if (outf != nullptr && row_ok) {
-          float* p = outf + static_cast<long long>(row) * ep.ldf + col0;
-          if (full && (ep.ldf & 3) == 0 && (reinterpret_cast<uintptr_t>(outf) & 15u) == 0) {
-#pragma unroll
-            for (int i = 0; i < 32; i += 4) *reinterpret_cast<float4*>(p + i) = make_float4(v[i], v[i + 1], v[i + 2], v[i + 3]);
-          } else {
-#pragma unroll
-            for (int i = 0; i < 32; ++i)
-              if (col0 + i < N) p[i] = v[i];
-          }
-        }
-        if (kBf16Out && ep.out != nullptr) {
-          if (full && (ep.ldo & 7) == 0) {
-            store_block_bf16(reinterpret_cast<uint4*>(red_stage), v,
-                             reinterpret_cast<__nv_bfloat16*>(ep.out) + static_cast<long long>(m0 + quarter * 32) * ep.ldo + col0, ep.ldo,
-                             M - (m0 + quarter * 32), lane);
-          } else if (row_ok) {
-            __nv_bfloat16* p = reinterpret_cast<__nv_bfloat16*>(ep.out) + static_cast<long long>(row) * ep.ldo + col0;
-#pragma unroll
-            for (int i = 0; i < 32; ++i)
-              if (col0 + i < N) p[i] = __float2bfloat16(v[i]);
-          }
-        }
-        if (kFwd && ep.out_t != nullptr && row_ok) {
-#pragma unroll
-          for (int i = 0; i < 32; ++i)
-            if (col0 + i < N)
-              reinterpret_cast<__nv_bfloat16*>(ep.out_t)[static_cast<long long>(col0 + i) * ep.ldot + row] = __float2bfloat16(v[i]);
+              if (col0 + i < N)
+                reinterpret_cast<__nv_bfloat16*>(ep.out_t)[static_cast<long long>(col0 + i) * ep.ldot + row] = __float2bfloat16(v[i]);
+          }
         }
       }
       if (MODE == kModeWgrad && use_tma_red) {
diff --git a/pulse_b200/csrc/gemm_wgmma.cu b/pulse_b200/csrc/gemm_wgmma.cu
--- a/pulse_b200/csrc/gemm_wgmma.cu
+++ b/pulse_b200/csrc/gemm_wgmma.cu
@@ -11,24 +11,24 @@
 #ifndef PULSE_GEMM_VARIANT
 #define PULSE_GEMM_VARIANT 0
 #endif
-constexpr int BM = 128, BN = 128, BK = 64, MMA_K = 16;
+constexpr int BM = 128, BK = 64, MMA_K = 16;
 constexpr int kConsumerWarps = 8;
 constexpr int kThreads = 128 + 32 * kConsumerWarps;
-constexpr int kCols = 64;
-constexpr int kChunks = kCols / 32;
-constexpr int kStages = 4;
 constexpr unsigned kStageBytesA = BM * BK * 2;
-constexpr unsigned kStageBytesB = BN * BK * 2;
-
+template <int BN> constexpr int kStageCols = BN == 256 ? 64 : 128;
+template <int BN> constexpr int kStages = BN == 256 ? 3 : 4;
+
+template <int BN>
 struct __align__(1024) GemmSmem {
-  unsigned char a[kStages][kStageBytesA];
-  unsigned char b[kStages][kStageBytesB];
-  float acc[2][64 * BN];
+  unsigned char a[kStages<BN>][kStageBytesA];
+  unsigned char b[kStages<BN>][BN * BK * 2];
+  float acc[2][64 * kStageCols<BN>];
   float red[kConsumerWarps][16 * 33];
-  float bias[kConsumerWarps][kCols];
-  unsigned long long full[kStages];
-  unsigned long long empty[kStages];
+  float bias[kConsumerWarps][BN / 2];
+  unsigned long long full[kStages<BN>];
+  unsigned long long empty[kStages<BN>];
 };
+static_assert(sizeof(GemmSmem<256>) + 1024 <= 227 * 1024, "128 x 256 tile: shared memory over the 227 KB per block");
 
 __device__ __forceinline__ unsigned s_u32(const void* p) { return static_cast<unsigned>(__cvta_generic_to_shared(p)); }
 __device__ __forceinline__ void g_mbar_init(unsigned long long* bar, unsigned count) {
@@ -76,9 +76,10 @@
 __device__ __forceinline__ void wgmma_commit() { asm volatile("wgmma.commit_group.sync.aligned;\n" ::: "memory"); }
 template <int N>
 __device__ __forceinline__ void wgmma_wait() { asm volatile("wgmma.wait_group.sync.aligned %0;\n" ::"n"(N) : "memory"); }
-__device__ __forceinline__ void acc_fence(float (&d)[64]) {
+template <int N>
+__device__ __forceinline__ void acc_fence(float (&d)[N]) {
 #pragma unroll
-  for (int i = 0; i < 64; ++i) asm volatile("" : "+f"(d[i])::"memory");
+  for (int i = 0; i < N; ++i) asm volatile("" : "+f"(d[i])::"memory");
 }
 template <int TA, int TB>
 __device__ __forceinline__ void wgmma_m64n128(float (&d)[64], unsigned long long da, unsigned long long db, unsigned accumulate) {
@@ -86,9 +87,11 @@
       "{\n\t.reg .pred p;\n\t"
       "setp.ne.b32 p, %66, 0;\n\t"
       "wgmma.mma_async.sync.aligned.m64n128k16.f32.bf16.bf16 "
-      "{%0, %1, %2, %3, %4, %5, %6, %7, %8, %9, %10, %11, %12, %13, %14, %15, %16, %17, %18, %19, %20, %21, %22, %23, %24, %25, %26, "
-      "%27, %28, %29, %30, %31, %32, %33, %34, %35, %36, %37, %38, %39, %40, %41, %42, %43, %44, %45, %46, %47, %48, %49, %50, %51, "
-      "%52, %53, %54, %55, %56, %57, %58, %59, %60, %61, %62, %63}, "
+      "{"
+      "%0, %1, %2, %3, %4, %5, %6, %7, %8, %9, %10, %11, %12, %13, %14, %15, %16, %17, %18, %19, %20, %21, %22, %23, %24, %25, "
+      "%26, %27, %28, %29, %30, %31, %32, %33, %34, %35, %36, %37, %38, %39, %40, %41, %42, %43, %44, %45, %46, %47, %48, %49, %50, %51, "
+      "%52, %53, %54, %55, %56, %57, %58, %59, %60, %61, %62, %63"
+      "}, "
       "%64, %65, p, 1, 1, %67, %68;\n\t}\n"
       : "+f"(d[0]), "+f"(d[1]), "+f"(d[2]), "+f"(d[3]), "+f"(d[4]), "+f"(d[5]), "+f"(d[6]), "+f"(d[7]),
         "+f"(d[8]), "+f"(d[9]), "+f"(d[10]), "+f"(d[11]), "+f"(d[12]), "+f"(d[13]), "+f"(d[14]), "+f"(d[15]),
@@ -100,6 +103,44 @@
         "+f"(d[56]), "+f"(d[57]), "+f"(d[58]), "+f"(d[59]), "+f"(d[60]), "+f"(d[61]), "+f"(d[62]), "+f"(d[63])
       : "l"(da), "l"(db), "r"(accumulate), "n"(TA), "n"(TB)
       : "memory");
+}
+template <int TA, int TB>
+__device__ __forceinline__ void wgmma_m64n256(float (&d)[128], unsigned long long da, unsigned long long db, unsigned accumulate) {
+  asm volatile(
+      "{\n\t.reg .pred p;\n\t"
+      "setp.ne.b32 p, %130, 0;\n\t"
+      "wgmma.mma_async.sync.aligned.m64n256k16.f32.bf16.bf16 "
+      "{"
+      "%0, %1, %2, %3, %4, %5, %6, %7, %8, %9, %10, %11, %12, %13, %14, %15, %16, %17, %18, %19, %20, %21, %22, %23, %24, %25, "
+      "%26, %27, %28, %29, %30, %31, %32, %33, %34, %35, %36, %37, %38, %39, %40, %41, %42, %43, %44, %45, %46, %47, %48, %49, %50, %51, "
+      "%52, %53, %54, %55, %56, %57, %58, %59, %60, %61, %62, %63, %64, %65, %66, %67, %68, %69, %70, %71, %72, %73, %74, %75, %76, %77, "
+      "%78, %79, %80, %81, %82, %83, %84, %85, %86, %87, %88, %89, %90, %91, %92, %93, %94, %95, %96, %97, %98, %99, %100, %101, %102, %103, "
+      "%104, %105, %106, %107, %108, %109, %110, %111, %112, %113, %114, %115, %116, %117, %118, %119, %120, %121, %122, %123, %124, %125, %126, %127"
+      "}, "
+      "%128, %129, p, 1, 1, %131, %132;\n\t}\n"
+      : "+f"(d[0]), "+f"(d[1]), "+f"(d[2]), "+f"(d[3]), "+f"(d[4]), "+f"(d[5]), "+f"(d[6]), "+f"(d[7]),
+        "+f"(d[8]), "+f"(d[9]), "+f"(d[10]), "+f"(d[11]), "+f"(d[12]), "+f"(d[13]), "+f"(d[14]), "+f"(d[15]),
+        "+f"(d[16]), "+f"(d[17]), "+f"(d[18]), "+f"(d[19]), "+f"(d[20]), "+f"(d[21]), "+f"(d[22]), "+f"(d[23]),
+        "+f"(d[24]), "+f"(d[25]), "+f"(d[26]), "+f"(d[27]), "+f"(d[28]), "+f"(d[29]), "+f"(d[30]), "+f"(d[31]),
+        "+f"(d[32]), "+f"(d[33]), "+f"(d[34]), "+f"(d[35]), "+f"(d[36]), "+f"(d[37]), "+f"(d[38]), "+f"(d[39]),
+        "+f"(d[40]), "+f"(d[41]), "+f"(d[42]), "+f"(d[43]), "+f"(d[44]), "+f"(d[45]), "+f"(d[46]), "+f"(d[47]),
+        "+f"(d[48]), "+f"(d[49]), "+f"(d[50]), "+f"(d[51]), "+f"(d[52]), "+f"(d[53]), "+f"(d[54]), "+f"(d[55]),
+        "+f"(d[56]), "+f"(d[57]), "+f"(d[58]), "+f"(d[59]), "+f"(d[60]), "+f"(d[61]), "+f"(d[62]), "+f"(d[63]),
+        "+f"(d[64]), "+f"(d[65]), "+f"(d[66]), "+f"(d[67]), "+f"(d[68]), "+f"(d[69]), "+f"(d[70]), "+f"(d[71]),
+        "+f"(d[72]), "+f"(d[73]), "+f"(d[74]), "+f"(d[75]), "+f"(d[76]), "+f"(d[77]), "+f"(d[78]), "+f"(d[79]),
+        "+f"(d[80]), "+f"(d[81]), "+f"(d[82]), "+f"(d[83]), "+f"(d[84]), "+f"(d[85]), "+f"(d[86]), "+f"(d[87]),
+        "+f"(d[88]), "+f"(d[89]), "+f"(d[90]), "+f"(d[91]), "+f"(d[92]), "+f"(d[93]), "+f"(d[94]), "+f"(d[95]),
+        "+f"(d[96]), "+f"(d[97]), "+f"(d[98]), "+f"(d[99]), "+f"(d[100]), "+f"(d[101]), "+f"(d[102]), "+f"(d[103]),
+        "+f"(d[104]), "+f"(d[105]), "+f"(d[106]), "+f"(d[107]), "+f"(d[108]), "+f"(d[109]), "+f"(d[110]), "+f"(d[111]),
+        "+f"(d[112]), "+f"(d[113]), "+f"(d[114]), "+f"(d[115]), "+f"(d[116]), "+f"(d[117]), "+f"(d[118]), "+f"(d[119]),
+        "+f"(d[120]), "+f"(d[121]), "+f"(d[122]), "+f"(d[123]), "+f"(d[124]), "+f"(d[125]), "+f"(d[126]), "+f"(d[127])
+      : "l"(da), "l"(db), "r"(accumulate), "n"(TA), "n"(TB)
+      : "memory");
+}
+template <int BN, int TA, int TB>
+__device__ __forceinline__ void wgmma_step(float (&d)[BN / 2], unsigned long long da, unsigned long long db, unsigned accumulate) {
+  if constexpr (BN == 256) wgmma_m64n256<TA, TB>(d, da, db, accumulate);
+  else wgmma_m64n128<TA, TB>(d, da, db, accumulate);
 }
 
 __device__ __forceinline__ float act_apply(float x, int act) {
@@ -164,6 +205,7 @@
 enum : int { kModeGeneric = 0, kModeFwd = 1, kModeDgrad = 2, kModeWgrad = 3, kModeDgradVec = 4 };
 
 constexpr int kMaxGroup = 4;
+constexpr int kGroupedBN = 128;
 struct GemmProblem {
   CUtensorMap map_a, map_b, map_c;
   pulse_gemm_epilogue_t ep;
@@ -223,7 +265,7 @@
   return ep.out_f32 != nullptr && ep.accumulate && (ep.ldf % 4) == 0 && (reinterpret_cast<uintptr_t>(ep.out_f32) % 16) == 0;
 }
 
-constexpr size_t kSmemBytes = sizeof(GemmSmem) + 1024;
+template <int BN> constexpr size_t kSmemBytes = sizeof(GemmSmem<BN>) + 1024;
 
 int gemm_num_sms(bool honour_limit) {
   static int num_sms = 0, limited = 0;
@@ -237,9 +279,18 @@
   return honour_limit ? limited : num_sms;
 }
 
-template <bool A_MN, bool B_MN, int MODE>
+long long ceil_div(long long a, long long b) { return (a + b - 1) / b; }
+
+int tile_n(long long m, long long n, int splits, int sms) {
+  const long long tm = ceil_div(m, BM);
+  const long long w256 = ceil_div(tm * ceil_div(n, 256) * splits, sms) * 256;
+  const long long w128 = ceil_div(tm * ceil_div(n, 128) * splits, sms) * 128;
+  return w256 <= w128 ? 256 : 128;
+}
+
+template <bool A_MN, bool B_MN, int MODE, int BN>
 int launch_gemm(const CUtensorMap& map_a, const CUtensorMap& map_b, const pulse_gemm_epilogue_t& ep, int m, int n, int k, int splits,
-                int kb_per_split, cudaStream_t stream) {
+                int kb_per_split, int num_sms, cudaStream_t stream) {
   static bool attr_set = false;
   CUtensorMap map_c;
   memset(&map_c, 0, sizeof(map_c));
@@ -252,11 +303,9 @@
     use_tma_red = 1;
   }
   if (!attr_set) {
-    PULSE_CUDA_OK(cudaFuncSetAttribute(gemm_bf16_kernel<A_MN, B_MN, MODE>, cudaFuncAttributeMaxDynamicSharedMemorySize, (int)kSmemBytes));
+    PULSE_CUDA_OK(cudaFuncSetAttribute(gemm_bf16_kernel<A_MN, B_MN, MODE, BN>, cudaFuncAttributeMaxDynamicSharedMemorySize, (int)kSmemBytes<BN>));
     attr_set = true;
   }
-  const int num_sms = gemm_num_sms(true);
-  PULSE_REQUIRE(num_sms > 0, "pulse_gemm_bf16: cannot query the device's SM count");
   const long long total = static_cast<long long>((n + BN - 1) / BN) * ((m + BM - 1) / BM) * splits;
   const unsigned grid = static_cast<unsigned>(total < num_sms ? total : num_sms);
   static int use_pdl = -1;
@@ -267,7 +316,7 @@
   cudaLaunchConfig_t cfg = {};
   cfg.gridDim = dim3(grid, 1, 1);
   cfg.blockDim = dim3(kThreads, 1, 1);
-  cfg.dynamicSmemBytes = kSmemBytes;
+  cfg.dynamicSmemBytes = kSmemBytes<BN>;
   cfg.stream = stream;
   cudaLaunchAttribute attr[1];
   int na = 0;
@@ -278,7 +327,7 @@
   }
   cfg.attrs = attr;
   cfg.numAttrs = na;
-  PULSE_CUDA_OK(cudaLaunchKernelEx(&cfg, gemm_bf16_kernel<A_MN, B_MN, MODE>, map_a, map_b, map_c, ep, m, n, k, kb_per_split, splits, use_tma_red));
+  PULSE_CUDA_OK(cudaLaunchKernelEx(&cfg, gemm_bf16_kernel<A_MN, B_MN, MODE, BN>, map_a, map_b, map_c, ep, m, n, k, kb_per_split, splits, use_tma_red));
   PULSE_LAUNCH_OK("gemm_bf16_kernel");
   return PULSE_OK;
 }
@@ -287,7 +336,8 @@
 int launch_gemm_grouped(const GemmGroup& grp, cudaStream_t stream) {
   static bool attr_set = false;
   if (!attr_set) {
-    PULSE_CUDA_OK(cudaFuncSetAttribute(gemm_bf16_grouped_kernel<A_MN, B_MN, MODE>, cudaFuncAttributeMaxDynamicSharedMemorySize, (int)kSmemBytes));
+    PULSE_CUDA_OK(cudaFuncSetAttribute(gemm_bf16_grouped_kernel<A_MN, B_MN, MODE, kGroupedBN>, cudaFuncAttributeMaxDynamicSharedMemorySize,
+                                       (int)kSmemBytes<kGroupedBN>));
     attr_set = true;
   }
   const int num_sms = gemm_num_sms(false);
@@ -296,14 +346,14 @@
   cudaLaunchConfig_t cfg = {};
   cfg.gridDim = dim3(grid, 1, 1);
   cfg.blockDim = dim3(kThreads, 1, 1);
-  cfg.dynamicSmemBytes = kSmemBytes;
+  cfg.dynamicSmemBytes = kSmemBytes<kGroupedBN>;
   cfg.stream = stream;
   cudaLaunchAttribute attr[1];
   attr[0].id = cudaLaunchAttributeProgrammaticStreamSerialization;
   attr[0].val.programmaticStreamSerializationAllowed = 1;
   cfg.attrs = attr;
   cfg.numAttrs = 1;
-  PULSE_CUDA_OK(cudaLaunchKernelEx(&cfg, gemm_bf16_grouped_kernel<A_MN, B_MN, MODE>, grp));
+  PULSE_CUDA_OK(cudaLaunchKernelEx(&cfg, gemm_bf16_grouped_kernel<A_MN, B_MN, MODE, kGroupedBN>, grp));
   PULSE_LAUNCH_OK("gemm_bf16_grouped_kernel");
   return PULSE_OK;
 }
@@ -332,6 +382,34 @@
   int splits = split_k < 1 ? 1 : (split_k > num_kb ? num_kb : split_k);
   const int kb_per_split = (num_kb + splits - 1) / splits;
   return (num_kb + kb_per_split - 1) / kb_per_split;
+}
+
+extern "C" int pulse_gemm_split_k(int64_t m, int64_t n, int64_t k) {
+  using namespace pulse;
+  constexpr int kEpilogueKb = 24;
+  constexpr int sms = 132;
+  if (m <= 0 || n <= 0 || k <= 0) return 0;
+  const int num_kb = static_cast<int>(ceil_div(k, BK));
+  int best = 1;
+  long long best_cost = -1;
+  for (int s = 1; s <= (num_kb < 64 ? num_kb : 64); ++s) {
+    const int per = static_cast<int>(ceil_div(num_kb, s));
+    if (ceil_div(num_kb, per) != s) continue;
+    const int bn = tile_n(m, n, s, sms);
+    const long long cost = ceil_div(ceil_div(m, BM) * ceil_div(n, bn) * s, sms) * (per + kEpilogueKb) * bn;
+    if (best_cost < 0 || cost < best_cost) {
+      best = s;
+      best_cost = cost;
+    }
+  }
+  return best;
+}
+
+extern "C" int pulse_gemm_tile_n(int64_t m, int64_t n, int64_t k, int32_t split_k) {
+  using namespace pulse;
+  const int sms = gemm_num_sms(true);
+  if (sms <= 0 || m <= 0 || n <= 0 || k <= 0) return 0;
+  return tile_n(m, n, pulse_gemm_num_splits(k, split_k), sms);
 }
 
 extern "C" int pulse_gemm_bf16(const void* a, int64_t lda, const void* b, int64_t ldb, int64_t m, int64_t n, int64_t k,
@@ -354,32 +432,39 @@
   PULSE_REQUIRE((ep->relu_mask == nullptr || ep->ld_rmask >= m) && (ep->gate_mask == nullptr || ep->ld_gmask >= m),
                 "pulse_gemm_bf16: mask word rows must hold at least M entries");
   PULSE_REQUIRE(!(ep->gate_mask && ep->gate), "pulse_gemm_bf16: give the ReLU gate either as bf16 activations or as bit words, not both");
+  const int num_sms = gemm_num_sms(true);
+  PULSE_REQUIRE(num_sms > 0, "pulse_gemm_bf16: cannot query the device's SM count");
+  const int num_kb = static_cast<int>((k + BK - 1) / BK);
+  const int splits = pulse_gemm_num_splits(k, split_k);
+  const int kb_per_split = (num_kb + splits - 1) / splits;
+  const int bn = tile_n(m, n, splits, num_sms);
   CUtensorMap map_a, map_b;
   const bool ok_a = a_mn ? make_map(&map_a, a, k, m, lda, 64) : make_map(&map_a, a, m, k, lda, BM);
-  const bool ok_b = b_mn ? make_map(&map_b, b, k, n, ldb, 64) : make_map(&map_b, b, n, k, ldb, BN);
+  const bool ok_b = b_mn ? make_map(&map_b, b, k, n, ldb, 64) : make_map(&map_b, b, n, k, ldb, bn);
   if (!ok_a || !ok_b) {
     set_error("pulse_gemm_bf16: cuTensorMapEncodeTiled failed (driver entry point missing or bad strides)");
     return PULSE_ERR_CUDA;
   }
-  const int num_kb = static_cast<int>((k + BK - 1) / BK);
-  const int splits = pulse_gemm_num_splits(k, split_k);
-  const int kb_per_split = (num_kb + splits - 1) / splits;
   cudaStream_t st = static_cast<cudaStream_t>(stream);
   const int mode = epilogue_mode(ep);
   const int mi = (int)m, ni = (int)n, ki = (int)k;
-#define PULSE_GEMM_DISPATCH(AM, BM_)                                                                                        \
-  switch (mode) {                                                                                                           \
-    case kModeFwd: return launch_gemm<AM, BM_, kModeFwd>(map_a, map_b, *ep, mi, ni, ki, splits, kb_per_split, st);             \
-    case kModeDgrad: return launch_gemm<AM, BM_, kModeDgrad>(map_a, map_b, *ep, mi, ni, ki, splits, kb_per_split, st);         \
-    case kModeWgrad: return launch_gemm<AM, BM_, kModeWgrad>(map_a, map_b, *ep, mi, ni, ki, splits, kb_per_split, st);         \
-    case kModeDgradVec: return launch_gemm<AM, BM_, kModeDgradVec>(map_a, map_b, *ep, mi, ni, ki, splits, kb_per_split, st);   \
-    default: return launch_gemm<AM, BM_, kModeGeneric>(map_a, map_b, *ep, mi, ni, ki, splits, kb_per_split, st);               \
+#define PULSE_GEMM_LAUNCH(AM, BM_, MD)                                                                                          \
+  return bn == 256 ? launch_gemm<AM, BM_, MD, 256>(map_a, map_b, *ep, mi, ni, ki, splits, kb_per_split, num_sms, st)            \
+                   : launch_gemm<AM, BM_, MD, 128>(map_a, map_b, *ep, mi, ni, ki, splits, kb_per_split, num_sms, st);
+#define PULSE_GEMM_DISPATCH(AM, BM_)                                  \
+  switch (mode) {                                                     \
+    case kModeFwd: PULSE_GEMM_LAUNCH(AM, BM_, kModeFwd)               \
+    case kModeDgrad: PULSE_GEMM_LAUNCH(AM, BM_, kModeDgrad)           \
+    case kModeWgrad: PULSE_GEMM_LAUNCH(AM, BM_, kModeWgrad)           \
+    case kModeDgradVec: PULSE_GEMM_LAUNCH(AM, BM_, kModeDgradVec)     \
+    default: PULSE_GEMM_LAUNCH(AM, BM_, kModeGeneric)                 \
   }
   if (a_mn && b_mn) { PULSE_GEMM_DISPATCH(true, true) }
   if (a_mn) { PULSE_GEMM_DISPATCH(true, false) }
   if (b_mn) { PULSE_GEMM_DISPATCH(false, true) }
   PULSE_GEMM_DISPATCH(false, false)
 #undef PULSE_GEMM_DISPATCH
+#undef PULSE_GEMM_LAUNCH
 }
 
 extern "C" int pulse_gemm_bf16_nt(const void* a, int64_t lda, const void* b, int64_t ldb, int64_t m, int64_t n, int64_t k,
@@ -420,7 +505,7 @@
     const pulse_gemm_problem_t& q = problems[i];
     GemmProblem& g = grp.p[i];
     const bool ok_a = a_mn ? make_map(&g.map_a, q.a, q.k, q.m, q.lda, 64) : make_map(&g.map_a, q.a, q.m, q.k, q.lda, BM);
-    const bool ok_b = b_mn ? make_map(&g.map_b, q.b, q.k, q.n, q.ldb, 64) : make_map(&g.map_b, q.b, q.n, q.k, q.ldb, BN);
+    const bool ok_b = b_mn ? make_map(&g.map_b, q.b, q.k, q.n, q.ldb, 64) : make_map(&g.map_b, q.b, q.n, q.k, q.ldb, kGroupedBN);
     if (!ok_a || !ok_b) {
       set_error("pulse_gemm_bf16_grouped: cuTensorMapEncodeTiled failed for problem %d", i);
       return PULSE_ERR_CUDA;
@@ -440,7 +525,7 @@
     const int num_kb = static_cast<int>((q.k + BK - 1) / BK);
     const int splits = pulse_gemm_num_splits(q.k, q.split_k);
     g.kb_per_split = (num_kb + splits - 1) / splits;
-    items += static_cast<long long>((q.n + BN - 1) / BN) * ((q.m + BM - 1) / BM) * splits;
+    items += static_cast<long long>((q.n + kGroupedBN - 1) / kGroupedBN) * ((q.m + BM - 1) / BM) * splits;
     PULSE_REQUIRE(items < (1ll << 30), "pulse_gemm_bf16_grouped: too many work items");
     g.item_end = static_cast<int>(items);
   }
diff --git a/pulse_b200/dense.py b/pulse_b200/dense.py
--- a/pulse_b200/dense.py
+++ b/pulse_b200/dense.py
@@ -15,6 +15,20 @@
 
 def num_splits(k: int, split_k: int) -> int:
     return int(_lib.load().pulse_gemm_num_splits(k, split_k))
+
+
+def split_k(m: int, n: int, k: int) -> int:
+    s = int(_lib.load().pulse_gemm_split_k(m, n, k))
+    if s < 1:
+        raise _lib.PulseError(f"pulse_gemm_split_k: empty problem {m} x {n} x {k}")
+    return s
+
+
+def tile_n(m: int, n: int, k: int, split_k: int = 1) -> int:
+    w = int(_lib.load().pulse_gemm_tile_n(m, n, k, split_k))
+    if w < 1:
+        raise _lib.PulseError("pulse_gemm_tile_n: cannot query the device's SM count")
+    return w
 
 
 def ordered_sum_add(x: torch.Tensor, out: torch.Tensor) -> None:
diff --git a/pulse_b200/nets.py b/pulse_b200/nets.py
--- a/pulse_b200/nets.py
+++ b/pulse_b200/nets.py
@@ -7,7 +7,7 @@
 import torch
 
 from . import _lib
-from .dense import gemm, gemm_nt
+from .dense import gemm, gemm_nt, split_k
 
 
 def pad8(n: int) -> int:
@@ -293,8 +293,8 @@
                     ws["pre"].append(bf(M, l.Np) if (l.act == "silu") else None)
                     ws["dact"].append(None if last else bf(M, l.Np))
                     ws["mask"].append(torch.zeros((l.N + 31) // 32, M, device=dev, dtype=torch.int32) if (l.act == "relu" and not last) else None)
-                    tiles = ((l.N + 127) // 128) * ((l.Kp + 127) // 128)
-                    ws["split"].append(pick_split(tiles, (M + 63) // 64))
+                    with torch.cuda.device(dev):
+                        ws["split"].append(split_k(l.N, l.Kp, M))
             hn = self.layers[-1].N
             ws["out"] = torch.zeros(M, (hn + 3) // 4 * 4, device=dev)[:, :hn]
             if train and self.input_grad_cols:
```

Result: faster. 1.494 million, median of 6 (+3.8%).
